# libsdl-org/libjxl

Hardware: AMD Instinct MI355X
Metric: megapixels/sec decode, 3840x2160 VarDCT d1.0 (higher is better)
Workload: dtype f32

## Files before the change

libjxl_amd/csrc/hip/jxl_hip_api.hip:

```cpp
#include <hip/hip_runtime.h>

#include <cmath>
#include <cstdio>
#include <cstdlib>
#include <cstring>
#include <algorithm>
#include <atomic>
#include <unistd.h>
#include <mutex>
#include <new>
#include <chrono>
#include <string>
#include <vector>

#include "../../../include/jxl_amd_hip.h"
#include "../host/jxh_enc_shared.h"
#include "jxl_hip_kernels.h"
#include "jxl_hip_entropy_lanes.h"
#include "jxl_hip_filter_fused.h"
#include "jxl_hip_modular.h"
#include "jxl_hip_enc.h"
#include "jxl_hip_canvas.h"
#include "jxl_hip_dc.h"

namespace {
#include "../host/afv_basis.inc"
#include "../host/dither.inc"

#define HIP_TRY(expr)                          \
  do {                                         \
    hipError_t e_ = (expr);                    \
    if (e_ != hipSuccess) return -int(e_);     \
  } while (0)

std::atomic<bool> g_yield_waits{false};
inline hipError_t WaitStream(hipStream_t st) {
  if (!g_yield_waits.load(std::memory_order_relaxed)) return hipStreamSynchronize(st);
  for (;;) {
    const hipError_t q = hipStreamQuery(st);
    if (q != hipErrorNotReady) return q;
    usleep(200);
  }
}
inline hipError_t WaitEvent(hipEvent_t ev) {
  if (!g_yield_waits.load(std::memory_order_relaxed)) return hipEventSynchronize(ev);
  for (;;) {
    const hipError_t q = hipEventQuery(ev);
    if (q != hipErrorNotReady) return q;
    usleep(100);
  }
}

constexpr size_t kGuardBytes = 4096;
inline bool GuardOn() {
  const char* e = getenv("JXLHIP_GUARD");
  return e && *e && atoi(e) != 0;
}
inline int GuardByte() {
  const char* e = getenv("JXLHIP_GUARD_BYTE");
  return e && *e ? (int(strtol(e, nullptr, 0)) & 0xFF) : 0xA5;
}

struct Buf {
  void* p = nullptr;
  size_t cap = 0;
  bool view = false;
  void* base = nullptr;
  int guard_byte = 0xA5;
  int Ensure(size_t n) {
    if (view) {
      p = nullptr;
      cap = 0;
      view = false;
    }
    if (n <= cap && p) return 0;
    if (p) {
      hipError_t e = hipFree(base ? base : p);
      p = base = nullptr;
      cap = 0;
      if (e != hipSuccess) return -int(e);
    }
    size_t want = n < 256 ? 256 : n;
    if (GuardOn()) {
      want = (want + 255) & ~size_t(255);
      hipError_t e = hipMalloc(&base, want + 2 * kGuardBytes);
      guard_byte = GuardByte();
      if (e == hipSuccess) e = hipMemset(base, guard_byte, want + 2 * kGuardBytes);
      if (e == hipSuccess) e = hipStreamSynchronize(nullptr);
      if (e != hipSuccess) {
        if (base) (void)hipFree(base);
        base = nullptr;
        return -int(e);
      }
      p = static_cast<uint8_t*>(base) + kGuardBytes;
      cap = want;
      return 0;
    }
    hipError_t e = hipMalloc(&p, want);
    if (e != hipSuccess) {
      p = nullptr;
      return -int(e);
    }
    cap = want;
    return 0;
  }
  void Free() {
    if (p && !view) (void)hipFree(base ? base : p);
    p = base = nullptr;
    cap = 0;
    view = false;
  }
  int GuardsTouched() const {
    if (!base || view) return 0;
    std::vector<uint8_t> h(2 * kGuardBytes);
    if (hipMemcpy(h.data(), base, kGuardBytes, hipMemcpyDeviceToHost) != hipSuccess) return 3;
    if (hipMemcpy(h.data() + kGuardBytes, static_cast<uint8_t*>(base) + kGuardBytes + cap, kGuardBytes, hipMemcpyDeviceToHost) != hipSuccess) return 3;
    int r = 0;
    for (size_t i = 0; i < kGuardBytes; i++) {
      if (h[i] != guard_byte) r |= 1;
      if (h[kGuardBytes + i] != guard_byte) r |= 2;
    }
    return r;
  }
  template <typename T>
  T* as() const { return static_cast<T*>(p); }
};

struct PassBufs {
  Buf ctx_map, alias, cfg, orders, ptable, poffset, alias_packed;
};

struct ModLaunch {
  uint32_t kind;
  size_t offset;
  uint32_t count, gx, gy;
};

struct Stage {
  uint8_t* p = nullptr;
  size_t cap = 0, used = 0;
  hipEvent_t done = nullptr;
  bool recorded = false;
};

constexpr int kEntropyWPG = 4;
constexpr int kLanesAdmitWaves = 4;
constexpr size_t kLdsBudget = 150 * 1024;

}

struct JxlHipContext {
  int device = 0;
  hipStream_t stream = nullptr;
  hipEvent_t ev[6] = {};
  bool ev_valid[3] = {false, false, false};
  Buf basis;
  Stage stage;
  Buf frame_blob;
  bool blob_mode = false;
  bool have_frame = false;
  uint32_t xs = 0, ys = 0, xb = 0, yb = 0, xg = 0, ng = 0, np = 0, xp = 0, yp = 0, coef_bits = 16;
  int gab = 0, epf_iters = 0;
  float epf_pass0 = 0.9f, epf_pass2 = 6.5f, epf_border = 2.0f / 3;
  Buf sections, sec_word, sec_size, blocks, gbb, bctx_lut, dequant, dc, inv_sigma, ytox, ytob, passes_dev, coeffs, errors;
  Buf dc_q, dc_ep;
  Buf dc_raw, sharp;
  Buf plane[3], rgb, tlist, scratch, sec_end, lz_window;
  bool generic_codec = false;
  bool lane_prefix = false;
  struct Modular {
    bool have = false;
    Buf pool, sections, blob, streams, rects, status, end_bits, scratch, windows, batch_streams;
    std::vector<size_t> buf_off;
    std::vector<uint32_t> buf_w, buf_h;
    std::vector<JxlHipModOp> ops;
    std::vector<jxlhip::ModStream> streams_host;
    std::vector<uint32_t> stream_samples;
    uint32_t out_buffer[4] = {0, 0, 0, 0};
    uint32_t num_color = 3, has_alpha = 0, bits = 8, alpha_bits = 8, xs = 0, ys = 0, nstreams = 0;
    bool xyb = false;
    float xyb_factor[3] = {0, 0, 0};
    jxlhip::FilterParams xyb_color;
    JxlHipColorTarget xyb_target;
    std::vector<const JxlHipContext*> batch_ctxs;
    std::vector<uint64_t> batch_gens;
    uint32_t batch_n = 0, batch_tree_cap = 0, batch_table_cap = 0;
    bool batch_wp = true, batch_refs = true;
    std::vector<uint32_t> code_table_words;
    Buf batch_ops;
    std::vector<ModLaunch> batch_launches;
  } mod;
  size_t plane_bytes = 0;
  Buf ep_dev;
  size_t batch_off_units = 0, batch_off_queue = 0, batch_off_wave_lanes = 0, batch_units = 0;
  Buf batch_params, batch_map, batch_lanes;
  uint32_t batch_wait_shift = 2;
  bool batch_galias = false;
  bool batch_a6 = false;
  bool batch_prefix = false;
  int batch_kernel = -1;
  std::vector<uint32_t> sec_size_host, sec_sel_host, pass_clusters, pass_log_alpha;
  std::vector<uint32_t> group_list;
  std::vector<uint32_t> absent_groups;
  std::vector<uint32_t> absent_blocks;
  std::vector<uint32_t> absent_sections;
  uint32_t band_y0 = 0, band_y1 = 0;
  uint32_t ext_y0 = 0, ext_y1 = 0;
  uint32_t ups = 1, oxs = 0, oys = 0;
  Buf ups_kernel;
  bool scan_order = false;
  bool lanes = false, lane_multi = false;
  uint32_t nblocks = 0;
  bool keep_filtered = false;
  bool keep_upsampled = false;
  bool ups_kept = false;
  bool transform_dense = false;
  bool band_halo = false;
  uint32_t out_type = 2, out_nc = 3, out_bits = 8, out_swap = 0;
  Buf enc_rgb, enc_planes[3], enc_act, enc_acs, enc_qf, enc_off, enc_dc, enc_coef, enc_lut, enc_dq, enc_ytox, enc_ytob;
  hipEvent_t enc_ev[6] = {nullptr, nullptr, nullptr, nullptr, nullptr, nullptr};
  bool enc_timed = false;
  jxlhip::EncTok enc_tok;
  bool enc_tok_ready = false;
  std::vector<uint32_t> enc_tok_totals;
  Buf enc_tok_orders, enc_tok_blk, enc_tok_info, enc_tok_off, enc_tok_nzmap, enc_tok_small, enc_tok_out, enc_tok_base;
  std::vector<uint32_t> ent_base, ent_count, ent_bits;
  bool ent_resident = false, ent_sized = false, ent_timed[3] = {false, false, false};
  jxlhip::EncAns ent;
  Buf ent_counts, ent_status, ent_grp, ent_tab, ent_rec, ent_fl, ent_small, ent_out, ent_obase;
  hipEvent_t ent_ev[6] = {nullptr, nullptr, nullptr, nullptr, nullptr, nullptr};
  jxlhip::EncFwd enc_last;
  jxlhip::EncAq enc_last_aq;
  Buf enc_aq_cells, enc_aq_map, enc_aq_mask, enc_aq_in;
  Buf enc_mask1x1;
  hipEvent_t mask_ev[2] = {nullptr, nullptr};
  bool mask_timed = false;
  bool enc_last_gaborish = false;
  uint32_t out_orient = 0;
  bool out_unpremul = false;
  Buf spl_seg, spl_row_start, spl_row_seg, spl_planes;
  uint32_t spl_segments = 0;
  Buf pat_rec, pat_row_start, pat_row_list;
  uint32_t pat_positions = 0;
  const float* pat_src[4] = {nullptr, nullptr, nullptr, nullptr};
  const float* pat_src_alpha[4] = {nullptr, nullptr, nullptr, nullptr};
  bool pat_uses_alpha = false, pat_premultiplied = false;
  Buf alpha_patched;
  bool alpha_patched_valid = false;
  uint32_t pat_src_w[4] = {0, 0, 0, 0}, pat_src_h[4] = {0, 0, 0, 0};
  bool keep_xyb = false;
  Buf noise;
  bool has_noise = false;
  float noise_lut[8] = {0, 0, 0, 0, 0, 0, 0, 0};
  uint32_t noise_seed[2] = {0, 0};
  float noise_ytox = 0.0f, noise_ytob = 1.0f;
  Buf alpha;
  bool have_alpha = false;
  bool color_out = false;
  bool gray8_fast = false;
  JxlHipColorTarget ct{};
  Buf kend, block_recs, dequant_scan;
  Buf trecs;
  Buf ec_stage;
  std::vector<JxlHipVarBlock> blocks_host;
  std::vector<uint32_t> gbb_host;
  std::vector<uint16_t> orders_host;
  uint32_t order_offset_host[39] = {};
  std::vector<const JxlHipContext*> batch_ctxs;
  std::vector<uint64_t> batch_gens;
  uint32_t batch_wgs = 0;
  size_t batch_lds = 0;
  hipEvent_t batch_done = nullptr;
  hipEvent_t pending_wait = nullptr;
  bool filter_async = false;
  bool entropy_gate = false;
  hipEvent_t halo_event = nullptr;
  Buf ups_planes;
  bool pooled_once = false;
  bool owns_stream = false;
  hipStream_t stream2 = nullptr;
  hipStream_t fstream = nullptr;
  hipEvent_t fork_event = nullptr, filter_done = nullptr, filter_wait = nullptr;
  hipEvent_t transform_done = nullptr;
  bool transform_done_valid = false;
  JxlHipContext* plane_lender = nullptr;
  hipEvent_t planes_event = nullptr;
  hipStream_t planes_stream = nullptr;
  struct FilterGroup {
    int key;
    uint32_t first, count, tiles_x, tiles_y;
    bool u8srgb;
  };
  Buf tb_params, tb_desc, fb_params;
  std::vector<const JxlHipContext*> db_ctxs;
  std::vector<uint64_t> db_gens;
  uint32_t desc_begin[27] = {}, desc_count[27] = {};
  uint32_t cs = 0;
  std::vector<FilterGroup> fgroups;
  hipEvent_t down_done = nullptr;
  uint64_t generation = 0;
  std::vector<PassBufs> pass_bufs;
  uint32_t list_begin[27] = {}, list_count[27] = {};
  jxlhip::EntropyParams ep;
  jxlhip::TransformParams tp;
  jxlhip::FilterParams fp;
  size_t lds_entropy = 0;
  bool alias_lds = false;
  int final_plane = 0;
};

static bool SectionEntropyForced() {
  static const bool v = [] {
    const char* e = getenv("JXLHIP_ENTROPY");
    return e && e[0] == '1';
  }();
  return v;
}
static JxlHipContext* PlaneHolder(JxlHipContext* c) { return c->plane_lender ? c->plane_lender : c; }
static const JxlHipContext* PlaneHolder(const JxlHipContext* c) { return c->plane_lender ? c->plane_lender : c; }

static size_t OutSampleBytes(const JxlHipContext* c) { return c->out_type == 2 ? 1 : (c->out_type == 0 ? 4 : 2); }
static size_t OutPixelBytes(const JxlHipContext* c) { return OutSampleBytes(c) * c->out_nc; }
static bool OutIsRgb8(const JxlHipContext* c) { return c->out_type == 2 && c->out_nc == 3 && c->out_bits == 8; }
static bool OutIsGray8(const JxlHipContext* c) { return c->out_type == 2 && c->out_nc == 1 && c->out_bits == 8; }
static bool OutIsRgbF32(const JxlHipContext* c) { return c->out_type == 0 && c->out_nc == 3 && !c->out_swap; }

static bool ValidPrefixTables(uint32_t offset_word, const uint32_t* table, size_t table_size) {
  const size_t first = offset_word & 0xFFFFFFu, root_bits = offset_word >> 24;
  if (root_bits > 15 || first + (size_t(1) << root_bits) > table_size) return false;
  for (size_t r = 0; r < (size_t(1) << root_bits); r++) {
    const uint32_t e = table[first + r];
    if (!(e & 0x80u)) {
      if ((e & 0xFFu) > 15) return false;
      continue;
    }
    const size_t sub_bits = e & 0x7Fu, sub = first + (e >> 8);
    if (sub_bits == 0 || root_bits + sub_bits > 15 || sub + (size_t(1) << sub_bits) > table_size) return false;
    for (size_t j = 0; j < (size_t(1) << sub_bits); j++)
      if ((table[sub + j] & 0x80u) || (table[sub + j] & 0xFFu) > 15) return false;
  }
  return true;
}

static int EnvInt(const char* name, int def) {
  const char* e = getenv(name);
  return e && *e ? atoi(e) : def;
}

extern "C" {

const char* jxlhip_version(void) { return "libjxl_amd 0.1 (gfx950)"; }

int jxlhip_device_count(void) {
  int n = 0;
  if (hipGetDeviceCount(&n) != hipSuccess) return 0;
  return n;
}

static hipStream_t PoolStream(int device) {
  static std::mutex mu;
  static std::vector<hipStream_t> pool[64];
  static size_t next[64] = {};
  std::lock_guard<std::mutex> lock(mu);
  if (device < 0 || device >= 64) return nullptr;
  if (pool[device].empty()) {
    int n = 4;
    if (const char* e = getenv("JXLHIP_STREAMS")) n = atoi(e);
    n = n < 1 ? 1 : (n > 16 ? 16 : n);
    for (int i = 0; i < n; i++) {
      hipStream_t st = nullptr;
      if (hipStreamCreateWithFlags(&st, hipStreamNonBlocking) != hipSuccess) break;
      pool[device].push_back(st);
    }
    if (pool[device].empty()) return nullptr;
  }
  return pool[device][next[device]++ % pool[device].size()];
}

static int EnsureOwnStream(JxlHipContext* c);

static std::mutex g_ctx_pool_mu;
static std::vector<JxlHipContext*> g_ctx_pool;
constexpr size_t kCtxPoolMax = 4, kCtxPoolBytes = size_t(1) << 30;
static std::vector<Buf*> AllBufs(JxlHipContext* c);
static JxlHipContext* RecycleContext(int device) {
  if (GuardOn() || !EnvInt("JXLHIP_CTX_POOL", 1)) return nullptr;
  JxlHipContext* o = nullptr;
  {
    std::lock_guard<std::mutex> lk(g_ctx_pool_mu);
    for (size_t i = 0; i < g_ctx_pool.size(); i++)
      if (g_ctx_pool[i]->device == device) {
        o = g_ctx_pool[i];
        g_ctx_pool.erase(g_ctx_pool.begin() + long(i));
        break;
      }
  }
  if (!o) return nullptr;
  JxlHipContext* c = new (std::nothrow) JxlHipContext;
  if (!c) {
    jxlhip_ctx_destroy(o);
    return nullptr;
  }
  c->device = device;
  c->stream = PoolStream(device);
  std::vector<Buf*> to = AllBufs(c), from = AllBufs(o);
  for (size_t i = 0; i < to.size(); i++) {
    *to[i] = *from[i];
    if (to[i]->view) *to[i] = Buf();
    *from[i] = Buf();
  }
  c->pass_bufs = std::move(o->pass_bufs);
  o->pass_bufs.clear();
  for (size_t i = 0; i < sizeof(c->ev) / sizeof(c->ev[0]); i++) std::swap(c->ev[i], o->ev[i]);
  for (size_t i = 0; i < sizeof(c->enc_ev) / sizeof(c->enc_ev[0]); i++) std::swap(c->enc_ev[i], o->enc_ev[i]);
  for (size_t i = 0; i < sizeof(c->ent_ev) / sizeof(c->ent_ev[0]); i++) std::swap(c->ent_ev[i], o->ent_ev[i]);
  for (size_t i = 0; i < sizeof(c->mask_ev) / sizeof(c->mask_ev[0]); i++) std::swap(c->mask_ev[i], o->mask_ev[i]);
  std::swap(c->stage, o->stage);
  jxlhip_ctx_destroy(o);
  return c;
}

int jxlhip_ctx_create(int device, JxlHipContext** out) {
  if (!out) return JXLHIP_ERR_INVALID_ARGUMENT;
  *out = nullptr;
  HIP_TRY(hipSetDevice(device));
  if (JxlHipContext* recycled = RecycleContext(device)) {
    *out = recycled;
    return 0;
  }
  JxlHipContext* c = new (std::nothrow) JxlHipContext;
  if (!c) return JXLHIP_ERR_INVALID_ARGUMENT;
  c->device = device;
  hipError_t e = hipSuccess;
  c->stream = PoolStream(device);
  if (!c->stream) {
    delete c;
    return JXLHIP_ERR_INVALID_ARGUMENT;
  }
  for (auto& ev : c->ev) {
    e = hipEventCreate(&ev);
    if (e != hipSuccess) {
      delete c;
      return -int(e);
    }
  }
  constexpr size_t kBasisFloats = 87381;
  std::vector<float> bt(2 * kBasisFloats + 4);
  for (int l = 0; l <= 8; l++) {
    const int N = 1 << l;
    float* dst = bt.data() + (size_t(N) * N - 1) / 3;
    float* dst_t = dst + kBasisFloats + 3;
    for (int k = 0; k < N; k++)
      for (int n = 0; n < N; n++) {
        const float v = float((k ? std::sqrt(2.0) : 1.0) * std::cos((n + 0.5) * k * M_PI / N));
        dst[size_t(k) * N + n] = v;
        dst_t[size_t(n) * N + k] = v;
      }
  }
  int r = c->basis.Ensure(bt.size() * sizeof(float));
  if (r) {
    jxlhip_ctx_destroy(c);
    return r;
  }
  float resample[63];
  for (int n = 1; n <= 32; n *= 2)
    for (int i = 0; i < n; i++) {
      const double N = 8.0 * n;
      resample[n - 1 + i] = float(1.0 / (std::cos(i / (2 * N) * M_PI) * std::cos(i / N * M_PI) * std::cos(i / (N / 2) * M_PI)));
    }
  e = hipMemcpy(c->basis.p, bt.data(), bt.size() * sizeof(float), hipMemcpyHostToDevice);
  if (e == hipSuccess) e = hipMemcpyToSymbol(HIP_SYMBOL(jxlhip::c_afv_basis), kAfvBasis, sizeof(kAfvBasis));
  if (e == hipSuccess) e = hipMemcpyToSymbol(HIP_SYMBOL(jxlhip::c_dither), kDither32, sizeof(kDither32));
  if (e == hipSuccess) e = hipMemcpyToSymbol(HIP_SYMBOL(jxlhip::c_resample), resample, sizeof(resample));
  if (e != hipSuccess) {
    jxlhip_ctx_destroy(c);
    return -int(e);
  }
  *out = c;
  return 0;
}

static std::vector<Buf*> AllBufs(JxlHipContext* c) {
  std::vector<Buf*> all = {&c->basis, &c->sections, &c->sec_word, &c->sec_size, &c->blocks, &c->gbb, &c->bctx_lut, &c->dequant, &c->dc, &c->dc_raw, &c->dc_q, &c->dc_ep, &c->sharp,
                &c->inv_sigma, &c->ytox, &c->ytob, &c->passes_dev, &c->coeffs, &c->errors, &c->plane[0], &c->plane[1],
                &c->plane[2], &c->rgb, &c->tlist, &c->scratch, &c->ep_dev, &c->batch_params, &c->batch_map, &c->batch_lanes, &c->ups_kernel, &c->kend, &c->block_recs, &c->dequant_scan, &c->ec_stage, &c->alpha_patched, &c->trecs, &c->enc_tok_orders, &c->enc_tok_blk, &c->enc_tok_info,
                &c->enc_tok_off, &c->enc_tok_nzmap, &c->enc_tok_small, &c->enc_tok_out, &c->enc_tok_base, &c->tb_params, &c->tb_desc, &c->fb_params, &c->alpha, &c->sec_end, &c->lz_window, &c->mod.pool, &c->mod.sections, &c->mod.blob, &c->mod.streams,
                &c->mod.rects, &c->mod.status, &c->mod.end_bits, &c->mod.scratch, &c->mod.windows, &c->mod.batch_streams, &c->mod.batch_ops, &c->frame_blob, &c->noise, &c->spl_seg, &c->spl_row_start, &c->spl_row_seg, &c->spl_planes, &c->pat_rec, &c->pat_row_start, &c->pat_row_list,
                &c->enc_rgb, &c->enc_planes[0], &c->enc_planes[1], &c->enc_planes[2], &c->enc_act, &c->enc_acs, &c->enc_qf, &c->enc_off, &c->enc_dc, &c->enc_coef, &c->enc_lut, &c->enc_dq, &c->enc_ytox, &c->enc_ytob, &c->ups_planes, &c->enc_aq_cells, &c->enc_aq_map, &c->enc_aq_mask, &c->enc_aq_in, &c->enc_mask1x1,
                &c->ent_counts, &c->ent_status, &c->ent_grp, &c->ent_tab, &c->ent_rec, &c->ent_fl, &c->ent_small, &c->ent_out, &c->ent_obase};
  for (auto& pb : c->pass_bufs)
    for (Buf* b : {&pb.ctx_map, &pb.alias, &pb.cfg, &pb.orders, &pb.ptable, &pb.poffset, &pb.alias_packed}) all.push_back(b);
  return all;
}

void jxlhip_ctx_destroy(JxlHipContext* c) {
  if (!c) return;
  (void)hipSetDevice(c->device);
  if (c->stream) (void)hipStreamSynchronize(c->stream);
  if (c->stream2) (void)hipStreamSynchronize(c->stream2);
  if (c->basis.p && !c->pooled_once && !GuardOn() && EnvInt("JXLHIP_CTX_POOL", 1)) {
    size_t bytes = 0;
    for (Buf* b : AllBufs(c))
      if (!b->view) bytes += b->cap;
    std::lock_guard<std::mutex> lk(g_ctx_pool_mu);
    if (bytes <= kCtxPoolBytes && g_ctx_pool.size() < kCtxPoolMax) {
      c->pooled_once = true;
      g_ctx_pool.push_back(c);
      return;
    }
  }
  std::vector<Buf*> all = AllBufs(c);
  for (Buf* b : all) b->Free();
  for (auto& ev : c->ev)
    if (ev) (void)hipEventDestroy(ev);
  for (auto& ev : c->enc_ev)
    if (ev) (void)hipEventDestroy(ev);
  for (auto& ev : c->ent_ev)
    if (ev) (void)hipEventDestroy(ev);
  for (auto& ev : c->mask_ev)
    if (ev) (void)hipEventDestroy(ev);
  if (c->stage.done) (void)hipEventDestroy(c->stage.done);
  if (c->stage.p) (void)hipHostFree(c->stage.p);
  if (c->batch_done) (void)hipEventDestroy(c->batch_done);
  if (c->down_done) (void)hipEventDestroy(c->down_done);
  if (c->fork_event) (void)hipEventDestroy(c->fork_event);
  if (c->transform_done) (void)hipEventDestroy(c->transform_done);
  if (c->filter_done) (void)hipEventDestroy(c->filter_done);
  if (c->halo_event) (void)hipEventDestroy(c->halo_event);
  if (c->stream2) (void)hipStreamDestroy(c->stream2);
  if (c->stream && c->owns_stream) (void)hipStreamDestroy(c->stream);
  delete c;
}

static int ApplyPendingWait(JxlHipContext* c) {
  if (c->pending_wait) {
    HIP_TRY(hipStreamWaitEvent(c->stream, c->pending_wait, 0));
    c->pending_wait = nullptr;
  }
  if (c->filter_wait) {
    HIP_TRY(hipStreamWaitEvent(c->stream, c->filter_wait, 0));
    c->filter_wait = nullptr;
  }
  return 0;
}

static hipStream_t CopyStream(int device) {
  static std::mutex mu;
  static hipStream_t streams[64] = {};
  std::lock_guard<std::mutex> lock(mu);
  if (device < 0 || device >= 64) return nullptr;
  if (!streams[device]) {
    int lo = 0, hi = 0;
    if (hipDeviceGetStreamPriorityRange(&lo, &hi) != hipSuccess) return nullptr;
    if (hipStreamCreateWithPriority(&streams[device], hipStreamNonBlocking, hi) != hipSuccess) streams[device] = nullptr;
  }
  return streams[device];
}

static int StageReset(JxlHipContext* c) {
  Stage& s = c->stage;
  if (!s.done) HIP_TRY(hipEventCreateWithFlags(&s.done, hipEventDisableTiming));
  if (s.recorded) HIP_TRY(hipEventSynchronize(s.done));
  else if (s.used) HIP_TRY(hipStreamSynchronize(c->stream));
  s.recorded = false;
  s.used = 0;
  return 0;
}
static int StageAlloc(JxlHipContext* c, size_t bytes, void** out) {
  Stage& s = c->stage;
  const size_t need = (bytes + 63) & ~size_t(63);
  if (s.used + need > s.cap) {
    if (c->blob_mode) return JXLHIP_ERR_INVALID_ARGUMENT;
    HIP_TRY(hipStreamSynchronize(c->stream));
    if (hipStream_t cs = CopyStream(c->device)) HIP_TRY(hipStreamSynchronize(cs));
    size_t want = s.cap * 2 > need ? s.cap * 2 : need;
    if (want < (size_t(1) << 22)) want = size_t(1) << 22;
    if (s.p) HIP_TRY(hipHostFree(s.p));
    s.p = nullptr;
    s.cap = 0;
    HIP_TRY(hipHostMalloc(reinterpret_cast<void**>(&s.p), want, hipHostMallocDefault));
    s.cap = want;
    s.used = 0;
  }
  *out = s.p + s.used;
  s.used += need;
  return 0;
}
static int UploadStaged(JxlHipContext* c, Buf& b, const void* staged, size_t bytes) {
  if (c->blob_mode) {
    const size_t at = size_t(static_cast<const uint8_t*>(staged) - c->stage.p);
    if (!staged || at + (bytes ? bytes : 16) > c->frame_blob.cap) return JXLHIP_ERR_INVALID_ARGUMENT;
    if (!b.view) b.Free();
    b.p = c->frame_blob.as<uint8_t>() + at;
    b.cap = bytes ? bytes : 16;
// ... 622 lines not shown
        rec |= (bctx & 15u) << (12 + 4 * ch);
        if (!carried) rec |= 1u << (24 + ch);
        rec |= hs << (27 + ch);
      }
      recs[i] = rec;
    }
    if ((r = Upload(c, c->block_recs, recs.data(), recs.size() * 4))) return r;
    ep.block_recs = c->block_recs.as<uint32_t>();
  }
  lap("records");
  c->absent_blocks.clear();
  for (uint32_t g : c->absent_groups) {
    c->absent_blocks.push_back(d->group_block_begin[g]);
    c->absent_blocks.push_back(d->group_block_begin[g + 1] - d->group_block_begin[g]);
  }
  if (c->scan_order) {
    c->blocks_host.assign(d->blocks, d->blocks + d->num_blocks);
    c->gbb_host.assign(d->group_block_begin, d->group_block_begin + d->num_groups + 1);
    c->orders_host.assign(d->passes[0].orders, d->passes[0].orders + d->passes[0].orders_size);
    memcpy(c->order_offset_host, d->passes[0].order_offset, sizeof(c->order_offset_host));
  }
  if ((r = Upload(c, c->ep_dev, &ep, sizeof(ep)))) return r;
  c->generation++;

  jxlhip::TransformParams& tp = c->tp;
  memset(&tp, 0, sizeof(tp));
  tp.coeffs = c->coeffs.p;
  tp.coef_bits = d->coef_bits;
  tp.blocks = c->blocks.as<JxlHipVarBlock>();
  tp.dequant = c->dequant.as<float>();
  memcpy(tp.dq_offset, d->dequant_offset, sizeof(tp.dq_offset));
  memcpy(tp.dq_size, d->dequant_size, sizeof(tp.dq_size));
  for (int s = 0; s < 27; s++) {
    if (c->list_count[s] == 0) continue;
    const uint32_t k = jxlhip::kStrategyQuantTable[s];
    if (d->dequant_size[k] != 64u * jxlhip::CoveredBlocks(s) || size_t(d->dequant_offset[k]) + 3 * size_t(d->dequant_size[k]) > d->dequant_floats)
      return JXLHIP_ERR_INVALID_ARGUMENT;
  }
  tp.dense = c->transform_dense ? 1 : 0;
  tp.cs = cs;
  tp.cs_out = c->plane[1].as<float>();
  tp.dc = c->dc.as<float>();
  tp.ytox = c->ytox.as<int8_t>();
  tp.ytob = c->ytob.as<int8_t>();
  tp.basis_t = c->basis.as<float>();
  tp.basis_n = c->basis.as<float>() + 87381 + 3;
  tp.inv_global_scale = d->inv_global_scale;
  tp.x_dm = d->x_dm;
  tp.b_dm = d->b_dm;
  tp.color_scale = d->color_scale;
  tp.base_x = d->base_corr_x;
  tp.base_b = d->base_corr_b;
  memcpy(tp.biases, d->quant_biases, sizeof(tp.biases));
  tp.xb = c->xb; tp.yb = c->yb; tp.xg = c->xg; tp.xp = c->xp; tp.yp = c->yp;
  tp.out = PlaneHolder(c)->plane[0].as<float>();
  tp.scratch = c->scratch.as<float>();
  tp.tlist = c->tlist.as<uint32_t>();
  tp.trecs = c->trecs.as<uint4>();
  memcpy(tp.list_begin, c->list_begin, sizeof(tp.list_begin));
  memcpy(tp.list_count, c->list_count, sizeof(tp.list_count));
  tp.scan_order = c->scan_order ? 1 : 0;
  tp.kend = c->kend.as<uint32_t>();
  tp.orders = c->pass_bufs[0].orders.as<uint16_t>();
  tp.dequant_scan = nullptr;
  if (c->scan_order) {
    std::vector<float> scan(d->dequant_floats, 0.0f);
    for (int st = 0; st < 27; st++) {
      if (!c->list_count[st]) continue;
      const uint32_t kind = jxlhip::kStrategyQuantTable[st], size = d->dequant_size[kind];
      for (int ch = 0; ch < 3; ch++) {
        const uint32_t oo = d->passes[0].order_offset[jxlhip::kStrategyOrder[st] * 3 + ch];
        if (size_t(oo) + size > d->passes[0].orders_size) return JXLHIP_ERR_INVALID_ARGUMENT;
        const uint16_t* order = d->passes[0].orders + oo;
        const float* m = d->dequant + d->dequant_offset[kind] + size_t(ch) * size;
        float* o = scan.data() + d->dequant_offset[kind] + size_t(ch) * size;
        for (uint32_t k = 0; k < size; k++) {
          if (order[k] >= size) return JXLHIP_ERR_INVALID_ARGUMENT;
          o[k] = m[order[k]];
        }
      }
    }
    if ((r = Upload(c, c->dequant_scan, scan.data(), scan.size() * 4))) return r;
    tp.dequant_scan = c->dequant_scan.as<float>();
  }
  memcpy(tp.order_offset, d->passes[0].order_offset, sizeof(tp.order_offset));

  jxlhip::FilterParams& fp = c->fp;
  memset(&fp, 0, sizeof(fp));
  fp.xs = c->xs; fp.ys = c->ys; fp.xp = c->xp; fp.yp = c->yp; fp.xb = c->xb;
  fp.y_begin = c->band_y0; fp.y_end = c->band_y1;
  fp.inv_sigma = c->inv_sigma.as<float>();
  for (int ch = 0; ch < 3; ch++) {
    const float w1 = d->gab_w[ch * 2], w2 = d->gab_w[ch * 2 + 1];
    const float mul = 1.0f / (1.0f + 4 * (w1 + w2));
    fp.gab_w[ch * 3] = mul;
    fp.gab_w[ch * 3 + 1] = w1 * mul;
    fp.gab_w[ch * 3 + 2] = w2 * mul;
    fp.ch_scale[ch] = d->epf_channel_scale[ch];
    fp.opsin_bias[ch] = d->opsin_bias[ch];
    fp.opsin_bias_cbrt[ch] = cbrtf(d->opsin_bias[ch]);
  }
  memcpy(fp.opsin_inv, d->opsin_inv, sizeof(fp.opsin_inv));
  fp.linear_output = d->linear_output;
  c->gray8_fast = OutIsGray8(c) && !c->color_out;
  fp.rgb = OutIsRgb8(c) || c->gray8_fast ? c->rgb.as<uint8_t>() : nullptr;
  fp.rgbf = !OutIsRgb8(c) && !c->gray8_fast && !c->color_out ? c->rgb.as<float>() : nullptr;
  c->epf_pass0 = d->epf_pass0_sigma_scale;
  c->epf_pass2 = d->epf_pass2_sigma_scale;
  c->epf_border = d->epf_border_sad_mul;
  c->ev_valid[0] = c->ev_valid[1] = c->ev_valid[2] = false;
  if ((r = BlobEnd(c, dev_smooth && !d->dc_device ? &smooth_p : nullptr, dev_sigma ? &sigma_p : nullptr, dev_dequant ? &dequant_p : nullptr))) return r;
  HIP_TRY(WaitEvent(c->stage.done));
  lap("rest");
  if (prof) fprintf(stderr, "[upload] %s\n", prof_line.c_str());
  c->have_frame = true;
  c->mod.have = false;
  return 0;
}

}

template <typename CoefT>
static int LaunchEntropy(JxlHipContext* c) {
  const dim3 grid(c->ng), block(64);
  if (c->generic_codec) {
    hipLaunchKernelGGL(jxlhip::k_entropy_generic<CoefT>, grid, block, 3072, c->stream, c->ep);
  } else if (c->alias_lds) {
    const size_t shared = size_t(c->ep.lds_ctx_bytes) + c->ep.lds_alias_bytes + 1024;
    jxlhip::EntropyBatch b{c->ep_dev.as<jxlhip::EntropyParams>(), nullptr};
    if (c->ep.num_hist == 1) {
      constexpr int WPG = kEntropyWPG;
      auto k = jxlhip::k_entropy_uni<CoefT, WPG>;
      const size_t lds = shared + WPG * 5120;
      if (lds > 48 * 1024)
        HIP_TRY(hipFuncSetAttribute(reinterpret_cast<const void*>(k), hipFuncAttributeMaxDynamicSharedMemorySize, int(lds)));
      hipLaunchKernelGGL(k, dim3((c->ng + WPG - 1) / WPG), dim3(64 * WPG), lds, c->stream, b);
    } else {
      auto k = jxlhip::k_entropy_uni<CoefT, 1>;
      const size_t lds = shared + 5120;
      if (lds > 48 * 1024)
        HIP_TRY(hipFuncSetAttribute(reinterpret_cast<const void*>(k), hipFuncAttributeMaxDynamicSharedMemorySize, int(lds)));
      hipLaunchKernelGGL(k, grid, block, lds, c->stream, b);
    }
  } else {
    hipLaunchKernelGGL(jxlhip::k_entropy_ans<CoefT>, grid, block, c->lds_entropy, c->stream, c->ep);
  }
  HIP_TRY(hipGetLastError());
  return 0;
}

static int RunEntropySingle(JxlHipContext* c) {
  if (!c) return JXLHIP_ERR_INVALID_ARGUMENT;
  if (!c->have_frame) return JXLHIP_ERR_NO_FRAME;
  HIP_TRY(hipSetDevice(c->device));
  {
    int pw = ApplyPendingWait(c);
    if (pw) return pw;
  }
  HIP_TRY(hipEventRecord(c->ev[0], c->stream));
  HIP_TRY(hipMemsetAsync(c->errors.p, 0, size_t(c->ng) * 4, c->stream));
  int r = c->coef_bits == 16 ? LaunchEntropy<int16_t>(c) : LaunchEntropy<int32_t>(c);
  if (r) return r;
  HIP_TRY(hipEventRecord(c->ev[1], c->stream));
  c->ev_valid[0] = true;
  return 0;
}

static uint32_t BlocksPerWG(int s) {
  const uint32_t cx = jxlhip::kCoveredX[s], cy = jxlhip::kCoveredY[s];
  if (s == 0 || (s >= 4 && s <= 11) || (s >= 18 && s <= 20))
    return jxlhip::IdctFastThreads(cx, cy) / ((cx > cy ? cx : cy) * 8);
  return 4;
}

template <typename CoefT, int CX, int CY, bool CS = false>
static int LaunchIdctFast(JxlHipContext* c0, int s) {
  constexpr int C = CX * 8, R = CY * 8, TB = R > C ? R : C, GROUPS = jxlhip::IdctFastThreads(CX, CY) / TB;
  constexpr size_t lds = size_t(GROUPS) * R * (C + 1) * sizeof(float);
  const int li = CS ? 21 : s;
  hipLaunchKernelGGL((jxlhip::k_idct_fast<CoefT, CX, CY, CS>), dim3(c0->desc_count[li]), dim3(jxlhip::IdctFastThreads(CX, CY)), lds, c0->stream,
                     c0->tb_params.as<jxlhip::TransformParams>(), c0->tb_desc.as<uint2>() + c0->desc_begin[li], uint32_t(s));
  return 0;
}

template <typename CoefT>
static int LaunchTransforms(JxlHipContext* c0) {
  for (int s = 0; s < 21; s++) {
    if (!c0->desc_count[s]) continue;
    int e = 0;
    switch (s) {
      case 0: e = LaunchIdctFast<CoefT, 1, 1>(c0, s); break;
      case 4: e = LaunchIdctFast<CoefT, 2, 2>(c0, s); break;
      case 5: e = LaunchIdctFast<CoefT, 4, 4>(c0, s); break;
      case 6: e = LaunchIdctFast<CoefT, 1, 2>(c0, s); break;
      case 7: e = LaunchIdctFast<CoefT, 2, 1>(c0, s); break;
      case 8: e = LaunchIdctFast<CoefT, 1, 4>(c0, s); break;
      case 9: e = LaunchIdctFast<CoefT, 4, 1>(c0, s); break;
      case 10: e = LaunchIdctFast<CoefT, 2, 4>(c0, s); break;
      case 11: e = LaunchIdctFast<CoefT, 4, 2>(c0, s); break;
      case 18: e = LaunchIdctFast<CoefT, 8, 8>(c0, s); break;
      case 19: e = LaunchIdctFast<CoefT, 4, 8>(c0, s); break;
      case 20: e = LaunchIdctFast<CoefT, 8, 4>(c0, s); break;
      default:
        hipLaunchKernelGGL((jxlhip::k_special<CoefT>), dim3(c0->desc_count[s]), dim3(256), 0, c0->stream,
                           c0->tb_params.as<jxlhip::TransformParams>(), c0->tb_desc.as<uint2>() + c0->desc_begin[s], uint32_t(s));
    }
    if (e) return e;
    HIP_TRY(hipGetLastError());
  }
  if (c0->desc_count[21]) {
    int e = LaunchIdctFast<CoefT, 1, 1, true>(c0, 0);
    if (e) return e;
    HIP_TRY(hipGetLastError());
  }
  for (const JxlHipContext* c : c0->db_ctxs) {
    if (!c->cs) continue;
    for (uint32_t ch = 0; ch < 3; ch++) {
      jxlhip::ChromaUpParams up;
      up.hs = (c->cs >> (2 * ch)) & 1u;
      up.vs = (c->cs >> (2 * ch + 1)) & 1u;
      if (!(up.hs | up.vs)) continue;
      const size_t plane = size_t(c->xp) * c->yp;
      up.src = c->plane[1].as<float>() + ch * plane;
      up.dst = PlaneHolder(c)->plane[0].as<float>() + ch * plane;
      up.xs = c->xs;
      up.ys = c->ys;
      up.xp = c->xp;
      up.y0 = c->ext_y0;
      up.y1 = c->ext_y1;
      if (up.y1 <= up.y0) continue;
      hipLaunchKernelGGL(jxlhip::k_chroma_upsample, dim3((up.xs + 63) / 64, (up.y1 - up.y0 + 3) / 4), dim3(256), 0, c0->stream, up);
    }
    HIP_TRY(hipGetLastError());
  }
  for (const JxlHipContext* c : c0->db_ctxs)
    for (int s = 21; s < 27; s++) {
      const uint32_t n = c->list_count[s];
      if (!n) continue;
      const uint32_t* list = c->tlist.as<uint32_t>() + c->list_begin[s];
      for (uint32_t i = 0; i < n; i += 32) {
        const uint32_t m = n - i < 32 ? n - i : 32;
        hipLaunchKernelGGL((jxlhip::k_dct_big<CoefT>), dim3(m * 3), dim3(256), 0, c0->stream, c->tp, list + i, m, uint32_t(s));
      }
      HIP_TRY(hipGetLastError());
    }
  return 0;
}

static void FillFusedParams(const JxlHipContext* c, jxlhip::FusedFilterParams* p) {
  p->debug = uint32_t(EnvInt("JXLHIP_FILTER_DEBUG", 0));
  p->f = c->fp;
  p->f.in = PlaneHolder(c)->plane[0].as<float>();
  p->f.out = nullptr;
  for (int stage = 0; stage < 3; stage++) {
    const float scale = stage == 0 ? c->epf_pass0 : stage == 2 ? c->epf_pass2 : 1.0f;
    p->sm[stage] = stage == 1 ? 1.65f : float(scale * 1.65);
    p->bsm[stage] = p->sm[stage] * c->epf_border;
  }
  p->filtered = (c->keep_filtered || c->ups != 1 || c->color_out) ? c->plane[1].as<float>() : nullptr;
  if (c->ups != 1 || c->color_out) {
    p->f.rgb = nullptr;
    p->f.rgbf = nullptr;
  }
}
static int FilterKey(const JxlHipContext* c) {
  const int epf = c->epf_iters < 0 ? 0 : (c->epf_iters > 3 ? 3 : c->epf_iters);
  return (c->gray8_fast ? 8 : 0) + (c->gab ? 4 : 0) + epf;
}
static int PrepareDownstream(JxlHipContext* c0, JxlHipContext* const* ctxs, size_t n) {
  bool same = c0->db_ctxs.size() == n;
  for (size_t i = 0; same && i < n; i++) same = c0->db_ctxs[i] == ctxs[i] && c0->db_gens[i] == ctxs[i]->generation;
  if (same) return 0;
  std::vector<jxlhip::TransformParams> tparams(n);
  for (size_t i = 0; i < n; i++) {
    tparams[i] = ctxs[i]->tp;
    const JxlHipContext* h = PlaneHolder(ctxs[i]);
    if (!h->plane[0].p || h->plane[0].cap < ctxs[i]->plane_bytes) return JXLHIP_ERR_INVALID_ARGUMENT;
    tparams[i].out = h->plane[0].as<float>();
    if (ctxs[i]->cs && (!ctxs[i]->plane[1].p || ctxs[i]->plane[1].cap < ctxs[i]->plane_bytes)) return JXLHIP_ERR_INVALID_ARGUMENT;
    tparams[i].cs_out = ctxs[i]->plane[1].as<float>();
  }
  std::vector<uint2> desc;
  for (int s = 0; s < 22; s++) {
    c0->desc_begin[s] = uint32_t(desc.size());
    const int st = s == 21 ? 0 : s;
    const uint32_t bpw = BlocksPerWG(st);
    for (size_t i = 0; i < n; i++) {
      if (st == 0 && (ctxs[i]->cs != 0) != (s == 21)) continue;
      for (uint32_t j = 0; j < ctxs[i]->list_count[st]; j += bpw) desc.push_back(make_uint2(uint32_t(i), j));
    }
    c0->desc_count[s] = uint32_t(desc.size()) - c0->desc_begin[s];
  }
  std::vector<size_t> order(n);
  for (size_t i = 0; i < n; i++) order[i] = i;
  std::stable_sort(order.begin(), order.end(), [&](size_t a, size_t b) { return FilterKey(ctxs[a]) < FilterKey(ctxs[b]); });
  std::vector<jxlhip::FusedFilterParams> fparams(n);
  c0->fgroups.clear();
  for (size_t j = 0; j < n; j++) {
    const JxlHipContext* c = ctxs[order[j]];
    FillFusedParams(c, &fparams[j]);
    const int key = FilterKey(c);
    const uint32_t tx = (c->xs + jxlhip::kFusedTW - 1) / jxlhip::kFusedTW;
    const uint32_t ty = (c->band_y1 - c->band_y0 + jxlhip::kFusedTH - 1) / jxlhip::kFusedTH;
    if (c0->fgroups.empty() || c0->fgroups.back().key != key) c0->fgroups.push_back({key, uint32_t(j), 0, 0, 0, true});
    JxlHipContext::FilterGroup& g = c0->fgroups.back();
    g.count++;
    g.u8srgb = g.u8srgb && fparams[j].f.rgb && !fparams[j].f.rgbf && !fparams[j].filtered && !fparams[j].f.linear_output;
    if (c->gray8_fast && !g.u8srgb) return JXLHIP_ERR_INVALID_ARGUMENT;
    g.tiles_x = tx > g.tiles_x ? tx : g.tiles_x;
    g.tiles_y = ty > g.tiles_y ? ty : g.tiles_y;
  }
  int r;
  if ((r = c0->tb_params.Ensure(n * sizeof(tparams[0])))) return r;
  if ((r = c0->tb_desc.Ensure((desc.size() + 1) * sizeof(uint2)))) return r;
  if ((r = c0->fb_params.Ensure(n * sizeof(fparams[0])))) return r;
  {
    ParamCopy pc;
    if ((r = pc.Begin(c0))) return r;
    if ((r = pc.Add(c0->tb_params.p, tparams.data(), n * sizeof(tparams[0])))) return r;
    if ((r = pc.Add(c0->tb_desc.p, desc.data(), desc.size() * sizeof(uint2)))) return r;
    if ((r = pc.Add(c0->fb_params.p, fparams.data(), n * sizeof(fparams[0])))) return r;
    if ((r = pc.End())) return r;
  }
  c0->db_ctxs.assign(ctxs, ctxs + n);
  c0->db_gens.resize(n);
  for (size_t i = 0; i < n; i++) c0->db_gens[i] = ctxs[i]->generation;
  return 0;
}

template <bool GAB, int EPF>
static int LaunchFused(JxlHipContext* c0, const JxlHipContext::FilterGroup& g) {
  auto k = jxlhip::k_filter_fused<GAB, EPF>;
  constexpr size_t lds = jxlhip::FusedLdsBytes(GAB, EPF);
  if (lds > 48 * 1024)
    HIP_TRY(hipFuncSetAttribute(reinterpret_cast<const void*>(k), hipFuncAttributeMaxDynamicSharedMemorySize, int(lds)));
  for (uint32_t z = 0; z < g.count; z += 65535) {
    const uint32_t zn = g.count - z < 65535 ? g.count - z : 65535;
    hipLaunchKernelGGL(k, dim3(g.tiles_x, g.tiles_y, zn), dim3(jxlhip::kFusedThreads), lds, c0->fstream,
                       c0->fb_params.as<jxlhip::FusedFilterParams>() + g.first + z);
  }
  HIP_TRY(hipGetLastError());
  return 0;
}

static int LaunchFilterRows(JxlHipContext* c0, const JxlHipContext::FilterGroup& g, int epf, bool gab, bool gray = false) {
  const uint32_t cols = g.tiles_x * jxlhip::kFusedTW, rows = g.tiles_y * jxlhip::kFusedTH;
  const uint32_t gx = ((cols + jxlhip::kRows2Cols - 1) / jxlhip::kRows2Cols + jxlhip::kRowsWaves - 1) / jxlhip::kRowsWaves;
  uint32_t strip = jxlhip::kRowsStrip;
  if (uint64_t(gx) * jxlhip::kRowsWaves * ((rows + 2 * strip - 1) / (2 * strip)) * g.count >= 6 * 1024) strip *= 2;
  const uint32_t gy = (rows + strip - 1) / strip;
  typedef void (*RowsKernel)(const jxlhip::FusedFilterParams*, int);
  const RowsKernel k1t = jxlhip::k_filter_rows2<true, 1>, k1f = jxlhip::k_filter_rows2<false, 1>;
  const RowsKernel k2t = jxlhip::k_filter_rows2<true, 2>, k2f = jxlhip::k_filter_rows2<false, 2>;
  const RowsKernel n1t = jxlhip::k_filter_rows2<true, 1, false>, n1f = jxlhip::k_filter_rows2<false, 1, false>;
  const RowsKernel n2t = jxlhip::k_filter_rows2<true, 2, false>, n2f = jxlhip::k_filter_rows2<false, 2, false>;
  const RowsKernel k1g = jxlhip::k_filter_rows2<true, 1, true, true>, k2g = jxlhip::k_filter_rows2<true, 2, true, true>;
  const RowsKernel n1g = jxlhip::k_filter_rows2<true, 1, false, true>, n2g = jxlhip::k_filter_rows2<true, 2, false, true>;
  if (gray && !g.u8srgb) return JXLHIP_ERR_INVALID_ARGUMENT;
  const RowsKernel k = gray ? (gab ? (epf == 2 ? k2g : k1g) : (epf == 2 ? n2g : n1g))
                       : gab ? (epf == 2 ? (g.u8srgb ? k2t : k2f) : (g.u8srgb ? k1t : k1f))
                             : (epf == 2 ? (g.u8srgb ? n2t : n2f) : (g.u8srgb ? n1t : n1f));
  for (uint32_t z = 0; z < g.count; z += 65535) {
    const uint32_t zn = g.count - z < 65535 ? g.count - z : 65535;
    const jxlhip::FusedFilterParams* fp = c0->fb_params.as<jxlhip::FusedFilterParams>() + g.first + z;
    hipLaunchKernelGGL(k, dim3(gx, gy, zn), dim3(64 * jxlhip::kRowsWaves), 0, c0->fstream, fp, int(strip));
  }
  HIP_TRY(hipGetLastError());
  return 0;
}

static int EnsureOwnStream(JxlHipContext* c) {
  if (c->owns_stream) return 0;
  HIP_TRY(hipSetDevice(c->device));
  HIP_TRY(hipStreamSynchronize(c->stream));
  hipStream_t st = nullptr;
  HIP_TRY(hipStreamCreateWithFlags(&st, hipStreamNonBlocking));
  c->stream = st;
  c->owns_stream = true;
  return 0;
}

struct EntropyGate {
  unsigned long long* counter = nullptr;
  unsigned long long total = 0;
  unsigned long long target = 0;
  unsigned cus = 256;
  size_t lds_per_cu = 160 * 1024;
  bool tried = false;
};
static std::mutex g_gate_mu;
static EntropyGate g_gate[16];
static bool RuntimeMaySerialise() {
  static const bool v = [] {
    auto on = [](const char* n) {
      const char* e = getenv(n);
      return e && *e && !(e[0] == '0' && !e[1]);
    };
    if (on("AMD_SERIALIZE_KERNEL") || on("AMD_SERIALIZE_COPY") || on("HIP_LAUNCH_BLOCKING") || on("ROCPROF_COUNTER_COLLECTION") ||
        on("HSA_ENABLE_DEBUG") || on("ROCM_DEBUG_AGENT") || on("HIP_ENABLE_DEFERRED_LOADING_DEBUG"))
      return true;
    if (const char* q = getenv("GPU_MAX_HW_QUEUES"))
      if (*q && atoi(q) < 2) return true;
    if (const char* t = getenv("HSA_TOOLS_LIB"))
      if (*t && (strstr(t, "debug") || strstr(t, "rocgdb"))) return true;
    return false;
  }();
  return v;
}
static unsigned long long* GateCounter(const JxlHipContext* c0) {
  const int device = c0->device;
  if (device < 0 || device >= 16 || !c0->entropy_gate || !EnvInt("JXLHIP_ENTROPY_GATE", 1) || RuntimeMaySerialise()) return nullptr;
  std::lock_guard<std::mutex> lk(g_gate_mu);
  EntropyGate& g = g_gate[device];
  if (!g.tried) {
    g.tried = true;
    int can = 0;
    if (hipDeviceGetAttribute(&can, hipDeviceAttributeCanUseStreamWaitValue, device) == hipSuccess && can) {
      void* p = nullptr;
      if (hipExtMallocWithFlags(&p, 8, hipMallocSignalMemory) == hipSuccess && hipMemset(p, 0, 8) == hipSuccess)
        g.counter = static_cast<unsigned long long*>(p);
    }
    (void)hipGetLastError();
    int cus = 0, lds = 0;
    if (hipDeviceGetAttribute(&cus, hipDeviceAttributeMultiprocessorCount, device) == hipSuccess && cus > 0) g.cus = unsigned(cus);
    if (hipDeviceGetAttribute(&lds, hipDeviceAttributeMaxSharedMemoryPerMultiprocessor, device) == hipSuccess && lds > 0) g.lds_per_cu = size_t(lds);
    (void)hipGetLastError();
  }
  return g.counter;
}
static void GateAdvance(int device, unsigned long long workgroups, unsigned long long resident_cap) {
  std::lock_guard<std::mutex> lk(g_gate_mu);
  EntropyGate& g = g_gate[device];
  g.target = g.total + (workgroups < resident_cap ? workgroups : resident_cap);
  g.total += workgroups;
}
static int GateWait(int device, hipStream_t stream) {
  if (device < 0 || device >= 16) return 0;
  unsigned long long* counter;
  unsigned long long target;
  {
    std::lock_guard<std::mutex> lk(g_gate_mu);
    counter = g_gate[device].counter;
    target = g_gate[device].target;
  }
  if (!counter || !target) return 0;
  HIP_TRY(hipStreamWaitValue64(stream, counter, target, hipStreamWaitValueGte, ~0ull));
  return 0;
}

static int BeginDownstreamBatch(JxlHipContext* const* ctxs, size_t n, bool filter_stage = false) {
  if (!ctxs || !n) return JXLHIP_ERR_INVALID_ARGUMENT;
  JxlHipContext* c0 = ctxs[0];
  for (size_t i = 0; i < n; i++) {
    if (!ctxs[i]) return JXLHIP_ERR_INVALID_ARGUMENT;
    if (!ctxs[i]->have_frame) return JXLHIP_ERR_NO_FRAME;
    if (ctxs[i]->device != c0->device || ctxs[i]->coef_bits != c0->coef_bits) return JXLHIP_ERR_INVALID_ARGUMENT;
  }
  HIP_TRY(hipSetDevice(c0->device));
  if (n > 1) {
    const int r = EnsureOwnStream(c0);
    if (r) return r;
  }
  hipStream_t ls = c0->stream;
  if (filter_stage && c0->filter_async) {
    if (!c0->stream2) {
      HIP_TRY(hipStreamCreateWithFlags(&c0->stream2, hipStreamNonBlocking));
      if (!c0->fork_event) HIP_TRY(hipEventCreateWithFlags(&c0->fork_event, hipEventDisableTiming));
      HIP_TRY(hipEventCreateWithFlags(&c0->filter_done, hipEventDisableTiming));
    }
    ls = c0->stream2;
    if (c0->transform_done_valid) {
      HIP_TRY(hipStreamWaitEvent(ls, c0->transform_done, 0));
    } else {
      HIP_TRY(hipEventRecord(c0->fork_event, c0->stream));
      HIP_TRY(hipStreamWaitEvent(ls, c0->fork_event, 0));
    }
  }
  c0->fstream = ls;
  if (n > 1 && c0->entropy_gate && !RuntimeMaySerialise()) {
    const int r = GateWait(c0->device, ls);
    if (r) return r;
  }
  hipEvent_t waited = nullptr;
  for (size_t i = 0; i < n; i++)
    if (ctxs[i]->pending_wait) {
      if (ctxs[i]->pending_wait != waited) HIP_TRY(hipStreamWaitEvent(ls, ctxs[i]->pending_wait, 0));
      waited = ctxs[i]->pending_wait;
      ctxs[i]->pending_wait = nullptr;
    }
  waited = nullptr;
  for (size_t i = 0; i < n; i++)
    if (ctxs[i]->filter_wait) {
      if (ctxs[i]->filter_wait != waited) HIP_TRY(hipStreamWaitEvent(ls, ctxs[i]->filter_wait, 0));
      waited = ctxs[i]->filter_wait;
      ctxs[i]->filter_wait = nullptr;
    }
  waited = nullptr;
  for (size_t i = 0; i < n; i++) {
    JxlHipContext* h = PlaneHolder(ctxs[i]);
    if (h->planes_event && h->planes_stream != ls && h->planes_event != waited) {
      HIP_TRY(hipStreamWaitEvent(ls, h->planes_event, 0));
      waited = h->planes_event;
    }
  }
  return PrepareDownstream(c0, ctxs, n);
}
static int EndDownstreamBatch(JxlHipContext* const* ctxs, size_t n, bool filter_stage = false) {
  JxlHipContext* c0 = ctxs[0];
  bool shared = false;
  for (size_t i = 0; i < n && !shared; i++) shared = ctxs[i]->plane_lender != nullptr || ctxs[i]->planes_event != nullptr;
  hipEvent_t done = nullptr;
  if (filter_stage && c0->fstream != c0->stream) {
    HIP_TRY(hipEventRecord(c0->filter_done, c0->fstream));
    done = c0->filter_done;
    for (size_t i = 0; i < n; i++) ctxs[i]->filter_wait = done;
  } else if (n > 1 || shared) {
    if (!c0->down_done) HIP_TRY(hipEventCreateWithFlags(&c0->down_done, hipEventDisableTiming));
    HIP_TRY(hipEventRecord(c0->down_done, c0->stream));
    done = c0->down_done;
    for (size_t i = 1; i < n; i++) ctxs[i]->pending_wait = done;
  }
  if (!filter_stage && c0->filter_async) {
    if (!c0->transform_done) HIP_TRY(hipEventCreateWithFlags(&c0->transform_done, hipEventDisableTiming));
    HIP_TRY(hipEventRecord(c0->transform_done, c0->stream));
    c0->transform_done_valid = true;
  }
  if (shared && filter_stage)
    for (size_t i = 0; i < n; i++) {
      JxlHipContext* h = PlaneHolder(ctxs[i]);
      h->planes_event = done;
      h->planes_stream = c0->fstream;
    }
  return 0;
}

template <typename CoefT, bool AIDS, bool GALIAS, bool PREFIX = false, bool A6 = false>
static int LaunchEntropyLanesW(JxlHipContext* c0) {
  auto k = jxlhip::k_entropy_lanes<CoefT, AIDS, GALIAS, PREFIX, A6>;
  if (c0->batch_lds > 48 * 1024)
    HIP_TRY(hipFuncSetAttribute(reinterpret_cast<const void*>(k), hipFuncAttributeMaxDynamicSharedMemorySize, int(c0->batch_lds)));
  jxlhip::EntropyLaneBatch b;
  b.params = c0->batch_params.as<jxlhip::EntropyParams>();
  uint8_t* blob = c0->batch_lanes.as<uint8_t>();
  b.wg_unit = c0->batch_map.as<uint32_t>();
  b.list = reinterpret_cast<const uint32_t*>(blob);
  b.units = reinterpret_cast<const uint4*>(blob + c0->batch_off_units);
  b.queue = reinterpret_cast<uint32_t*>(blob + c0->batch_off_queue);
  b.wave_lanes = blob + c0->batch_off_wave_lanes;
  HIP_TRY(hipMemsetAsync(b.queue, 0, c0->batch_units * 4, c0->stream));
  b.wait_shift = c0->batch_wait_shift;
  b.refill_mask = jxlhip::kLanesAsmTrip<CoefT, GALIAS, PREFIX> ? 0u : jxlhip::kLanesRefillEvery - 1;
  b.extra_pass_min = jxlhip::kLanesExtraPassMin;
  b.debug = uint32_t(EnvInt("JXLHIP_LANES_DEBUG", 0));
  b.prof = nullptr;
  b.started = c0->batch_ctxs.size() > 1 ? GateCounter(c0) : nullptr;
  const bool prof = EnvInt("JXLHIP_LANES_PROF", 0) != 0;
  const size_t nwaves = c0->batch_wgs;
  if (prof) {
    HIP_TRY(hipMalloc(reinterpret_cast<void**>(&b.prof), nwaves * 64));
    HIP_TRY(hipMemsetAsync(b.prof, 0, nwaves * 64, c0->stream));
  }
  hipLaunchKernelGGL(k, dim3(c0->batch_wgs), dim3(64), c0->batch_lds, c0->stream, b);
  HIP_TRY(hipGetLastError());
  if (b.started) {
    unsigned long long cus, lds_cu;
    {
      std::lock_guard<std::mutex> lk(g_gate_mu);
      cus = g_gate[c0->device].cus;
      lds_cu = g_gate[c0->device].lds_per_cu;
    }
    const unsigned long long per_cu = c0->batch_lds ? lds_cu / c0->batch_lds : 8, cap = cus * (per_cu ? per_cu : 1) * 3 / 4;
    GateAdvance(c0->device, c0->batch_wgs, cap);
  }
  if (prof) {
    std::vector<unsigned long long> h(nwaves * 8);
    HIP_TRY(hipStreamSynchronize(c0->stream));
    HIP_TRY(hipMemcpy(h.data(), b.prof, nwaves * 64, hipMemcpyDeviceToHost));
    (void)hipFree(b.prof);
    unsigned long long mx[8] = {0, 0, 0, 0, 0, 0, 0, 0};
    double sum[8] = {0, 0, 0, 0, 0, 0, 0, 0};
    size_t used = 0;
    for (size_t w = 0; w < nwaves; w++) {
      if (!h[w * 8 + 3] && !h[w * 8 + 2]) continue;
      used++;
      if (h[w * 8] > mx[0]) for (int j = 0; j < 8; j++) mx[j] = h[w * 8 + j];
      for (int j = 0; j < 8; j++) sum[j] += double(h[w * 8 + j]);
    }
    const char* names[8] = {"cycles", "refill_cycles", "passes", "trips", "lane_trips", "trip_cycles", "pass_lanes_served", "pass_cycles"};
    std::string line = "{\"waves\": " + std::to_string(used) + ", \"longest\": {";
    for (int j = 0; j < 8; j++) line += std::string(j ? ", " : "") + "\"" + names[j] + "\": " + std::to_string(mx[j]);
    line += "}, \"mean\": {";
    for (int j = 0; j < 8; j++) line += std::string(j ? ", " : "") + "\"" + names[j] + "\": " + std::to_string((unsigned long long)(sum[j] / (used ? used : 1)));
    line += "}}";
    fprintf(stderr, "[lanes prof] %s\n", line.c_str());
    if (b.debug & 16)
      for (size_t w = 0; w < nwaves && w < 64; w++) {
        const unsigned long long hw = h[w * 8 + 6];
        fprintf(stderr, "[lanes wave] %zu cycles %llu trips %llu trip_cycles %llu pass_cycles %llu passes %llu refill_cycles %llu simd %llu cu %llu sh %llu se %llu xcc %llu\n", w, h[w * 8], h[w * 8 + 3], h[w * 8 + 5], h[w * 8 + 7], h[w * 8 + 2], h[w * 8 + 1], (hw >> 4) & 3,
                (hw >> 8) & 15, (hw >> 12) & 1, (hw >> 13) & 7, (hw >> 32) & 15);
      }
  }
  return 0;
}

template <typename CoefT>
static int LaunchEntropyLanes(JxlHipContext* c0) {
  if (c0->batch_prefix) return LaunchEntropyLanesW<CoefT, false, true, true>(c0);
  if constexpr (sizeof(CoefT) == 2) {
    if (c0->batch_a6) return LaunchEntropyLanesW<CoefT, false, false, false, true>(c0);
  }
  if (EnvInt("JXLHIP_LANES_DEBUG", 0) || EnvInt("JXLHIP_LANES_PROF", 0))
    return c0->batch_galias ? LaunchEntropyLanesW<CoefT, true, true>(c0) : LaunchEntropyLanesW<CoefT, true, false>(c0);
  return c0->batch_galias ? LaunchEntropyLanesW<CoefT, false, true>(c0) : LaunchEntropyLanesW<CoefT, false, false>(c0);
}

template <typename CoefT>
static int LaunchEntropyUniBatch(JxlHipContext* c0) {
  auto k = jxlhip::k_entropy_uni<CoefT, kEntropyWPG>;
  if (c0->batch_lds > 48 * 1024)
    HIP_TRY(hipFuncSetAttribute(reinterpret_cast<const void*>(k), hipFuncAttributeMaxDynamicSharedMemorySize, int(c0->batch_lds)));
  jxlhip::EntropyBatch b{c0->batch_params.as<jxlhip::EntropyParams>(), c0->batch_map.as<uint32_t>()};
  hipLaunchKernelGGL(k, dim3(c0->batch_wgs), dim3(64 * kEntropyWPG), c0->batch_lds, c0->stream, b);
  HIP_TRY(hipGetLastError());
  return 0;
}

static int PrepareBatch(JxlHipContext* c0, JxlHipContext* const* ctxs, size_t n, int kernel) {
  bool same = c0->batch_ctxs.size() == n && c0->batch_kernel == kernel;
  for (size_t i = 0; same && i < n; i++) same = c0->batch_ctxs[i] == ctxs[i] && c0->batch_gens[i] == ctxs[i]->generation;
  if (same) return 0;
  std::vector<jxlhip::EntropyParams> params(n);
  std::vector<uint32_t> map, list, unit_desc;
  std::vector<uint8_t> wave_lanes;
  size_t lds = 0;
  for (size_t i = 0; i < n; i++) params[i] = ctxs[i]->ep;
  if (kernel == 2) {
    constexpr uint32_t kSectionBytes = 4000;
    constexpr size_t kTargetWaves = 1024;
    const int forced = EnvInt("JXLHIP_LANES", 0);
    c0->batch_wait_shift = uint32_t(EnvInt("JXLHIP_WAIT_SHIFT", 1));
    struct Unit {
      uint32_t frame, sel, pass, begin, count, min_lanes, lanes;
    };
    std::vector<Unit> units;
    std::vector<uint32_t> order;
    size_t min_total = 0, total_sections = 0;
    for (size_t i = 0; i < n; i++) {
      const JxlHipContext* c = ctxs[i];
      for (uint32_t pass = 0; pass < c->np; pass++)
      for (uint32_t sel = 0; sel < c->ep.num_hist; sel++) {
        const uint32_t* sz = c->sec_size_host.data() + size_t(pass) * c->ng;
        const uint32_t* ssel = c->sec_sel_host.data() + size_t(pass) * c->ng;
        order.clear();
        for (uint32_t g : c->group_list) {
          if (pass && sz[g] == 0 && !c->absent_sections.empty()) continue;
          if (ssel[g] == sel || (sel == 0 && ssel[g] >= c->ep.num_hist)) order.push_back(g);
        }
        if (order.empty()) continue;
        std::stable_sort(order.begin(), order.end(), [sz](uint32_t a, uint32_t b) { return sz[a] > sz[b]; });
        uint64_t total = 0;
        for (uint32_t g : order) total += uint64_t(sz[g]) + kSectionBytes;
        const uint64_t longest = uint64_t(sz[order[0]]) + kSectionBytes;
        Unit u;
        u.frame = uint32_t(i);
        u.sel = sel;
        u.pass = pass;
        u.begin = uint32_t(list.size());
        u.count = uint32_t(order.size());
        u.min_lanes = uint32_t((total + longest - 1) / longest);
        u.min_lanes = u.min_lanes > u.count ? u.count : (u.min_lanes ? u.min_lanes : 1);
        u.lanes = u.min_lanes;
        list.insert(list.end(), order.begin(), order.end());
        min_total += u.min_lanes;
        total_sections += u.count;
        units.push_back(u);
      }
    }
    uint32_t lanes_per_wave = 1;
    while (lanes_per_wave < 64 && (min_total + lanes_per_wave - 1) / lanes_per_wave > kTargetWaves) lanes_per_wave *= 2;
    if (forced >= 1 && forced <= 64 && (forced & (forced - 1)) == 0) lanes_per_wave = uint32_t(forced);
    if (lanes_per_wave >= 32) {
      lanes_per_wave = 64;
      for (Unit& u : units)
        if (u.lanes < 64) u.lanes = u.count < 64 ? u.count : 64;
    }
    if (lanes_per_wave == 1 && min_total < kTargetWaves) {
      const double grow = double(kTargetWaves) / double(min_total);
      for (Unit& u : units) {
        const uint32_t want = uint32_t(double(u.min_lanes) * grow);
        u.lanes = want > u.count ? u.count : (want < u.min_lanes ? u.min_lanes : want);
      }
    }
    for (const Unit& u : units) {
      const uint32_t waves = (u.lanes + lanes_per_wave - 1) / lanes_per_wave;
      const uint32_t unit_index = uint32_t(unit_desc.size() / 4);
      unit_desc.push_back(u.frame | u.sel << 16);
      unit_desc.push_back(u.begin);
      unit_desc.push_back(u.count);
      unit_desc.push_back(u.pass);
      for (uint32_t w = 0; w < waves; w++) {
        const uint32_t cnt = u.lanes / waves + (w < u.lanes % waves ? 1u : 0u);
        map.push_back(unit_index);
        wave_lanes.push_back(uint8_t(cnt));
      }
    }
    size_t lds_by_form[3] = {0, 0, 0};
    const size_t num_wgs = map.size();
    bool a6_ok = !c0->lane_prefix && c0->coef_bits == 16 && EnvInt("JXLHIP_A6", 1) != 0;
    for (int form = 0; form < 3; form++)
      for (size_t wg = 0; wg < num_wgs; wg++) {
        const JxlHipContext* c = ctxs[unit_desc[size_t(map[wg]) * 4] & 0xFFFF];
        const uint32_t up = unit_desc[size_t(map[wg]) * 4 + 3];
        if (c->pass_log_alpha[up] > 7 || c->pass_clusters[up] > jxlhip::kLanesA6Clusters ||
            (size_t(c->pass_clusters[up]) << c->pass_log_alpha[up]) > jxlhip::kLanesA6Slots)
          a6_ok = false;
        size_t l = jxlhip::LanesLdsLayout(1, c->ep.nctx, c->pass_clusters[up], c->pass_log_alpha[up], 0, 0, form == 0 && !c0->lane_prefix,
                                          c0->lane_prefix, form == 2).wave0;
        l += size_t(jxlhip::kLanesPerLaneBytes) * 64;
        lds_by_form[form] = l > lds_by_form[form] ? l : lds_by_form[form];
      }
    int dev_cus = 256;
    (void)hipDeviceGetAttribute(&dev_cus, hipDeviceAttributeMultiprocessorCount, c0->device);
    const size_t resident = lds_by_form[0] ? size_t(dev_cus) * ((160 * 1024) / lds_by_form[0]) : num_wgs;
    bool galias = lds_by_form[0] > kLdsBudget || resident < num_wgs;
    const int forced_form = EnvInt("JXLHIP_GALIAS", -1);
    if (forced_form == 0 && lds_by_form[0] <= kLdsBudget) galias = false;
    if (forced_form == 1) galias = true;
    if (c0->lane_prefix) galias = true;
    const size_t resident6 = lds_by_form[2] ? size_t(dev_cus) * ((160 * 1024) / lds_by_form[2]) : num_wgs;
    const bool a6 = a6_ok && lds_by_form[2] <= kLdsBudget &&
                    ((galias && forced_form != 1 && resident6 >= num_wgs) || EnvInt("JXLHIP_A6", 1) == 2);
    if (a6) galias = false;
    c0->batch_a6 = a6;
    c0->batch_galias = galias;
    c0->batch_prefix = c0->lane_prefix;
    lds = lds_by_form[a6 ? 2 : (galias ? 1 : 0)];
    if (EnvInt("JXLHIP_PACK_DEBUG", 0))
      fprintf(stderr, "[pack] units %zu sections %zu lanes(min) %zu lanes/wave %u waves/wg 1 workgroups %zu lds %zu tables %s\n", units.size(),
              total_sections, min_total, lanes_per_wave, map.size(), lds,
              c0->lane_prefix ? "prefix" : (a6 ? "lds6" : (galias ? "global" : "lds8")));
  } else {
    for (size_t i = 0; i < n; i++) {
      const uint32_t wgs = (ctxs[i]->ng + kEntropyWPG - 1) / kEntropyWPG;
      for (uint32_t j = 0; j < wgs; j++) map.push_back(uint32_t(i) << 16 | j);
      const size_t l = size_t(ctxs[i]->ep.lds_ctx_bytes) + ctxs[i]->ep.lds_alias_bytes + 1024 + kEntropyWPG * 5120;
      lds = l > lds ? l : lds;
    }
  }
  int r;
  if ((r = c0->batch_params.Ensure(params.size() * sizeof(params[0])))) return r;
  if ((r = c0->batch_map.Ensure(map.size() * 4))) return r;
  ParamCopy pc;
  if ((r = pc.Begin(c0))) return r;
  if ((r = pc.Add(c0->batch_params.p, params.data(), params.size() * sizeof(params[0])))) return r;
  if ((r = pc.Add(c0->batch_map.p, map.data(), map.size() * 4))) return r;
  if (!list.empty()) {
    const size_t o_units = (list.size() * 4 + 15) & ~size_t(15), o_queue = o_units + unit_desc.size() * 4;
    const size_t o_wl = o_queue + unit_desc.size(), total = o_wl + wave_lanes.size();
    std::vector<uint8_t> blob(total, 0);
    memcpy(blob.data(), list.data(), list.size() * 4);
    memcpy(blob.data() + o_units, unit_desc.data(), unit_desc.size() * 4);
    memcpy(blob.data() + o_wl, wave_lanes.data(), wave_lanes.size());
    if ((r = c0->batch_lanes.Ensure(total))) return r;
    if ((r = pc.Add(c0->batch_lanes.p, blob.data(), total))) return r;
    c0->batch_off_units = o_units;
    c0->batch_off_queue = o_queue;
    c0->batch_off_wave_lanes = o_wl;
    c0->batch_units = unit_desc.size() / 4;
  }
  if ((r = pc.End())) return r;
  c0->batch_ctxs.assign(ctxs, ctxs + n);
  c0->batch_gens.resize(n);
  for (size_t i = 0; i < n; i++) c0->batch_gens[i] = ctxs[i]->generation;
  c0->batch_wgs = uint32_t(map.size());
  c0->batch_lds = lds;
  c0->batch_kernel = kernel;
  return 0;
}

extern "C" int jxlhip_run_entropy_batch(JxlHipContext* const* ctxs, size_t n) {
  if (!ctxs || !n || n > 0xFFFF) return JXLHIP_ERR_INVALID_ARGUMENT;
  JxlHipContext* c0 = ctxs[0];
  bool all_scan = true, all_uni = true;
  for (size_t i = 0; i < n; i++) {
    const JxlHipContext* c = ctxs[i];
    if (!c) return JXLHIP_ERR_INVALID_ARGUMENT;
    if (!c->have_frame) return JXLHIP_ERR_NO_FRAME;
    if (c->device != c0->device) return JXLHIP_ERR_INVALID_ARGUMENT;
    if (n > 1 && !c->absent_groups.empty()) return JXLHIP_ERR_INVALID_ARGUMENT;
    if (!c->lanes || c->coef_bits != c0->coef_bits || c->lane_prefix != c0->lane_prefix) all_scan = false;
    if (c->lanes || c->generic_codec || !c->alias_lds || c->ep.num_hist != 1 || c->np != 1 || c->coef_bits != c0->coef_bits ||
        c->ng > 0xFFFF * kEntropyWPG)
      all_uni = false;
  }
  if (!all_scan && !all_uni) {
    for (size_t i = 0; i < n; i++) {
      int r = ctxs[i]->lanes ? jxlhip_run_entropy_batch(&ctxs[i], 1) : RunEntropySingle(ctxs[i]);
      if (r) return r;
    }
    return 0;
  }
  const int kernel = all_scan ? 2 : 1;
  HIP_TRY(hipSetDevice(c0->device));
  if (n > 1) {
    const int r = EnsureOwnStream(c0);
    if (r) return r;
  }
  const bool prof = EnvInt("JXLHIP_BATCH_PROF", 0) != 0;
  std::chrono::steady_clock::time_point tp0 = std::chrono::steady_clock::now();
  std::string prof_line;
  auto lap = [&](const char* what) {
    if (!prof) return;
    const auto now = std::chrono::steady_clock::now();
    prof_line += std::string(what) + " " + std::to_string(std::chrono::duration_cast<std::chrono::microseconds>(now - tp0).count()) + "  ";
    tp0 = now;
  };
  if (!c0->batch_done) HIP_TRY(hipEventCreateWithFlags(&c0->batch_done, hipEventDisableTiming));
  int r = PrepareBatch(c0, ctxs, n, kernel);
  if (r) return r;
  lap("prepare");
  for (size_t i = 1; i < n; i++) {
    if (ctxs[i]->ev_valid[2]) HIP_TRY(hipStreamWaitEvent(c0->stream, ctxs[i]->ev[5], 0));
  }
  hipEvent_t waited = nullptr;
  for (size_t i = 0; i < n; i++)
    if (ctxs[i]->pending_wait) {
      if (ctxs[i]->pending_wait != waited) HIP_TRY(hipStreamWaitEvent(c0->stream, ctxs[i]->pending_wait, 0));
      waited = ctxs[i]->pending_wait;
      ctxs[i]->pending_wait = nullptr;
    }
  lap("waits");
  HIP_TRY(hipEventRecord(c0->ev[0], c0->stream));
  for (size_t i = 0; i < n; i++)
    if (kernel != 2 || ctxs[i]->np > 1) HIP_TRY(hipMemsetAsync(ctxs[i]->errors.p, 0, size_t(ctxs[i]->ng) * 4, c0->stream));
  if (kernel == 2) r = c0->coef_bits == 16 ? LaunchEntropyLanes<int16_t>(c0) : LaunchEntropyLanes<int32_t>(c0);
  else r = c0->coef_bits == 16 ? LaunchEntropyUniBatch<int16_t>(c0) : LaunchEntropyUniBatch<int32_t>(c0);
  if (r) return r;
  if (kernel == 2)
    for (size_t i = 0; i < n; i++) {
      const JxlHipContext* c = ctxs[i];
      if (!c->lane_multi) continue;
      jxlhip::MergeParams m;
      m.coeffs = c->coeffs.p;
      m.blocks = c->blocks.as<JxlHipVarBlock>();
      m.passes = c->passes_dev.as<jxlhip::PassDev>();
      m.kend = c->kend.as<uint32_t>();
      m.pass_stride = c->ep.coef_pass_stride;
      m.num_blocks = c->nblocks;
      m.num_passes = c->np;
      m.xg = c->xg;
      m.kend_stride = c->ep.kend_pass_stride;
      if (!m.num_blocks) continue;
      if (c->coef_bits == 16) hipLaunchKernelGGL(jxlhip::k_merge_passes<int16_t>, dim3(m.num_blocks), dim3(64), 0, c0->stream, m);
      else hipLaunchKernelGGL(jxlhip::k_merge_passes<int32_t>, dim3(m.num_blocks), dim3(64), 0, c0->stream, m);
      HIP_TRY(hipGetLastError());
    }
  lap("launch");
  if (prof) fprintf(stderr, "[entropy batch] %s\n", prof_line.c_str());
  HIP_TRY(hipEventRecord(c0->ev[1], c0->stream));
  c0->ev_valid[0] = true;
  if (n > 1) {
    HIP_TRY(hipEventRecord(c0->batch_done, c0->stream));
    for (size_t i = 1; i < n; i++) {
      ctxs[i]->pending_wait = c0->batch_done;
      ctxs[i]->ev_valid[0] = false;
    }
  }
  return 0;
}

static int ZeroAbsentGroups(JxlHipContext* c) {
  if (c->absent_groups.empty() && c->absent_sections.empty()) return 0;
  HIP_TRY(hipSetDevice(c->device));
  const size_t coef_group_bytes = size_t(3) * 65536 * (c->coef_bits / 8);
  for (size_t i = 0; i < c->absent_groups.size(); i++) {
    const uint32_t g = c->absent_groups[i], b0 = c->absent_blocks[2 * i], nb = c->absent_blocks[2 * i + 1];
    HIP_TRY(hipMemsetAsync(c->coeffs.as<uint8_t>() + size_t(g) * coef_group_bytes, 0, coef_group_bytes, c->stream));
    for (uint32_t p = 0; p < c->np && nb && c->lanes; p++)
      HIP_TRY(hipMemsetAsync(c->kend.as<uint32_t>() + size_t(p) * c->ep.kend_pass_stride + size_t(b0) * 3, 0, size_t(nb) * 12, c->stream));
  }
  for (size_t i = 0; c->lanes && i + 2 < c->absent_sections.size(); i += 3) {
    const uint32_t p = c->absent_sections[i], b0 = c->absent_sections[i + 1], nb = c->absent_sections[i + 2];
    if (nb) HIP_TRY(hipMemsetAsync(c->kend.as<uint32_t>() + size_t(p) * c->ep.kend_pass_stride + size_t(b0) * 3, 0, size_t(nb) * 12, c->stream));
  }
  return 0;
}

extern "C" int jxlhip_run_entropy(JxlHipContext* c) {
  if (!c) return JXLHIP_ERR_INVALID_ARGUMENT;
  if (!c->have_frame) return JXLHIP_ERR_NO_FRAME;
  const int r = ZeroAbsentGroups(c);
  if (r) return r;
  if (c->group_list.empty()) {
    HIP_TRY(hipMemsetAsync(c->errors.p, 0, size_t(c->ng) * 4, c->stream));
    return 0;
  }
  return c->lanes ? jxlhip_run_entropy_batch(&c, 1) : RunEntropySingle(c);
}


static int UploadSplines(JxlHipContext* c, const JxlHipSplines& sp, uint32_t ysize) {
// ... 2137 lines not shown
```

libjxl_amd/csrc/hip/jxl_hip_entropy_lanes.h:

```cpp
#ifndef JXL_HIP_ENTROPY_LANES_H_
#define JXL_HIP_ENTROPY_LANES_H_

#include "jxl_hip_kernels.h"
#include "jxl_hip_lanes_trip.inc"

namespace jxlhip {

struct EntropyLaneBatch {
  const EntropyParams* params;
  const uint32_t* wg_unit;
  const uint4* units;
  const uint32_t* list;
  uint32_t* queue;
  const uint8_t* wave_lanes;
  uint32_t extra_pass_min;
  uint32_t wait_shift;
  uint32_t refill_mask;
  uint32_t debug;
  unsigned long long* started;
  unsigned long long* prof;
};

struct LanesLds {
  uint32_t f2, alias, ctx, ctx2, cfg, poff, wave0, per_wave, total;
};
constexpr uint32_t kLanesF2Bytes = 128;
constexpr uint32_t kLanesNzRows = 96;
constexpr uint32_t kLanesRingWords = 16;
constexpr uint32_t kLanesBlockRing = 8;
constexpr int kLanesTrips = 4;
constexpr uint32_t kLanesRefillEvery = 4;
constexpr uint32_t kLanesExtraPassMin = 8;
constexpr uint32_t kLanesPerLaneBytes = kLanesNzRows + (kLanesRingWords + 2) * 4 + kLanesBlockRing * 4;
constexpr uint32_t kLanesA6Clusters = 128, kLanesA6Slots = 8192, kLanesA6B = 128, kLanesA6A = kLanesA6B + kLanesA6Slots * 2,
                   kLanesA6Cfg = kLanesA6A + kLanesA6Slots * 4, kLanesA6End = kLanesA6Cfg + kLanesA6Clusters * 2;
static_assert(kLanesA6A == 16512 && kLanesA6Cfg == 49280, "jxl_hip_lanes_trip.inc LT_EREAD_6 has these as immediates");
__host__ __device__ inline LanesLds LanesLdsLayout(uint32_t num_hist, uint32_t nctx, uint32_t num_clusters, uint32_t log_alpha,
                                                   uint32_t waves, uint32_t lanes, bool alias_lds = true, bool prefix = false, bool a6 = false) {
  LanesLds l;
  l.f2 = 0;
  l.alias = kLanesF2Bytes;
  l.ctx = a6 ? kLanesA6End : l.alias + (alias_lds ? (num_clusters << log_alpha) * 8 : 0);
  l.ctx2 = l.ctx + ((num_hist * nctx + 16 + 15) & ~15u);
  l.cfg = l.ctx2 + 64 * 2;
  l.poff = l.cfg + (prefix ? 256 * 2 : 0);
  l.wave0 = l.poff + (prefix ? 256 * 4 : 0);
  l.per_wave = kLanesPerLaneBytes * lanes;
  l.total = l.wave0 + waves * l.per_wave;
  return l;
}

typedef uint8_t __attribute__((address_space(3))) LdsU8;
typedef uint16_t __attribute__((address_space(3))) LdsU16;
typedef uint32_t __attribute__((address_space(3))) LdsU32;
typedef uint32_t LanesU32x2 __attribute__((ext_vector_type(2)));
typedef LanesU32x2 __attribute__((address_space(3))) LdsU32x2;

__device__ __forceinline__ void LaneStore64(const void* base, uint32_t off, uint32_t lo, uint32_t hi) {
  const LanesU32x2 v = {lo, hi};
  asm volatile("global_store_dwordx2 %0, %1, %2" : : "v"(off), "v"(v), "s"(base));
}
__device__ __forceinline__ void LaneStore32(const void* base, uint32_t off, uint32_t v) {
  asm volatile("global_store_dword %0, %1, %2" : : "v"(off), "v"(v), "s"(base));
}
__device__ __forceinline__ void LaneStore16(const void* base, uint32_t off, uint32_t v) {
  asm volatile("global_store_short %0, %1, %2" : : "v"(off), "v"(v), "s"(base));
}
__device__ __forceinline__ void LaneDmaDword(uint32_t lds_row, const void* base, uint32_t off) {
  uint32_t keep;
  asm volatile(
      "s_mov_b32 %0, m0\n\ts_mov_b32 m0, %2\n\ts_nop 0\n\tglobal_load_lds_dword %1, %3\n\ts_mov_b32 m0, %0"
      : "=&s"(keep)
      : "v"(off), "s"(lds_row), "s"(base)
      : "memory");
}
__device__ __forceinline__ void LaneDmaWait() { asm volatile("s_waitcnt vmcnt(0)" : : : "memory"); }
typedef uint32_t LanesU32x4 __attribute__((ext_vector_type(4)));
__device__ __forceinline__ void LaneLoad128(LanesU32x4& d, unsigned long long mask, const void* base, uint32_t off) {
  asm volatile("s_mov_b64 s[96:97], exec\n\ts_and_b64 exec, exec, %3\n\tglobal_load_dwordx4 %0, %1, %2\n\ts_mov_b64 exec, s[96:97]"
               : "+v"(d)
               : "v"(off), "s"(base), "s"(mask)
               : "memory", "s96", "s97", "scc");
}
__device__ __forceinline__ void LaneLoadWait(LanesU32x4& a, LanesU32x4& b) {
  asm volatile("s_waitcnt vmcnt(0)" : "+v"(a), "+v"(b) : : "memory");
}

__device__ __forceinline__ uint32_t LaneHybrid(uint32_t tok, uint32_t cfg, uint32_t w0, uint32_t w1, uint32_t w2, uint32_t boff,
                                               uint32_t& nb) {
  const uint32_t se = cfg & 15, msb = (cfg >> 4) & 15, lsb = (cfg >> 8) & 15;
  nb = (se - (msb + lsb) + ((tok - (1u << se)) >> (msb + lsb))) & 31u;
  const uint32_t low = tok & ((1u << lsb) - 1), top = tok >> lsb;
  const bool up = boff >= 32;
  const uint32_t xb = __builtin_amdgcn_alignbit(up ? w2 : w1, up ? w1 : w0, boff & 31) & ((1u << nb) - 1);
  return (((((1u << msb) | (top & ((1u << msb) - 1))) << nb) | xb) << lsb) | low;
}

template <typename CoefT, bool GALIAS, bool PREFIX>
constexpr bool kLanesAsmTrip = sizeof(CoefT) == 2 && !GALIAS && !PREFIX;

template <typename CoefT, bool AIDS, bool GALIAS = false, bool PREFIX = false, bool A6 = false>
__global__ __launch_bounds__(64) void k_entropy_lanes(EntropyLaneBatch B_) {
  constexpr bool ASMT = kLanesAsmTrip<CoefT, GALIAS, PREFIX>;
  static_assert(!A6 || (!GALIAS && !PREFIX), "the six-byte form is an LDS form of the rANS tables");
  EntropyLaneBatch B = B_;
  if (!AIDS) {
    B.prof = nullptr;
    B.debug = 0;
  }
  extern __shared__ __align__(16) uint8_t lds_raw[];
  const uint32_t tid = threadIdx.x, lane = tid & 63;
  if (B_.started && tid == 0) __hip_atomic_fetch_add(B_.started, 1ull, __ATOMIC_RELAXED, __HIP_MEMORY_SCOPE_SYSTEM);
  typedef const uint32_t __attribute__((address_space(4)))* CU32;
  const uint32_t wid = blockIdx.x;
  const uint32_t unit = ((CU32)(uintptr_t)B.wg_unit)[wid];
  const CU32 ud = (CU32)(uintptr_t)(B.units + unit);
  const uint32_t wg_desc = ud[0], list_begin = ud[1], list_count = ud[2], pass = ud[3];
  const uint32_t wg_sel = wg_desc >> 16;
  EntropyParams P;
  LoadParams(P, B.params + (wg_desc & 0xFFFF));
  PassDev T;
  LoadParams(T, P.passes + pass);
  const uint32_t log_alpha = T.log_alpha, log_entry = 12 - log_alpha, nclusters = T.num_clusters;
  const uint32_t entry_mask = (1u << log_entry) - 1, cl_shift = (A6 ? 1 : 3) + log_alpha;
  const uint32_t num_bctx = P.num_bctx, nctx = P.nctx, num_hist = P.num_hist;
  const LanesLds L = LanesLdsLayout(1, nctx, nclusters, log_alpha, 0, 0, !GALIAS && !PREFIX, PREFIX, A6);
  const uint2* const galias = T.alias_packed;
  const uint32_t* const ptable = T.prefix_table;
  LdsU8* const lds = (LdsU8*)lds_raw;
  auto alias_entry = [&](uint32_t cluster, uint32_t slot) -> LanesU32x2 {
    if constexpr (A6) {
      const uint32_t i = ((cluster << log_alpha) + slot) & (kLanesA6Slots - 1);
      const uint32_t b = ((LdsU16*)(lds + kLanesA6B))[i], a = ((LdsU32*)(lds + kLanesA6A))[i];
      const uint32_t cfg = ((LdsU16*)(lds + kLanesA6Cfg))[cluster & (kLanesA6Clusters - 1)];
      const uint32_t cutoff = (b >> 12) << (8 - log_alpha) | a >> (24 + log_alpha);
      return LanesU32x2{(b & 0xFFFu) | cfg << 12 | cutoff << 24, a & ((1u << (24 + log_alpha)) - 1)};
    } else {
      return *(LdsU32x2*)((LdsU8*)lds + kLanesF2Bytes + (cluster << cl_shift) + slot * 8);
    }
  };
  LdsU8* const l_ctx = lds + L.ctx;
  LdsU16* const l_nnz2 = (LdsU16*)(lds + L.ctx2);
  LdsU16* const l_cfg = (LdsU16*)(lds + L.cfg);
  LdsU32* const l_poff = (LdsU32*)(lds + L.poff);
  const uint32_t wave_base = L.wave0;
  const uint32_t col = lane;
  LdsU8* const l_nz = lds + wave_base + col;
  const uint32_t ring_row0 = wave_base + kLanesNzRows * 64;
  const uint32_t bring_row0 = ring_row0 + (kLanesRingWords + 2) * 256;
  LdsU32* const ring = (LdsU32*)(lds + ring_row0) + col;
  LdsU32* const bring = (LdsU32*)(lds + bring_row0) + col;
  const uint32_t lds_abs = uint32_t(uintptr_t(lds));

  {
    const uint32_t n_ctx = nctx + 16;
    const uint8_t* ctx_slice = T.ctx_map + size_t(wg_sel) * nctx;
    for (uint32_t i = tid; i < n_ctx; i += 64) {
      const uint32_t cl = ctx_slice[i];
      l_ctx[i] = uint8_t(cl < nclusters ? cl : nclusters - 1);
    }
    if (PREFIX)
      for (uint32_t i = tid; i < nclusters; i += 64) {
        const uint32_t cfg = T.cfg[i];
        l_cfg[i] = uint16_t((cfg & 15) | (((cfg >> 8) & 15) << 4) | (((cfg >> 16) & 15) << 8));
      }
    if (PREFIX)
      for (uint32_t i = tid; i < nclusters; i += 64) l_poff[i] = T.prefix_offset[i];
    const uint32_t n_alias = (GALIAS || PREFIX) ? 0u : nclusters << log_alpha;
    if constexpr (A6) {
      LdsU16* const lb = (LdsU16*)(lds + kLanesA6B);
      LdsU32* const la = (LdsU32*)(lds + kLanesA6A);
      LdsU16* const lc = (LdsU16*)(lds + kLanesA6Cfg);
      for (uint32_t i = tid; i < n_alias; i += 64) {
        const uint2 e = galias[i];
        uint32_t cutoff = e.x >> 24, y = e.y & ((1u << (24 + log_alpha)) - 1);
        if (cutoff > entry_mask) {
          cutoff = entry_mask;
          y = (e.x & 0xFFFu) | (i & ((1u << log_alpha) - 1)) << 24;
        }
        const uint32_t lo_bits = 8 - log_alpha;
        lb[i] = uint16_t((e.x & 0xFFFu) | (cutoff >> lo_bits) << 12);
        la[i] = y | (cutoff & ((1u << lo_bits) - 1)) << (24 + log_alpha);
        if ((i & ((1u << log_alpha) - 1)) == 0) lc[i >> log_alpha] = uint16_t((e.x >> 12) & 0xFFFu);
      }
    } else {
      LdsU32x2* l_alias = (LdsU32x2*)(lds + L.alias);
      for (uint32_t i = tid; i < n_alias; i += 64) {
        const uint2 e = galias[i];
        l_alias[i] = LanesU32x2{e.x, e.y};
      }
    }
    if (tid < 64) l_nnz2[tid] = uint16_t(uint32_t(c_coeff_nnz_ctx[tid]) * 2);
    for (uint32_t b = tid; b < kLanesF2Bytes; b += 64)
      lds[L.f2 + b] = uint8_t(b < 64 ? uint32_t(c_coeff_freq_ctx[b]) * 2 : 2 * min(min(b - 1, 7 + (b >> 1)), 15 + (b >> 2)));
    LdsU32* z = (LdsU32*)(lds + wave_base);
    for (uint32_t i = lane; i < kLanesNzRows * 64 / 4; i += 64) z[i] = 0;
  }
  __syncthreads();

  enum : uint32_t { kWait = 0, kRun = 1, kFlush = 2, kDone = 3 };
  auto take_section = [&]() -> uint32_t {
    const uint32_t idx = atomicAdd(B.queue + unit, 1u);
    return idx < list_count ? B.list[list_begin + idx] : 0xFFFFFFFFu;
  };
  uint32_t g = lane < B.wave_lanes[wid] ? take_section() : 0xFFFFFFFFu;
  uint32_t mode = g == 0xFFFFFFFFu ? uint32_t(kDone) : uint32_t(kWait);
  uint32_t err = 0, ntok = 0;
  uint32_t b1 = 0, bi = 0, ci = 2;
  const uint32_t sec0 = pass * P.num_groups;
  const void* const kend_base = P.kend + size_t(pass) * P.kend_pass_stride;
  const void* const coef_base = static_cast<CoefT*>(P.coeffs) + P.coef_pass_base + size_t(pass) * P.coef_pass_stride;
  uint32_t sec_off = 0, nwords = 0, sec_size = 0, ring_end = 0, pend_s = 0, bring_end = 0, pend_b = 0, bitpos = 0, state = 0;
  LanesU32x4 stg = {0, 0, 0, 0}, btg = {0, 0, 0, 0};
  uint32_t stg_n = 0, btg_n = 0;
  bool started = false;
  uint32_t info = 0, lbx = 0, lby = 0, coef_offset = 0, next_offset = 0;
  auto open_section = [&]() {
    const uint32_t first = P.gbb[g];
    bi = first - 1;
    b1 = P.gbb[g + 1];
    bring_end = first;
    sec_off = P.sec_word[sec0 + g] * 4;
    sec_size = P.sec_size[sec0 + g];
    nwords = (sec_size + 3) / 4;
    bitpos = sec0 + g == 0 ? P.first_bit_offset : 0;
    ring_end = 0;
    pend_s = pend_b = 0;
    stg_n = btg_n = 0;
    next_offset = 0;
    ci = 2;
    err = 0;
    started = false;
  };
  if (mode == kWait) open_section();
  uint32_t nzeros = 0, k = 0, size = 0, log2c = 0, covm1 = 0, cbase = 0, addr_a = 0, nnz_b = 0, ctxe = 0, kidx = 0, covm2 = 0;
  const uint32_t ring_addr = uint32_t(uintptr_t(ring)), cl_mul = 1u << cl_shift, nnz2_addr = uint32_t(uintptr_t(l_nnz2));
  if (ASMT && uint32_t(uintptr_t(lds)) != 0) __builtin_trap();
  uint32_t acc_lo = 0, acc_hi = 0;
  uint32_t dst = 0;
  const uint32_t shift = T.shift;
  constexpr uint32_t kPerChunk = 8 / sizeof(CoefT);

  unsigned long long t_begin = 0, t_service = 0, n_service = 0, n_trips = 0, n_lane_trips = 0, t_wait = 0, t_dma = 0, t_trans = 0, n_calls = 0;
  if (B.prof) t_begin = __builtin_readcyclecounter();
  __builtin_amdgcn_s_waitcnt(0);
  auto dma_group4 = [&](bool in, uint32_t row_lds, const void* base, uint32_t off) {
    if (in) {
      uint32_t keep, tmp;
      asm volatile(
          "s_mov_b32 %0, m0\n\t"
          "s_mov_b32 m0, %3\n\ts_nop 0\n\tglobal_load_lds_dword %2, %4\n\t"
          "v_add_u32 %1, 4, %2\n\ts_add_u32 m0, m0, 0x100\n\ts_nop 0\n\tglobal_load_lds_dword %1, %4\n\t"
          "v_add_u32 %1, 8, %2\n\ts_add_u32 m0, m0, 0x100\n\ts_nop 0\n\tglobal_load_lds_dword %1, %4\n\t"
          "v_add_u32 %1, 12, %2\n\ts_add_u32 m0, m0, 0x100\n\ts_nop 0\n\tglobal_load_lds_dword %1, %4\n\t"
          "s_mov_b32 m0, %0"
          : "=&s"(keep), "=&v"(tmp)
          : "v"(off), "s"(row_lds), "s"(base)
          : "memory", "scc");
    }
  };
  uint32_t round = 0;
  for (;;) {
    {
      const bool low = (ring_end - (bitpos >> 5)) < 2 * kLanesTrips + 1;
      bool act = mode == kRun && !low;
      if constexpr (ASMT) {
        const unsigned long long actm = __ballot(act);
        if (actm) {
          unsigned long long th = 0;
          const uint32_t k_before = k;
          const uint32_t n_total = uint32_t(__popcll(actm)) + uint32_t(__popcll(__ballot(mode == kWait || mode == kFlush)));
          const uint32_t cont_min = __builtin_amdgcn_readfirstlane(((n_total << B.wait_shift) / (1u + (1u << B.wait_shift))) + 1u);
          uint32_t groups = 0;
          if (AIDS) {
            if (B.prof) th = __builtin_readcyclecounter();
            if constexpr (A6) {
              JXL_LANES_TRIP_LOOP6_COUNTED(groups, state, bitpos, k, nzeros, ctxe, addr_a, nnz_b, dst, acc_lo, acc_hi, log2c, cbase, covm2, ring_addr,
                                           ring_end, size, actm, cont_min, log_entry, entry_mask, cl_mul, nnz2_addr, shift, coef_base, log_alpha);
            } else {
              JXL_LANES_TRIP_LOOP_COUNTED(groups, state, bitpos, k, nzeros, ctxe, addr_a, nnz_b, dst, acc_lo, acc_hi, log2c, cbase, covm2, ring_addr,
                                          ring_end, size, actm, cont_min, log_entry, entry_mask, cl_mul, nnz2_addr, shift, coef_base, log_alpha);
            }
            if (B.prof) t_wait += __builtin_readcyclecounter() - th;
            n_trips += groups * kLanesTrips;
            n_calls++;
          } else {
            if constexpr (A6) {
              JXL_LANES_TRIP_LOOP6(groups, state, bitpos, k, nzeros, ctxe, addr_a, nnz_b, dst, acc_lo, acc_hi, log2c, cbase, covm2, ring_addr, ring_end,
                                   size, actm, cont_min, log_entry, entry_mask, cl_mul, nnz2_addr, shift, coef_base, log_alpha);
            } else {
              JXL_LANES_TRIP_LOOP(groups, state, bitpos, k, nzeros, ctxe, addr_a, nnz_b, dst, acc_lo, acc_hi, log2c, cbase, covm2, ring_addr, ring_end,
                                  size, actm, cont_min, log_entry, entry_mask, cl_mul, nnz2_addr, shift, coef_base, log_alpha);
            }
          }
          mode = (act && (nzeros == 0 || k >= size)) ? uint32_t(kFlush) : mode;
          if (AIDS && B.prof) n_lane_trips += act ? k - k_before : 0u;
          if (AIDS && (B.debug & 2)) ntok += act ? k - k_before : 0u;
        }
      } else
      if (__ballot(act)) {
        unsigned long long th = 0;
        if (B.prof) th = __builtin_readcyclecounter();
        if (AIDS) n_trips += kLanesTrips;
        uint32_t pw0 = 0, pw1 = 0, pw2 = 0, pe_zero = 0, pe_nonzero = 0, pnnz_c = 0;
        uint32_t ppo = 0, pcfg = 0, proot = 0;
        LanesU32x2 pe = {0, 0};
        auto request = [&]() {
          LdsU32* const rp = ring + ((bitpos >> 5) & (kLanesRingWords - 1)) * 64;
          if (PREFIX) {
            ppo = l_poff[ctxe & 255];
            pcfg = l_cfg[ctxe & 255];
          } else if (GALIAS) {
            if (act) {
              const uint2 ge = galias[(ctxe << log_alpha) + ((state & 0xFFFu) >> log_entry)];
              pe = LanesU32x2{ge.x, ge.y};
            }
          } else {
            pe = alias_entry(ctxe, (state & 0xFFFu) >> log_entry);
          }
          pw0 = rp[0];
          pw1 = rp[64];
          pw2 = rp[128];
          __builtin_amdgcn_sched_barrier(0);
          const uint32_t b = (k + 1) >> log2c;
          const uint32_t f2 = min(min(b - 1, 7 + (b >> 1)), 15 + (b >> 2)) << 1;
          pe_zero = l_ctx[(GALIAS || PREFIX) ? ((addr_a + f2) & 0x1FFF) : (addr_a + f2)];
          pe_nonzero = l_ctx[(GALIAS || PREFIX) ? ((cbase + 1 + nnz_b + f2) & 0x1FFF) : (cbase + 1 + nnz_b + f2)];
          pnnz_c = l_nnz2[((nzeros - 2 + covm1) >> log2c) & 63];
          if (PREFIX) {
            const uint32_t win = __builtin_amdgcn_alignbit(pw1, pw0, bitpos);
            proot = 0;
            if (act) proot = ptable[(ppo & 0xFFFFFFu) + (win & ((1u << (ppo >> 24)) - 1))];
          }
        };
        request();
#pragma unroll
        for (int rep = 0; rep < kLanesTrips; rep++) {
          if (AIDS && B.prof) n_lane_trips += act ? 1u : 0u;
          uint32_t w0, w1, w2, e_zero, e_nonzero, nnz_c;
          const uint32_t kn = k + 1;
          const uint32_t addr_b = cbase + 1 + nnz_b;
          uint32_t tok, cfg, adv, nstate = state;
          w0 = pw0, w1 = pw1, w2 = pw2, e_zero = pe_zero, e_nonzero = pe_nonzero, nnz_c = pnnz_c;
          if (PREFIX) {
            uint32_t e = proot;
            if (act && (e & 0x80u)) {
              const uint32_t win = __builtin_amdgcn_alignbit(w1, w0, bitpos);
              e = ptable[(ppo & 0xFFFFFFu) + (e >> 8) + ((win >> (ppo >> 24)) & ((1u << (e & 0x7Fu)) - 1))];
            }
            tok = e >> 8;
            adv = e & 0xFFu;
            cfg = pcfg;
          } else {
            const LanesU32x2 e = pe;
            const uint32_t res = state & 0xFFFu, slot = res >> log_entry, pos = res & entry_mask;
            const bool gt = pos >= (e.x >> 24);
            const uint32_t x = gt ? e.y : e.x;
            tok = gt ? (e.y >> 24) : slot;
            const uint32_t hi = state >> 12;
            nstate = (x & 0xFFFu) * hi + hi + (gt ? ((e.y >> 12) & 0xFFFu) : 0u) + pos;
            const bool need = nstate < (1u << 16);
            const uint32_t win = __builtin_amdgcn_alignbit(w1, w0, bitpos);
            nstate = need ? ((nstate << 16) | (win & 0xFFFFu)) : nstate;
            adv = need ? 16u : 0u;
            cfg = e.x >> 12;
          }
          const bool take = act && tok >= (1u << (cfg & 15));
          if (__ballot(take)) {
            uint32_t nbits;
            const uint32_t big = LaneHybrid(tok, cfg, w0, w1, w2, (bitpos & 31) + adv, nbits);
            tok = take ? big : tok;
            adv += take ? nbits : 0u;
          }
          const bool nz = tok != 0;
          const uint32_t n_nzeros = nzeros - (nz ? 1u : 0u);
          const bool done = n_nzeros == 0 || kn >= size;
          const bool full = act && (kn & (kPerChunk - 1)) == 0;
          const uint32_t acc_lo0 = acc_lo, acc_hi0 = acc_hi, dst0 = dst;
          state = act ? nstate : state;
          bitpos += act ? adv : 0u;
          k = act ? kn : k;
          nzeros = act ? n_nzeros : nzeros;
          ctxe = act ? (nz ? e_nonzero : e_zero) : ctxe;
          addr_a = (act && nz) ? addr_b - 1 : addr_a;
          nnz_b = (act && nz) ? nnz_c : nnz_b;
          if (rep + 1 < kLanesTrips) request();
          const uint32_t sgn = uint32_t(-int32_t(tok & 1));
          const int32_t coeff = int32_t(((tok >> 1) ^ sgn) << shift);
          uint32_t n_lo, n_hi;
          if (sizeof(CoefT) == 2) {
            n_lo = __builtin_amdgcn_alignbit(acc_hi0, acc_lo0, 16);
            n_hi = (acc_hi0 >> 16) | (uint32_t(coeff) << 16);
          } else {
            n_lo = acc_hi0;
            n_hi = uint32_t(coeff);
          }
          if ((B.debug & 1) == 0 && full) LaneStore64(coef_base, dst0, n_lo, n_hi);
          if (AIDS && (B.debug & 2)) ntok += act ? 1u : 0u;
          acc_lo = act ? n_lo : acc_lo0;
          acc_hi = act ? n_hi : acc_hi0;
          dst = dst0 + (full ? 8u : 0u);
          mode = (act && done) ? uint32_t(kFlush) : mode;
          act = act && !done;
        }
        if (B.prof) t_wait += __builtin_readcyclecounter() - th;
      }
    }
    {
      unsigned long long t2 = 0;
      if (B.prof) t2 = __builtin_readcyclecounter();
      const bool fl = mode == kFlush;
      const bool next_block = ci == 2 && started;
      const bool ran_out = fl && nzeros != 0;
      const bool rare = !started || (next_block && bi + 1 >= b1) || ran_out;
      const bool go = (mode == kWait || fl) && !rare && (ring_end - (bitpos >> 5)) >= 3 && (!next_block || bi + 1 < bring_end);
      const uint32_t n_go = uint32_t(__popcll(__ballot(fl || go))), n_run = uint32_t(__popcll(__ballot(mode == kRun)));
      if (n_go && (n_go << B.wait_shift) >= n_run) {
        if (ASMT) {
          if (fl) {
            const uint32_t part = (k - covm1 - 1) & 3;
            if (!(B.debug & 1)) {
              if (part >= 2) LaneStore32(coef_base, dst, acc_lo);
              if (part & 1) LaneStore16(coef_base, dst + (part & 2) * 2, part == 3 ? acc_hi : acc_lo);
            }
            if (!(B.debug & 4)) LaneStore32(kend_base, kidx * 4, k);
          }
        } else
        if (fl) {
          const uint32_t part = k & (kPerChunk - 1);
          const uint64_t v = ((uint64_t(acc_hi) << 32) | acc_lo) >> (((kPerChunk - part) & (kPerChunk - 1)) * (64 / kPerChunk));
          if (!(B.debug & 1) && part) LaneStore64(coef_base, dst, uint32_t(v), uint32_t(v >> 32));
          if (!(B.debug & 4)) LaneStore32(kend_base, kidx * 4, k);
        }
        err |= ran_out ? kErrNzeros : 0u;
        bi = ran_out ? b1 : bi;
        ci = ran_out ? 2u : ci;
        mode = fl ? uint32_t(kWait) : mode;
        if constexpr (ASMT) {
          if (go) {
            const bool nb = ci == 2;
            const uint32_t n_ci = nb ? 0u : ci + 1, n_bi = bi + (nb ? 1u : 0u);
            if (nb) {
              info = bring[(n_bi & (kLanesBlockRing - 1)) * 64];
              coef_offset = next_offset;
            }
            const uint32_t n_log2c = ((info >> 6) & 7) + ((info >> 9) & 7);
            if (nb) next_offset += 64u << n_log2c;
            const uint32_t c = n_ci == 0 ? 1u : (n_ci == 1 ? 0u : 2u);
            if ((info >> (24 + c)) & 1u) {
              if (!(B.debug & 4)) LaneStore32(kend_base, (n_bi * 3 + c) * 4, 0);
              bi = n_bi;
              ci = n_ci;
            } else {
            const uint32_t n_lbx = (info & 31) >> ((info >> (27 + c)) & 1u), n_lby = (info >> 5) & 1;
            const uint32_t log2cx = (info >> 6) & 7;
            const uint32_t bctx = (info >> (12 + 4 * c)) & 15;
            LdsU8* line = l_nz + (c * 32) * 64;
            const uint32_t top = line[n_lbx * 64], left = line[(n_lbx ? n_lbx - 1 : 0) * 64];
            const uint32_t l0 = n_lbx ? left : 32u, tt = n_lby ? top : l0, ll = n_lbx ? left : tt;
            const uint32_t pred = (tt + ll + 1) >> 1;
            uint32_t nzb = pred >= 64 ? 64 : pred;
            nzb = nzb < 8 ? nzb : 4 + nzb / 2;
            const uint32_t cluster = l_ctx[(nzb * num_bctx + bctx) & 0x1FFF];
            const uint32_t slotw = (bitpos >> 5) & (kLanesRingWords - 1);
            const uint32_t w0 = ring[slotw * 64], w1 = ring[slotw * 64 + 64], w2 = ring[slotw * 64 + 128];
            const uint32_t res = state & 0xFFFu, slot = res >> log_entry, pos = res & entry_mask;
            const LanesU32x2 e = alias_entry(cluster, slot);
            const bool gt = pos >= (e.x >> 24);
            const uint32_t x = gt ? e.y : e.x;
            uint32_t tok = gt ? (e.y >> 24) : slot;
            const uint32_t hi = state >> 12;
            uint32_t nstate = (x & 0xFFFu) * hi + hi + (gt ? ((e.y >> 12) & 0xFFFu) : 0u) + pos;
            const bool need = nstate < (1u << 16);
            const uint32_t win = __builtin_amdgcn_alignbit(w1, w0, bitpos);
            state = need ? ((nstate << 16) | (win & 0xFFFFu)) : nstate;
            uint32_t adv = need ? 16u : 0u;
            const uint32_t cfg = e.x >> 12;
            const bool take = tok >= (1u << (cfg & 15));
            if (__ballot(take)) {
              uint32_t nbits;
              const uint32_t big = LaneHybrid(tok, cfg, w0, w1, w2, (bitpos & 31) + adv, nbits);
              tok = take ? big : tok;
              adv += take ? nbits : 0u;
            }
            bitpos += adv;
            const uint32_t covered = 1u << n_log2c;
            log2c = n_log2c;
            size = covered * 64;
            kidx = n_bi * 3 + c;
            const bool bad = tok > size - covered;
            const uint8_t nzv = uint8_t((tok + covered - 1) >> n_log2c);
            if (!bad) {
              line[n_lbx * 64] = nzv;
              if (__ballot(log2cx != 0)) {
                const uint32_t cx = 1u << log2cx;
                for (uint32_t i = 1; i < cx; i++) line[(n_lbx + i) * 64] = nzv;
              }
            }
            if (tok == 0 && !(B.debug & 4)) LaneStore32(kend_base, kidx * 4, 0);
            covm1 = covered - 1;
            covm2 = covered - 3;
            const uint32_t n_cbase = num_bctx * 37 + 458 * bctx;
            const uint32_t prev = tok > size / 16 ? 0 : 1;
            const uint32_t n_addr_a = n_cbase + l_nnz2[((tok + covm1) >> n_log2c) & 63];
            nnz_b = l_nnz2[((tok - 1 + covm1) >> n_log2c) & 63];
            ctxe = l_ctx[(n_addr_a + prev) & 0x1FFF];
            cbase = n_cbase + L.ctx;
            addr_a = n_addr_a + L.ctx;
            dst = uint32_t(((g * 3 + c) * 65536 + coef_offset + covered) * sizeof(CoefT));
            nzeros = tok;
            k = covered;
            mode = (tok != 0 && !bad) ? uint32_t(kRun) : mode;
            err |= bad ? kErrNzeros : 0u;
            bi = bad ? b1 : n_bi;
            ci = bad ? 2u : n_ci;
            }
          }
        } else {
        const bool nb = ci == 2;
        const uint32_t n_ci = nb ? 0u : ci + 1, n_bi = bi + (nb ? 1u : 0u);
        const uint32_t rec = bring[(n_bi & (kLanesBlockRing - 1)) * 64];
        const uint32_t n_info = nb ? rec : info;
        const uint32_t n_log2c = ((n_info >> 6) & 7) + ((n_info >> 9) & 7);
        const uint32_t n_coef_offset = nb ? next_offset : coef_offset;
        const uint32_t c = n_ci == 0 ? 1u : (n_ci == 1 ? 0u : 2u);
        const bool absent = ((n_info >> (24 + c)) & 1u) != 0;
        const bool go_all = go;
        const bool go = go_all && !absent;
        const uint32_t n_lbx = (n_info & 31) >> ((n_info >> (27 + c)) & 1u), n_lby = (n_info >> 5) & 1;
        const uint32_t log2cx = (n_info >> 6) & 7;
        const uint32_t bctx = (n_info >> (12 + 4 * c)) & 15;
        LdsU8* line = l_nz + (c * 32) * 64;
        const uint32_t top = line[n_lbx * 64], left = line[(n_lbx ? n_lbx - 1 : 0) * 64];
        const uint32_t l0 = n_lbx ? left : 32u, tt = n_lby ? top : l0, ll = n_lbx ? left : tt;
        const uint32_t pred = (tt + ll + 1) >> 1;
        uint32_t nzb = pred >= 64 ? 64 : pred;
        nzb = nzb < 8 ? nzb : 4 + nzb / 2;
        const uint32_t cluster = l_ctx[(nzb * num_bctx + bctx) & 0x1FFF];
        const uint32_t slotw = (bitpos >> 5) & (kLanesRingWords - 1);
        const uint32_t w0 = ring[slotw * 64], w1 = ring[slotw * 64 + 64], w2 = ring[slotw * 64 + 128];
        uint32_t tok, cfg, adv, nstate = state;
        if (PREFIX) {
          const uint32_t po = l_poff[cluster];
          const uint32_t win = __builtin_amdgcn_alignbit(w1, w0, bitpos);
          uint32_t e = 0;
          if (go) e = PrefixLookup(ptable + (po & 0xFFFFFFu), po >> 24, win);
          tok = e >> 8;
          adv = e & 0xFFu;
          cfg = l_cfg[cluster];
        } else {
          const uint32_t res = state & 0xFFFu, slot = res >> log_entry, pos = res & entry_mask;
          LanesU32x2 e = {0, 0};
          if (GALIAS) {
            if (go) {
              const uint2 ge = galias[(cluster << log_alpha) + slot];
              e = LanesU32x2{ge.x, ge.y};
            }
          } else {
            e = alias_entry(cluster, slot);
          }
          const bool gt = pos >= (e.x >> 24);
          const uint32_t x = gt ? e.y : e.x;
          tok = gt ? (e.y >> 24) : slot;
          const uint32_t hi = state >> 12;
          nstate = (x & 0xFFFu) * hi + hi + (gt ? ((e.y >> 12) & 0xFFFu) : 0u) + pos;
          const bool need = nstate < (1u << 16);
          const uint32_t win = __builtin_amdgcn_alignbit(w1, w0, bitpos);
          nstate = need ? ((nstate << 16) | (win & 0xFFFFu)) : nstate;
          adv = need ? 16u : 0u;
          cfg = e.x >> 12;
        }
        const bool take = go && tok >= (1u << (cfg & 15));
        if (__ballot(take)) {
          uint32_t nbits;
          const uint32_t big = LaneHybrid(tok, cfg, w0, w1, w2, (bitpos & 31) + adv, nbits);
          tok = take ? big : tok;
          adv += take ? nbits : 0u;
        }
        const uint32_t covered = 1u << n_log2c, n_size = covered * 64;
        const uint32_t n_kidx = n_bi * 3 + c;
        const bool bad = tok > n_size - covered;
        const uint8_t nzv = uint8_t((tok + covered - 1) >> n_log2c);
        if (go && !bad) {
          line[n_lbx * 64] = nzv;
          if (__ballot(log2cx != 0)) {
            const uint32_t cx = 1u << log2cx;
            for (uint32_t i = 1; i < cx; i++) line[(n_lbx + i) * 64] = nzv;
          }
        }
        if (((go && tok == 0) || (go_all && absent)) && !(B.debug & 4)) LaneStore32(kend_base, n_kidx * 4, 0);
        const uint32_t n_covm1 = covered - 1;
        const uint32_t n_cbase = num_bctx * 37 + 458 * bctx;
        const uint32_t prev = tok > n_size / 16 ? 0 : 1;
        const uint32_t n_addr_a = n_cbase + l_nnz2[((tok + n_covm1) >> n_log2c) & 63];
        const uint32_t n_nnz_b = l_nnz2[((tok - 1 + n_covm1) >> n_log2c) & 63];
        const uint32_t n_ctxe = l_ctx[(n_addr_a + prev) & 0x1FFF];
        state = go ? nstate : state;
        bitpos += go ? adv : 0u;
        info = go_all ? n_info : info;
        coef_offset = go_all ? n_coef_offset : coef_offset;
        next_offset += (go_all && nb) ? (64u << n_log2c) : 0u;
        log2c = go ? n_log2c : log2c;
        size = go ? n_size : size;
        kidx = go ? n_kidx : kidx;
        nzeros = go ? tok : nzeros;
        k = go ? covered : k;
        covm1 = go ? n_covm1 : covm1;
        if (ASMT) {
          covm2 = go ? n_covm1 - 2 : covm2;
          cbase = go ? n_cbase + L.ctx : cbase;
          dst = go ? uint32_t(((g * 3 + c) * 65536 + n_coef_offset + covered) * sizeof(CoefT)) : dst;
          addr_a = go ? n_addr_a + L.ctx : addr_a;
        } else {
        cbase = go ? n_cbase : cbase;
        dst = go ? uint32_t(((g * 3 + c) * 65536 + n_coef_offset + (covered & ~(kPerChunk - 1))) * sizeof(CoefT)) : dst;
        acc_lo = go ? 0u : acc_lo;
        acc_hi = go ? 0u : acc_hi;
        addr_a = go ? n_addr_a : addr_a;
        }
        nnz_b = go ? n_nnz_b : nnz_b;
        ctxe = go ? n_ctxe : ctxe;
        mode = (go && tok != 0 && !bad) ? uint32_t(kRun) : mode;
        err |= (go && bad) ? kErrNzeros : 0u;
        bi = go_all ? ((go && bad) ? b1 : n_bi) : bi;
        ci = go_all ? ((go && bad) ? 2u : n_ci) : ci;
        }
        if (B.prof) {
          t_trans += __builtin_readcyclecounter() - t2;
          n_service++;
          t_dma += n_go;
        }
      }
    }
    if ((++round & B.refill_mask) != 0) continue;
    {
      unsigned long long t0 = 0;
      if (B.prof) t0 = __builtin_readcyclecounter();
      if (!__ballot(mode != kDone)) break;
      if constexpr (ASMT) {
        if (__ballot(stg_n | btg_n)) LaneLoadWait(stg, btg);
        if (__ballot(stg_n != 0)) {
          if (stg_n) {
            const bool zeros = stg_n == 8;
            const uint32_t s0 = zeros ? 0u : stg.x, s1 = zeros ? 0u : stg.y, s2 = zeros ? 0u : stg.z, s3 = zeros ? 0u : stg.w;
            LdsU32* const r4 = ring + (ring_end & (kLanesRingWords - 1)) * 64;
            r4[0] = s0;
            r4[64] = s1;
            r4[128] = s2;
            r4[192] = s3;
            if ((ring_end & (kLanesRingWords - 1)) == 0) {
              ring[16 * 64] = s0;
              ring[17 * 64] = s1;
            }
            ring_end += 4;
            stg_n = 0;
          }
        }
        if (__ballot(btg_n != 0)) {
          if (btg_n) {
            LdsU32* const r4 = bring + (bring_end & (kLanesBlockRing - 1) & ~3u) * 64;
            r4[0] = btg.x;
            r4[64] = btg.y;
            r4[128] = btg.z;
            r4[192] = btg.w;
            bring_end = (bring_end & ~3u) + 4;
            btg_n = 0;
          }
        }
      } else {
      LaneDmaWait();
      ring_end += pend_s;
      bring_end += pend_b;
      pend_s = pend_b = 0;
      }
      {
        const bool next_block = ci == 2 && started;
        const bool rare = mode == kWait && (ring_end - (bitpos >> 5)) >= 3 && (!started || (next_block && bi + 1 >= b1));
        if (__ballot(rare)) {
          if (rare) {
            if (!started) {
              started = true;
              uint32_t hb = 0;
              while ((1u << hb) < num_hist) hb++;
              const uint32_t w0 = ring[0], w1 = ring[64];
              const uint64_t win = ((uint64_t(w1) << 32) | w0) >> bitpos;
              const uint32_t sel = hb ? uint32_t(win) & ((1u << hb) - 1) : 0;
              if (sel != wg_sel) err = kErrSelector;
              state = PREFIX ? 0x13u << 16 : uint32_t(win >> hb);
              bitpos += hb + (PREFIX ? 0 : 32);
            } else {
              if (state != (0x13u << 16)) err |= kErrFinalState;
              if (bitpos > sec_size * 8) err |= kErrOverread;
              P.sec_end_bits[sec0 + g] = bitpos;
              if (P.num_passes > 1) atomicOr(P.errors + g, err);
              else P.errors[g] = (B.debug & 2) ? ntok : err;
              ntok = 0;
              g = take_section();
              if (g == 0xFFFFFFFFu) mode = kDone;
              else open_section();
            }
          }
          __builtin_amdgcn_s_waitcnt(0);
        }
      }
      if constexpr (ASMT) {
        const uint32_t used = ring_end - (bitpos >> 5);
        const bool want_s = mode != kDone && kLanesRingWords - used >= 4;
        const bool want_b = mode != kDone && bring_end < b1 && (bi + 1 + kLanesBlockRing - bring_end) >= 4;
        const unsigned long long ms = __ballot(want_s && ring_end < nwords), mb = __ballot(want_b);
        if (ms) LaneLoad128(stg, ms, P.sections, sec_off + ring_end * 4);
        if (mb) LaneLoad128(btg, mb, P.block_recs, (bring_end & ~3u) * 4);
        stg_n = want_s ? (ring_end < nwords ? 4u : 8u) : 0u;
        btg_n = want_b ? 4u : 0u;
      } else {
        const uint32_t used = ring_end - (bitpos >> 5);
        const uint32_t groups_s = mode == kDone ? 0u : (kLanesRingWords - used) >> 2;
        const uint32_t first_g = (ring_end >> 2) & 3;
        const uint32_t next_b = bi + 1;
        const uint32_t bfirst = (bring_end >> 2) & 1;
        uint32_t groups_b = 0;
        if (mode != kDone && bring_end < b1) groups_b = (next_b + kLanesBlockRing - bring_end) >> 2;
        if (__ballot(groups_s != 0)) {
#pragma unroll
          for (uint32_t gi = 0; gi < 4; gi++) {
            const uint32_t d = (gi - first_g) & 3;
            const bool in = d < groups_s;
            const uint32_t w = ring_end + d * 4;
            const bool beyond = w >= nwords;
            dma_group4(in && !beyond, lds_abs + ring_row0 + gi * 1024, P.sections, sec_off + w * 4);
            if (gi == 0) {
              if (in && !beyond) {
                LaneDmaDword(lds_abs + ring_row0 + 16 * 256, P.sections, sec_off + w * 4);
                LaneDmaDword(lds_abs + ring_row0 + 17 * 256, P.sections, sec_off + w * 4 + 4);
              }
            }
            if (__ballot(in && beyond)) {
              if (in && beyond) {
                for (uint32_t j = 0; j < 4; j++) ring[(gi * 4 + j) * 64] = 0;
                if (gi == 0) ring[16 * 64] = ring[17 * 64] = 0;
              }
            }
          }
          pend_s = groups_s * 4;
        }
        if (__ballot(groups_b != 0)) {
#pragma unroll
          for (uint32_t gi = 0; gi < 2; gi++) {
            const uint32_t d = (gi - bfirst) & 1;
            const bool in = d < groups_b;
            dma_group4(in, lds_abs + bring_row0 + gi * 1024, P.block_recs, ((bring_end & ~3u) + d * 4) * 4);
          }
          pend_b = groups_b * 4 - (groups_b ? (bring_end & 3) : 0);
        }
      }
      if (B.prof) t_service += __builtin_readcyclecounter() - t0;
    }
  }
  if (B.prof && lane == 0) {
    unsigned long long* o = B.prof + size_t(blockIdx.x) * 8;
    o[0] = __builtin_readcyclecounter() - t_begin;
    o[1] = t_service;
    o[2] = n_service;
    o[3] = n_trips;
    o[5] = t_wait;
    o[6] = t_dma;
    o[7] = t_trans;
    if (B.debug & 32) o[6] = n_calls;
    if (B.debug & 16) {
      uint32_t hw, xcc;
      asm volatile("s_getreg_b32 %0, hwreg(HW_REG_HW_ID)" : "=s"(hw));
      asm volatile("s_getreg_b32 %0, hwreg(HW_REG_XCC_ID)" : "=s"(xcc));
      o[6] = (unsigned long long)hw | ((unsigned long long)xcc << 32);
    }
  }
  if (B.prof) {
    unsigned long long total = n_lane_trips;
    for (int off = 32; off; off >>= 1) total += __shfl_down(total, off);
    if (lane == 0) B.prof[size_t(blockIdx.x) * 8 + 4] = total;
  }
}

}
#endif
```

libjxl_amd/csrc/hip/jxl_hip_filter_fused.h:

```cpp
#ifndef JXL_HIP_FILTER_FUSED_H_
#define JXL_HIP_FILTER_FUSED_H_

#include <type_traits>

#include "jxl_hip_color.h"
#include "jxl_hip_kernels.h"

namespace jxlhip {

struct FusedFilterParams {
  FilterParams f;
  float sm[3], bsm[3];
  float* filtered;
  uint32_t debug;
};

constexpr int kFusedTW = 64, kFusedTH = 16;
constexpr int kFusedThreads = 512;
constexpr int kFusedSigW = kFusedTW / 8 + 3, kFusedSigH = kFusedTH / 8 + 3;
__host__ __device__ constexpr int FusedHalo(bool gab, int epf) {
  return (gab ? 1 : 0) + (epf >= 3 ? 3 : 0) + (epf >= 1 ? 2 : 0) + (epf >= 2 ? 1 : 0);
}
__host__ __device__ constexpr size_t FusedLdsBytes(bool gab, int epf) {
  return (size_t(2) * 3 * (kFusedTW + 2 * FusedHalo(gab, epf)) * (kFusedTH + 2 * FusedHalo(gab, epf)) + kFusedSigW * kFusedSigH) *
// ... 35 lines not shown
          const int d = plus[k][0] * S + plus[k][1];
          s += fabsf(p[o + d] - p[n + d]);
        }
        sad = s * P.f.ch_scale[c] + sad;
      }
    }
    float weight = sad * inv_sig + 1.0f;
    weight = weight < 0.0f ? 0.0f : weight;
    w += weight;
    a0 = weight * src[n] + a0;
    a1 = weight * src[PL + n] + a1;
    a2 = weight * src[2 * PL + n] + a2;
  }
  const float inv_w = 1.0f / w;
  *out0 = a0 * inv_w;
  *out1 = a1 * inv_w;
  *out2 = a2 * inv_w;
}

template <int S, int PL, int HO, int H>
__device__ __forceinline__ void Epf1Stage(const FusedFilterParams& P, const float* src, float* dst, const float* l_sig, int x0,
                                          int y0, int xs, int ys, int tid) {
  const int sbx = (x0 >> 3) - 1, sby = (y0 >> 3) - 1;
  constexpr int TW = kFusedTW, TH = kFusedTH;
  {
    constexpr int w = TW + 2 * HO + 3, n = w * (TH + 2 * HO + 3), NITD = (n + kFusedThreads - 1) / kFusedThreads;
#pragma unroll 4
    for (int it = 0; it < NITD; it++) {
      const int i = tid + it * kFusedThreads;
      if (i >= n) break;
      const int ry = i / w, rx = i - ry * w;
      const int q = (ry + H - HO - 2) * S + rx + H - HO - 2;
      float dh = 0.0f, dv = 0.0f;
#pragma unroll
      for (int c = 0; c < 3; c++) {
        const float v = src[c * PL + q];
        dh = fabsf(v - src[c * PL + q + 1]) * P.f.ch_scale[c] + dh;
        dv = fabsf(v - src[c * PL + q + S]) * P.f.ch_scale[c] + dv;
      }
      dst[q] = dh;
      dst[PL + q] = dv;
    }
  }
  __syncthreads();
  constexpr int w = TW + 2 * HO, n = w * (TH + 2 * HO), NIT = (n + kFusedThreads - 1) / kFusedThreads;
  float out[NIT][3];
#pragma unroll
  for (int it = 0; it < NIT; it++) {
    const int i = tid + it * kFusedThreads;
    if (i < n) {
      const int ry = i / w, rx = i - ry * w;
      const int o = (ry + H - HO) * S + rx + H - HO;
      const int mx = MirrorI(x0 + rx - HO, xs), my = MirrorI(y0 + ry - HO, ys);
      const float is = l_sig[((my >> 3) - sby) * kFusedSigW + (mx >> 3) - sbx];
      const float c0 = src[o], c1 = src[PL + o], c2 = src[2 * PL + o];
      if (is < -3.90524291751269967465540850526868f) {
        out[it][0] = c0;
        out[it][1] = c1;
        out[it][2] = c2;
      } else {
        const bool border = ((mx & 7) == 0) || ((mx & 7) == 7) || ((my & 7) == 0) || ((my & 7) == 7);
        const float inv_sig = is * (border ? P.bsm[1] : P.sm[1]);
        const float* dh = dst;
        const float* dv = dst + PL;
        const int nb[4] = {o - S, o - 1, o + 1, o + S};
        const float sad[4] = {
            (dv[o - S] + dv[o - 2 * S]) + (dv[o - S - 1] + dv[o]) + dv[o - S + 1],
            (dh[o - 1] + dh[o - S - 1]) + (dh[o - 2] + dh[o + S - 1]) + dh[o],
            (dh[o] + dh[o - S]) + (dh[o - 1] + dh[o + S]) + dh[o + 1],
            (dv[o] + dv[o - S]) + (dv[o - 1] + dv[o + S]) + dv[o + 1]};
        float wsum = 1.0f, a0 = c0, a1 = c1, a2 = c2;
#pragma unroll
        for (int j = 0; j < 4; j++) {
          float weight = sad[j] * inv_sig + 1.0f;
          weight = weight < 0.0f ? 0.0f : weight;
          wsum += weight;
          a0 = weight * src[nb[j]] + a0;
          a1 = weight * src[PL + nb[j]] + a1;
          a2 = weight * src[2 * PL + nb[j]] + a2;
        }
        const float inv_w = __builtin_amdgcn_rcpf(wsum);
        out[it][0] = a0 * inv_w;
        out[it][1] = a1 * inv_w;
        out[it][2] = a2 * inv_w;
      }
    }
  }
  __syncthreads();
#pragma unroll
  for (int it = 0; it < NIT; it++) {
    const int i = tid + it * kFusedThreads;
    if (i < n) {
      const int ry = i / w, rx = i - ry * w;
      const int o = (ry + H - HO) * S + rx + H - HO;
      dst[o] = out[it][0];
      dst[PL + o] = out[it][1];
      dst[2 * PL + o] = out[it][2];
    }
  }
  __syncthreads();
}

struct UpsampleParams {
  FilterParams f;
  const float* kernel;
  uint32_t n, oxs, oys;
  PixelOut po;
  float* xyb_out;
  uint32_t oxp;
  JxlHipColorTarget t;
};

__device__ __forceinline__ void XybToRgb(const FilterParams& f, float X, float Y, float Bc, float* r, float* g, float* b) {
  if (f.linear_output >= 2) {
    if (f.linear_output == 2) {
      const float y = Y + 128.0f / 255;
      *r = fmaf(1.402f, Bc, y);
      *g = fmaf(-0.299f * 1.402f / 0.587f, Bc, fmaf(-0.114f * 1.772f / 0.587f, X, y));
      *b = fmaf(1.772f, X, y);
    } else {
      *r = X;
      *g = Y;
      *b = Bc;
    }
    return;
  }
  const float gr = (Y + X) - f.opsin_bias_cbrt[0], gg = (Y - X) - f.opsin_bias_cbrt[1], gb = Bc - f.opsin_bias_cbrt[2];
  const float mr = (gr * gr) * gr + f.opsin_bias[0], mg = (gg * gg) * gg + f.opsin_bias[1], mb = (gb * gb) * gb + f.opsin_bias[2];
  *r = f.opsin_inv[2] * mb + (f.opsin_inv[1] * mg + f.opsin_inv[0] * mr);
  *g = f.opsin_inv[5] * mb + (f.opsin_inv[4] * mg + f.opsin_inv[3] * mr);
  *b = f.opsin_inv[8] * mb + (f.opsin_inv[7] * mg + f.opsin_inv[6] * mr);
  if (!f.linear_output) {
    *r = LinearToSrgb(*r);
    *g = LinearToSrgb(*g);
    *b = LinearToSrgb(*b);
  }
}

struct ColorOutParams {
  FilterParams f;
  PixelOut po;
  JxlHipColorTarget t;
};
__global__ __launch_bounds__(256) void k_color_out(ColorOutParams P) {
  const int x = blockIdx.x * 64 + (threadIdx.x & 63), y = int(P.f.y_begin) + blockIdx.y * 4 + (threadIdx.x >> 6);
  if (x >= int(P.f.xs) || y >= int(P.f.y_end)) return;
  const size_t plane = size_t(P.f.xp) * P.f.yp, gi = size_t(y) * P.f.xp + x;
  float r, g, b;
  XybToRgb(P.f, P.f.in[gi], P.f.in[plane + gi], P.f.in[2 * plane + gi], &r, &g, &b);
  if (P.t.tf) ApplyColorTarget(P.t, &r, &g, &b);
  StorePixel(P.po, x, y, r, g, b);
}

__global__ __launch_bounds__(256) void k_upsample_color(UpsampleParams P) {
  const int x = blockIdx.x * 64 + (threadIdx.x & 63), y = blockIdx.y * 4 + (threadIdx.x >> 6);
  const int xs = int(P.f.xs), ys = int(P.f.ys);
  if (x >= xs || y >= ys) return;
  const size_t plane = size_t(P.f.xp) * P.f.yp;
  float v[3][25], mn[3], mx[3];
#pragma unroll
  for (int iy = 0; iy < 5; iy++) {
    const size_t row = size_t(MirrorI(y + iy - 2, ys)) * P.f.xp;
#pragma unroll
    for (int ix = 0; ix < 5; ix++) {
      const size_t g = row + MirrorI(x + ix - 2, xs);
#pragma unroll
      for (int c = 0; c < 3; c++) {
        const float t = P.f.in[c * plane + g];
        v[c][iy * 5 + ix] = t;
        mn[c] = (iy | ix) == 0 ? t : fminf(mn[c], t);
        mx[c] = (iy | ix) == 0 ? t : fmaxf(mx[c], t);
      }
    }
  }
  const int N = int(P.n);
  for (int oy = 0; oy < N; oy++) {
    const int Y = y * N + oy;
    if (Y >= int(P.oys)) break;
    for (int ox = 0; ox < N; ox++) {
      const int X = x * N + ox;
      if (X >= int(P.oxs)) break;
      const float* k = P.kernel + (N * oy + ox) * 25;
      float ch[3];
#pragma unroll
      for (int c = 0; c < 3; c++) {
        float a0 = v[c][0] * k[0], a1 = v[c][1] * k[1], a2 = v[c][2] * k[2];
#pragma unroll
        for (int i = 3; i < 24; i += 3) {
          a0 = fmaf(v[c][i], k[i], a0);
          a1 = fmaf(v[c][i + 1], k[i + 1], a1);
          a2 = fmaf(v[c][i + 2], k[i + 2], a2);
        }
        a0 = fmaf(v[c][24], k[24], a0);
        const float r = (a1 + a2) + a0;
        ch[c] = r < mn[c] ? mn[c] : (r > mx[c] ? mx[c] : r);
      }
      const float Xc = ch[0], Yc = ch[1], Bc = ch[2];
      if (P.xyb_out) {
        const size_t oplane = size_t(P.oxp) * P.oys, gi = size_t(Y) * P.oxp + X;
        P.xyb_out[gi] = Xc;
        P.xyb_out[oplane + gi] = Yc;
        P.xyb_out[2 * oplane + gi] = Bc;
        continue;
      }
      float r, g, b;
      XybToRgb(P.f, Xc, Yc, Bc, &r, &g, &b);
      if (P.t.tf) ApplyColorTarget(P.t, &r, &g, &b);
      if (P.po.dst) {
        StorePixel(P.po, X, Y, r, g, b);
        continue;
      }
      uint8_t* dst = P.f.rgb + (size_t(Y) * P.oxs + X) * 3;
      dst[0] = ToU8(r, X, Y, 0);
      dst[1] = ToU8(g, X, Y, 1);
      dst[2] = ToU8(b, X, Y, 2);
    }
  }
}

struct UpsamplePlaneParams {
  const float* in;
  float* out;
  const float* kernel;
  uint32_t xs, ys, n, oxs, oys;
};
__global__ __launch_bounds__(256) void k_upsample_plane(UpsamplePlaneParams P) {
  const int x = blockIdx.x * 64 + (threadIdx.x & 63), y = blockIdx.y * 4 + (threadIdx.x >> 6);
  const int xs = int(P.xs), ys = int(P.ys);
  if (x >= xs || y >= ys) return;
  float v[25], mn = 0.0f, mx = 0.0f;
#pragma unroll
  for (int iy = 0; iy < 5; iy++) {
    const size_t row = size_t(MirrorI(y + iy - 2, ys)) * P.xs;
#pragma unroll
    for (int ix = 0; ix < 5; ix++) {
      const float t = P.in[row + MirrorI(x + ix - 2, xs)];
      v[iy * 5 + ix] = t;
      mn = (iy | ix) == 0 ? t : fminf(mn, t);
      mx = (iy | ix) == 0 ? t : fmaxf(mx, t);
    }
  }
  const int N = int(P.n);
  for (int oy = 0; oy < N; oy++) {
    const int Y = y * N + oy;
    if (Y >= int(P.oys)) break;
    for (int ox = 0; ox < N; ox++) {
      const int X = x * N + ox;
      if (X >= int(P.oxs)) break;
      const float* k = P.kernel + (N * oy + ox) * 25;
      float a0 = v[0] * k[0], a1 = v[1] * k[1], a2 = v[2] * k[2];
#pragma unroll
      for (int i = 3; i < 24; i += 3) {
        a0 = fmaf(v[i], k[i], a0);
        a1 = fmaf(v[i + 1], k[i + 1], a1);
        a2 = fmaf(v[i + 2], k[i + 2], a2);
      }
      a0 = fmaf(v[24], k[24], a0);
      const float r = (a1 + a2) + a0;
      P.out[size_t(Y) * P.oxs + X] = r < mn ? mn : (r > mx ? mx : r);
    }
  }
}

constexpr int kRowsHalo = 3;
constexpr int kRowsStrip = 64;
constexpr int kRowsWaves = 4;

__device__ __forceinline__ float FromLeft(float v) {
  return __builtin_bit_cast(float, __builtin_amdgcn_update_dpp(0, __builtin_bit_cast(int, v), 0x138, 0xF, 0xF, true));
}
__device__ __forceinline__ float FromRight(float v) {
  return __builtin_bit_cast(float, __builtin_amdgcn_update_dpp(0, __builtin_bit_cast(int, v), 0x130, 0xF, 0xF, true));
}
__device__ __forceinline__ float FmacFromLeft(float acc, float v, float w) {
  asm("v_fmac_f32_dpp %0, %1, %2 wave_shr:1 row_mask:0xf bank_mask:0xf bound_ctrl:1" : "+v"(acc) : "v"(v), "v"(w));
  return acc;
}
__device__ __forceinline__ float FmacFromRight(float acc, float v, float w) {
  asm("v_fmac_f32_dpp %0, %1, %2 wave_shl:1 row_mask:0xf bank_mask:0xf bound_ctrl:1" : "+v"(acc) : "v"(v), "v"(w));
  return acc;
}

typedef float f2 __attribute__((ext_vector_type(2)));
constexpr int kRows2Cols = 120;
__device__ __forceinline__ f2 LeftOf(f2 v) { return f2{FromLeft(v.y), v.x}; }
__device__ __forceinline__ f2 RightOf(f2 v) { return f2{v.y, FromRight(v.x)}; }
__device__ __forceinline__ f2 Abs2(f2 v) { return __builtin_elementwise_abs(v); }
__device__ __forceinline__ f2 LinearToSrgb2(f2 v) {
  const f2 a = Abs2(v);
  const f2 s = f2{__builtin_amdgcn_sqrtf(a.x), __builtin_amdgcn_sqrtf(a.y)};
  f2 yp = 7.352629620e-01f * s + 1.474205315e+00f;
  yp = yp * s + 3.903842876e-01f;
  yp = yp * s + 5.287254571e-03f;
  yp = yp * s + -5.135152395e-04f;
  f2 yq = 2.424867759e-02f * s + 9.258482155e-01f;
  yq = yq * s + 1.340816930e+00f;
  yq = yq * s + 3.036675394e-01f;
  yq = yq * s + 1.004519624e-02f;
  const f2 hi = yp * f2{__builtin_amdgcn_rcpf(yq.x), __builtin_amdgcn_rcpf(yq.y)};
  const f2 lo = a * 12.92f;
  return f2{copysignf(a.x > 0.0031308f ? hi.x : lo.x, v.x), copysignf(a.y > 0.0031308f ? hi.y : lo.y, v.y)};
}

__device__ __forceinline__ f2 LinearToSrgb2ForU8(f2 v) {
  const f2 p = f2{__builtin_amdgcn_exp2f(__builtin_amdgcn_logf(v.x) * (1.0f / 2.4f)), __builtin_amdgcn_exp2f(__builtin_amdgcn_logf(v.y) * (1.0f / 2.4f))};
  const f2 hi = p * 1.055f - 0.055f;
  const f2 lo = v * 12.92f;
  return f2{v.x > 0.0031308f ? hi.x : lo.x, v.y > 0.0031308f ? hi.y : lo.y};
}

struct P2 {
  float x, y;
};
__device__ __forceinline__ P2 operator+(P2 a, P2 b) { return P2{a.x + b.x, a.y + b.y}; }
__device__ __forceinline__ P2 operator-(P2 a, P2 b) { return P2{a.x - b.x, a.y - b.y}; }
__device__ __forceinline__ P2 operator*(P2 a, P2 b) { return P2{a.x * b.x, a.y * b.y}; }
__device__ __forceinline__ P2 operator+(P2 a, float b) { return P2{a.x + b, a.y + b}; }
__device__ __forceinline__ P2 operator-(P2 a, float b) { return P2{a.x - b, a.y - b}; }
__device__ __forceinline__ P2 operator*(P2 a, float b) { return P2{a.x * b, a.y * b}; }
__device__ __forceinline__ P2 operator*(float b, P2 a) { return P2{b * a.x, b * a.y}; }
__device__ __forceinline__ P2 Max0(P2 a) { return P2{__builtin_fmaxf(a.x, 0.0f), __builtin_fmaxf(a.y, 0.0f)}; }
__device__ __forceinline__ P2 Srgb2(P2 v) {
  const f2 r = LinearToSrgb2(f2{v.x, v.y});
  return P2{r.x, r.y};
}
__device__ __forceinline__ P2 Srgb2ForU8(P2 v) {
  const f2 r = LinearToSrgb2ForU8(f2{v.x, v.y});
  return P2{r.x, r.y};
}
__device__ __forceinline__ __amdgpu_buffer_rsrc_t RawBuffer(const void* p) {
  return __builtin_amdgcn_make_buffer_rsrc(const_cast<void*>(p), 0, 0xFFFFFFFFu, 0x00020000);
}
template <int AUX = 0>
__device__ __forceinline__ float BufF32(__amdgpu_buffer_rsrc_t r, uint32_t voff, uint32_t soff) {
  return __builtin_bit_cast(float, __builtin_amdgcn_raw_buffer_load_b32(r, voff, soff, AUX));
}
template <int AUX = 0>
__device__ __forceinline__ P2 BufP2(__amdgpu_buffer_rsrc_t r, uint32_t voff, uint32_t soff) {
  typedef unsigned int u2 __attribute__((ext_vector_type(2)));
  const u2 v = __builtin_amdgcn_raw_buffer_load_b64(r, voff, soff, AUX);
  const f2 f = __builtin_bit_cast(f2, v);
  return P2{f.x, f.y};
}

template <bool U8SRGB, int EPF = 1, bool GAB = true, bool GREY = false>
__global__ __launch_bounds__(64 * kRowsWaves) void k_filter_rows2(const FusedFilterParams* params, int strip_rows) {
  static_assert(EPF == 1 || EPF == 2, "(Gaborish +) one or two EPF iterations");
  static_assert(U8SRGB || !GREY, "the one-channel writer exists for 8-bit sRGB only");
  constexpr int HALO = kRowsHalo + (EPF == 2 ? 1 : 0);
  FusedFilterParams P;
  LoadParams(P, params + blockIdx.z);
  const int lane = threadIdx.x & 63, wave = threadIdx.x >> 6;
  const int xs = int(P.f.xs), ys = int(P.f.ys);
  const int xw0 = (int(blockIdx.x) * kRowsWaves + wave) * kRows2Cols;
  const int y0 = int(P.f.y_begin) + int(blockIdx.y) * strip_rows;
  const int y1 = y0 + strip_rows < int(P.f.y_end) ? y0 + strip_rows : int(P.f.y_end);
  if (xw0 >= xs || y0 >= y1) return;
  const int x = xw0 - 4 + 2 * lane;
  const int mx0 = MirrorI(x, xs), mx1 = MirrorI(x + 1, xs);
  const bool emit_lane = lane >= 2 && lane < 62;
  const bool emit0 = emit_lane && x < xs, emit1 = emit_lane && x + 1 < xs;
  const bool xb0 = ((mx0 & 7) == 0) || ((mx0 & 7) == 7), xb1 = ((mx1 & 7) == 0) || ((mx1 & 7) == 7);
  const size_t gplane = size_t(P.f.xp) * P.f.yp;
  typedef float __attribute__((address_space(1)))* GF32W;
  typedef f2 __attribute__((address_space(1)))* GF32x2W;
  const bool paired = __all(x >= 0 && x + 1 < xs) && (P.f.xp & 1) == 0;
  const uint32_t vo0 = uint32_t(mx0) * 4u, vo1 = uint32_t(mx1) * 4u;
  const uint32_t vsig = uint32_t(mx0 >> 3) * 4u;
  const uint32_t vout = uint32_t(x) * (GREY ? 1u : 3u);
  const uint32_t vd0 = uint32_t(x & 31) * 4u;
  const uint32_t vd1a = uint32_t((x + 23) & 31) * 4u, vd1b = uint32_t((x + 24) & 31) * 4u;
  const uint32_t vd2 = uint32_t((x + 46) & 31) * 4u;
  const __amdgpu_buffer_rsrc_t in_buf = RawBuffer(P.f.in), sig_buf = RawBuffer(P.f.inv_sigma);
  const __amdgpu_buffer_rsrc_t dither_buf = RawBuffer(c_dither), rgb_buf = RawBuffer(P.f.rgb);
  const uint32_t plane_bytes = uint32_t(gplane * 4);
  const GF32W filtered = U8SRGB ? nullptr : (GF32W)(uintptr_t)P.filtered;
  const bool has_rgb = U8SRGB || P.f.rgb != nullptr;
  const GF32W rgbf = U8SRGB ? nullptr : (GF32W)(uintptr_t)P.f.rgbf;
  const bool linear_output = U8SRGB ? false : P.f.linear_output != 0;
  const P2 zero2 = P2{0.0f, 0.0f};
  P2 p[3][4], h1[3][4], g[3][4], dh[4], dv[4];
  P2 e[3][4];
  float is_prev = 0.0f;
  P2 pv_prev = zero2, dh_new = zero2;
#pragma unroll
  for (int c = 0; c < 3; c++) {
#pragma unroll
    for (int k = 0; k < 4; k++) p[c][k] = h1[c][k] = g[c][k] = e[c][k] = zero2;
  }
#pragma unroll
  for (int k = 0; k < 4; k++) dh[k] = dv[k] = zero2;
  const int steps = (y1 - y0 + 2 * HALO + 3) / 4 * 4;
  int ym = MirrorI(y0 - HALO, ys), ydir;
  {
    const int ym_next = MirrorI(y0 - HALO + 1, ys);
    ydir = ym_next > ym ? 1 : (ym_next < ym ? -1 : (ym == 0 ? -1 : 1));
  }
  constexpr int kPlaneAux = 0;
  auto load_row = [&](P2 (&dst)[3]) {
    const uint32_t row = uint32_t(ym) * uint32_t(P.f.xp) * 4u;
    if (paired) {
#pragma unroll
      for (int c = 0; c < 3; c++) dst[c] = BufP2<kPlaneAux>(in_buf, vo0, row + c * plane_bytes);
    } else {
#pragma unroll
      for (int c = 0; c < 3; c++) dst[c] = P2{BufF32<kPlaneAux>(in_buf, vo0, row + c * plane_bytes), BufF32<kPlaneAux>(in_buf, vo1, row + c * plane_bytes)};
    }
    int nxt = ym + ydir;
    if (nxt < 0) {
      nxt = 0;
      ydir = 1;
    } else if (nxt >= ys) {
      nxt = ys - 1;
      ydir = -1;
    }
    ym = nxt;
  };
  auto load_aux = [&](int rs, int r, float& is, P2 (&di)[3]) {
    const int rc = rs < 0 ? 0 : (rs >= ys ? ys - 1 : rs);
    is = BufF32(sig_buf, vsig, uint32_t(rc >> 3) * uint32_t(P.f.xb) * 4u);
    if (!has_rgb) return;
    di[0] = BufP2(dither_buf, vd0, uint32_t(r & 31) * 128u);
    if constexpr (GREY) return;
    di[1] = P2{BufF32(dither_buf, vd1a, uint32_t((r + 13) & 31) * 128u), BufF32(dither_buf, vd1b, uint32_t((r + 13) & 31) * 128u)};
    di[2] = BufP2(dither_buf, vd2, uint32_t((r + 26) & 31) * 128u);
  };
  P2 nx[3], ndi[3] = {zero2, zero2, zero2};
  float nis = 0.0f;
  load_row(nx);
  load_aux(y0 - 2 * HALO + (EPF == 2 ? 1 : 0), y0 - 2 * HALO, nis, ndi);
  auto step = [&](auto phase, int j) {
    constexpr int PH = decltype(phase)::value;
    constexpr int N = PH % 4, M1 = (PH + 3) % 4, M2 = (PH + 2) % 4, M3 = (PH + 1) % 4;
    const P2 cur[3] = {nx[0], nx[1], nx[2]};
    const float is = nis;
    const P2 di[3] = {ndi[0], ndi[1], ndi[2]};
    const int r = y0 - 2 * HALO + j;
    const int r1 = EPF == 2 ? r + 1 : r;
    load_row(nx);
    load_aux(r1 + 1, r + 1, nis, ndi);
#pragma unroll
    for (int c = 0; c < 3; c++) {
      p[c][N] = cur[c];
      if constexpr (GAB) h1[c][N] = P2{FromLeft(cur[c].y) + cur[c].y, cur[c].x + FromRight(cur[c].x)};
    }
#pragma unroll
    for (int c = 0; c < 3; c++) {
      const P2 m = p[c][M1];
      if constexpr (GAB) {
        const P2 s1 = h1[c][M1] + (p[c][M2] + p[c][N]);
        const P2 s2 = h1[c][M2] + h1[c][N];
        g[c][N] = s2 * P.f.gab_w[c * 3 + 2] + (s1 * P.f.gab_w[c * 3 + 1] + m * P.f.gab_w[c * 3]);
      } else {
        g[c][N] = m;
      }
    }
    dh[N] = dh_new;
    {
      P2 a = zero2, b = zero2;
#pragma unroll
      for (int c = 0; c < 3; c++) {
        const P2 gn = g[c][N], gm = g[c][M1];
        a.x = __builtin_fabsf(gn.x - gn.y) * P.f.ch_scale[c] + a.x;
        a.y = __builtin_fabsf(FromRight(gn.x) - gn.y) * P.f.ch_scale[c] + a.y;
        b.x = __builtin_fabsf(gm.x - gn.x) * P.f.ch_scale[c] + b.x;
        b.y = __builtin_fabsf(gm.y - gn.y) * P.f.ch_scale[c] + b.y;
      }
      dh_new = a;
      dv[N] = b;
    }
    auto plus_sum = [&](const P2 (&d)[4]) {
      const P2 t = d[M1] + d[M2];
      const P2 u = P2{FromLeft(d[M1].y) + d[N].x, d[M1].x + d[N].y};
      const P2 w = t + u;
      return P2{w.x + d[M1].y, w.y + FromRight(d[M1].x)};
    };
    const P2 pv = plus_sum(dv);
    const P2 ph = plus_sum(dh);
    if (EPF == 2 ? (j >= 2 * HALO - 2 && r1 <= y1) : (j >= 2 * HALO && r < y1)) {
      P2 o[3] = {g[0][M2], g[1][M2], g[2][M2]};
      {
        const float is_k = is < -3.90524291751269967465540850526868f ? -__builtin_inff() : is;
        const int rm1 = EPF == 2 ? (r1 < 0 ? -1 - r1 : (r1 >= ys ? 2 * ys - 1 - r1 : r1)) : r;
        const bool yb = ((rm1 & 7) == 0) || ((rm1 & 7) == 7);
        const P2 inv_sig = P2{is_k * ((xb0 || yb) ? P.bsm[1] : P.sm[1]), is_k * ((xb1 || yb) ? P.bsm[1] : P.sm[1])};
        P2 wk[4];
        wk[0] = pv_prev * inv_sig + 1.0f;
        wk[1] = P2{FromLeft(ph.y) * inv_sig.x + 1.0f, ph.x * inv_sig.y + 1.0f};
        wk[2] = ph * inv_sig + 1.0f;
        wk[3] = pv * inv_sig + 1.0f;
        P2 wsum = P2{1.0f, 1.0f};
#pragma unroll
        for (int k = 0; k < 4; k++) {
          wk[k] = Max0(wk[k]);
          wsum = wsum + wk[k];
        }
        const P2 inv_w = P2{__builtin_amdgcn_rcpf(wsum.x), __builtin_amdgcn_rcpf(wsum.y)};
#pragma unroll
        for (int c = 0; c < 3; c++) {
          const P2 oc = o[c];
          P2 a = wk[0] * g[c][M3] + oc;
          a.x = FmacFromLeft(a.x, oc.y, wk[1].x);
          a.y = wk[1].y * oc.x + a.y;
          a.x = wk[2].x * oc.y + a.x;
          a.y = FmacFromRight(a.y, oc.x, wk[2].y);
          a = wk[3] * g[c][M1] + a;
          o[c] = a * inv_w;
        }
      }
      if constexpr (EPF == 2) {
#pragma unroll
        for (int c = 0; c < 3; c++) e[c][N] = o[c];
      }
     if (EPF == 1 || (j >= 2 * HALO && r < y1)) {
      if constexpr (EPF == 2) {
        const float is2 = is_prev;
        const bool keep2 = is2 < -3.90524291751269967465540850526868f;
        const bool yb2 = ((r & 7) == 0) || ((r & 7) == 7);
        const P2 inv_sig2 = P2{is2 * ((xb0 || yb2) ? P.bsm[2] : P.sm[2]), is2 * ((xb1 || yb2) ? P.bsm[2] : P.sm[2])};
        P2 nb[4][3];
#pragma unroll
        for (int c = 0; c < 3; c++) {
          const P2 cc = e[c][M1];
          nb[0][c] = e[c][M2];
          nb[1][c] = P2{FromLeft(cc.y), cc.x};
          nb[2][c] = P2{cc.y, FromRight(cc.x)};
          nb[3][c] = e[c][N];
        }
        P2 wsum = P2{1.0f, 1.0f};
        P2 acc[3] = {e[0][M1], e[1][M1], e[2][M1]};
#pragma unroll
        for (int k = 0; k < 4; k++) {
          P2 sad = zero2;
#pragma unroll
          for (int c = 0; c < 3; c++) {
            sad.x = __builtin_fabsf(nb[k][c].x - e[c][M1].x) * P.f.ch_scale[c] + sad.x;
            sad.y = __builtin_fabsf(nb[k][c].y - e[c][M1].y) * P.f.ch_scale[c] + sad.y;
          }
          const P2 wk2 = Max0(sad * inv_sig2 + 1.0f);
          wsum = wsum + wk2;
#pragma unroll
          for (int c = 0; c < 3; c++) acc[c] = wk2 * nb[k][c] + acc[c];
        }
        const P2 inv_w2 = P2{__builtin_amdgcn_rcpf(wsum.x), __builtin_amdgcn_rcpf(wsum.y)};
#pragma unroll
        for (int c = 0; c < 3; c++) o[c] = P2{keep2 ? e[c][M1].x : acc[c].x * inv_w2.x, keep2 ? e[c][M1].y : acc[c].y * inv_w2.y};
      }
      if (U8SRGB || emit0) {
        if (!U8SRGB && filtered) {
          const size_t gi = size_t(r) * P.f.xp + x;
#pragma unroll
          for (int c = 0; c < 3; c++) {
            filtered[c * gplane + gi] = o[c].x;
            if (emit1) filtered[c * gplane + gi + 1] = o[c].y;
          }
        }
        if (has_rgb || rgbf) {
          const P2 X = o[0], Y = o[1], Bc = o[2];
          const P2 gr = (Y + X) - P.f.opsin_bias_cbrt[0], gg = (Y - X) - P.f.opsin_bias_cbrt[1], gb = Bc - P.f.opsin_bias_cbrt[2];
          const P2 mr = (gr * gr) * gr + P.f.opsin_bias[0], mg = (gg * gg) * gg + P.f.opsin_bias[1], mb = (gb * gb) * gb + P.f.opsin_bias[2];
          P2 cr = P.f.opsin_inv[2] * mb + (P.f.opsin_inv[1] * mg + P.f.opsin_inv[0] * mr);
          if constexpr (GREY) {
            cr = Srgb2ForU8(cr);
            const bool even = ((r & xs) & 1) == 0;
            uint32_t w = __builtin_amdgcn_cvt_pk_u8_f32(cr.x * 255.0f + di[0].x, 0, 0u);
            w = __builtin_amdgcn_cvt_pk_u8_f32(cr.y * 255.0f + di[0].y, 1, w);
            const uint32_t orow = uint32_t(r) * uint32_t(xs);
            asm volatile("" : "+v"(w));
            if (!emit0) {
            } else if (even && emit1) {
              __builtin_amdgcn_raw_buffer_store_b16(uint16_t(w), rgb_buf, vout, orow, 0);
            } else {
              __builtin_amdgcn_raw_buffer_store_b8(uint8_t(w), rgb_buf, vout, orow, 0);
              if (emit1) __builtin_amdgcn_raw_buffer_store_b8(uint8_t(w >> 8), rgb_buf, vout + 1, orow, 0);
            }
          } else {
          P2 cg = P.f.opsin_inv[5] * mb + (P.f.opsin_inv[4] * mg + P.f.opsin_inv[3] * mr);
          P2 cb = P.f.opsin_inv[8] * mb + (P.f.opsin_inv[7] * mg + P.f.opsin_inv[6] * mr);
          const bool even = ((r & xs) & 1) == 0;
          if (!U8SRGB && rgbf) {
            if (!linear_output) {
              cr = Srgb2(cr);
              cg = Srgb2(cg);
              cb = Srgb2(cb);
            }
            const GF32W d = rgbf + (size_t(r) * xs + x) * 3;
            if (emit1 && even) {
              *(GF32x2W)(d) = f2{cr.x, cg.x};
              *(GF32x2W)(d + 2) = f2{cb.x, cr.y};
              *(GF32x2W)(d + 4) = f2{cg.y, cb.y};
            } else {
              d[0] = cr.x;
              d[1] = cg.x;
              d[2] = cb.x;
              if (emit1) {
                d[3] = cr.y;
                d[4] = cg.y;
                d[5] = cb.y;
              }
            }
          } else {
            if (!linear_output) {
              cr = Srgb2ForU8(cr);
              cg = Srgb2ForU8(cg);
              cb = Srgb2ForU8(cb);
            }
            uint32_t w01 = __builtin_amdgcn_cvt_pk_u8_f32(cr.x * 255.0f + di[0].x, 0, 0u);
            w01 = __builtin_amdgcn_cvt_pk_u8_f32(cg.x * 255.0f + di[1].x, 1, w01);
            w01 = __builtin_amdgcn_cvt_pk_u8_f32(cb.x * 255.0f + di[2].x, 2, w01);
            w01 = __builtin_amdgcn_cvt_pk_u8_f32(cr.y * 255.0f + di[0].y, 3, w01);
            uint32_t w2 = __builtin_amdgcn_cvt_pk_u8_f32(cg.y * 255.0f + di[1].y, 0, 0u);
            w2 = __builtin_amdgcn_cvt_pk_u8_f32(cb.y * 255.0f + di[2].y, 1, w2);
            const uint32_t orow = uint32_t(r) * uint32_t(xs) * 3u;
            constexpr int kRgbAux = 0;
            if constexpr (U8SRGB) asm volatile("" : "+v"(w01), "+v"(w2));
            if (U8SRGB && !emit0) {
            } else if (even) {
              __builtin_amdgcn_raw_buffer_store_b16(uint16_t(w01), rgb_buf, vout, orow, kRgbAux);
              if (emit1) {
                __builtin_amdgcn_raw_buffer_store_b16(uint16_t(w01 >> 16), rgb_buf, vout + 2, orow, kRgbAux);
                __builtin_amdgcn_raw_buffer_store_b16(uint16_t(w2), rgb_buf, vout + 4, orow, kRgbAux);
              } else {
                __builtin_amdgcn_raw_buffer_store_b8(uint8_t(w01 >> 16), rgb_buf, vout + 2, orow, 0);
              }
            } else {
              __builtin_amdgcn_raw_buffer_store_b8(uint8_t(w01), rgb_buf, vout, orow, 0);
              __builtin_amdgcn_raw_buffer_store_b8(uint8_t(w01 >> 8), rgb_buf, vout + 1, orow, 0);
              __builtin_amdgcn_raw_buffer_store_b8(uint8_t(w01 >> 16), rgb_buf, vout + 2, orow, 0);
              if (emit1) {
                __builtin_amdgcn_raw_buffer_store_b8(uint8_t(w01 >> 24), rgb_buf, vout + 3, orow, 0);
                __builtin_amdgcn_raw_buffer_store_b8(uint8_t(w2), rgb_buf, vout + 4, orow, 0);
                __builtin_amdgcn_raw_buffer_store_b8(uint8_t(w2 >> 8), rgb_buf, vout + 5, orow, 0);
              }
            }
          }
          }
        }
      }
     }
    }
    if constexpr (EPF == 2) is_prev = is;
    pv_prev = pv;
  };
  for (int j = 0; j < steps; j += 4) {
    step(std::integral_constant<int, 0>{}, j);
    step(std::integral_constant<int, 1>{}, j + 1);
    step(std::integral_constant<int, 2>{}, j + 2);
    step(std::integral_constant<int, 3>{}, j + 3);
  }
}

template <bool GAB, int EPF>
__global__ __launch_bounds__(kFusedThreads) void k_filter_fused(const FusedFilterParams* params) {
  static_assert(EPF == 0 || EPF == 3, "1 or 2 EPF iterations: k_filter_rows2");
  FusedFilterParams P;
  LoadParams(P, params + blockIdx.z);
  constexpr int H = FusedHalo(GAB, EPF);
  constexpr int TW = kFusedTW, TH = kFusedTH, S = TW + 2 * H, SH = TH + 2 * H, PL = S * SH;
  extern __shared__ __align__(16) float lds_ff[];
  float* src = lds_ff;
  float* dst = lds_ff + 3 * PL;
  float* l_sig = lds_ff + 6 * PL;
  const int tid = threadIdx.x;
  const int x0 = blockIdx.x * TW, y0 = int(P.f.y_begin) + blockIdx.y * TH;
  const int xs = int(P.f.xs), ys = int(P.f.ys);
  if (x0 >= xs || y0 >= int(P.f.y_end)) return;
  const size_t gplane = size_t(P.f.xp) * P.f.yp;
  const int sbx = (x0 >> 3) - 1, sby = (y0 >> 3) - 1;
  if (EPF > 0 && tid < kFusedSigW * kFusedSigH) {
    int bx = sbx + tid % kFusedSigW, by = sby + tid / kFusedSigW;
    bx = bx < 0 ? 0 : (bx >= int(P.f.xb) ? int(P.f.xb) - 1 : bx);
    by = by < 0 ? 0 : (by >= int((P.f.ys + 7) / 8) ? int((P.f.ys + 7) / 8) - 1 : by);
    l_sig[tid] = P.f.inv_sigma[size_t(by) * P.f.xb + bx];
  }
  {
    constexpr int NLD = (PL + kFusedThreads - 1) / kFusedThreads;
    float v[NLD][3];
    const bool interior = x0 >= H && y0 >= H && x0 + TW + H <= xs && y0 + TH + H <= ys;
#pragma unroll
    for (int it = 0; it < NLD; it++) {
      const int i = tid + it * kFusedThreads;
      if (i < PL) {
        const int ly = i / S, lx = i - ly * S;
        const size_t g = interior ? size_t(y0 + ly - H) * P.f.xp + (x0 + lx - H)
                                  : size_t(MirrorI(y0 + ly - H, ys)) * P.f.xp + MirrorI(x0 + lx - H, xs);
        v[it][0] = P.f.in[g];
        v[it][1] = P.f.in[gplane + g];
        v[it][2] = P.f.in[2 * gplane + g];
      }
    }
#pragma unroll
    for (int it = 0; it < NLD; it++) {
      const int i = tid + it * kFusedThreads;
      if (i < PL) {
        src[i] = v[it][0];
        src[PL + i] = v[it][1];
        src[2 * PL + i] = v[it][2];
      }
    }
  }
  __syncthreads();
  int h = H;
  if (GAB && !(P.debug & 1)) {
    h -= 1;
    constexpr int HG = H - 1, w = TW + 2 * HG, n = w * (TH + 2 * HG), NIT = (n + kFusedThreads - 1) / kFusedThreads;
#pragma unroll 4
    for (int it = 0; it < NIT; it++) {
      const int i = tid + it * kFusedThreads;
      if (i >= n) break;
      const int ry = i / w, rx = i - ry * w;
      const int o = (ry + H - HG) * S + rx + H - HG;
#pragma unroll
      for (int c = 0; c < 3; c++) {
        const float* p = src + c * PL;
        const float m = p[o];
        const float s1 = (p[o - 1] + p[o + 1]) + (p[o - S] + p[o + S]);
        const float s2 = (p[o - S - 1] + p[o - S + 1]) + (p[o + S - 1] + p[o + S + 1]);
        dst[c * PL + o] = s2 * P.f.gab_w[c * 3 + 2] + (s1 * P.f.gab_w[c * 3 + 1] + m * P.f.gab_w[c * 3]);
      }
    }
    __syncthreads();
    float* t = src;
    src = dst;
    dst = t;
  }
#define JXL_EPF_STAGE(STAGE_, RADIUS_)                                                                       \
  {                                                                                                          \
    h -= RADIUS_;                                                                                            \
    const int w = TW + 2 * h, n = w * (TH + 2 * h);                                                          \
    for (int i = tid; i < n; i += kFusedThreads) {                                                                     \
      const int ry = i / w, rx = i - ry * w;                                                                 \
      const int o = (ry + H - h) * S + rx + H - h;                                                           \
      const int mx = MirrorI(x0 + rx - h, xs), my = MirrorI(y0 + ry - h, ys);                                \
      const float is = l_sig[((my >> 3) - sby) * kFusedSigW + (mx >> 3) - sbx];                              \
      const bool border = ((mx & 7) == 0) || ((mx & 7) == 7) || ((my & 7) == 0) || ((my & 7) == 7);          \
      EpfPixel<STAGE_, S, PL>(P, src, o, is, border, &dst[o], &dst[PL + o], &dst[2 * PL + o]);               \
    }                                                                                                        \
    __syncthreads();                                                                                         \
    float* t = src;                                                                                          \
    src = dst;                                                                                               \
    dst = t;                                                                                                 \
  }
  if (EPF >= 3) JXL_EPF_STAGE(0, 3)
  if (EPF >= 1 && !(P.debug & 2)) {
    constexpr int HO = H - (GAB ? 1 : 0) - (EPF >= 3 ? 3 : 0) - 2;
    Epf1Stage<S, PL, HO, H>(P, src, dst, l_sig, x0, y0, xs, ys, tid);
    h = HO;
    float* t = src;
    src = dst;
    dst = t;
  }
  if (EPF >= 2) JXL_EPF_STAGE(2, 1)
#undef JXL_EPF_STAGE
  uint8_t* bytes = reinterpret_cast<uint8_t*>(dst);
#pragma unroll 2
  for (int i = tid; i < TW * TH; i += kFusedThreads) {
    const int ry = i / TW, rx = i - ry * TW;
    const int o = (ry + H) * S + rx + H;
    const int x = x0 + rx, y = y0 + ry;
    const float X = src[o], Y = src[PL + o], Bc = src[2 * PL + o];
    if (P.filtered && x < xs && y < ys) {
      const size_t g = size_t(y) * P.f.xp + x;
      P.filtered[g] = X;
      P.filtered[gplane + g] = Y;
      P.filtered[2 * gplane + g] = Bc;
    }
    const float gr = (Y + X) - P.f.opsin_bias_cbrt[0], gg = (Y - X) - P.f.opsin_bias_cbrt[1], gb = Bc - P.f.opsin_bias_cbrt[2];
    const float mr = (gr * gr) * gr + P.f.opsin_bias[0], mg = (gg * gg) * gg + P.f.opsin_bias[1], mb = (gb * gb) * gb + P.f.opsin_bias[2];
    float r = P.f.opsin_inv[2] * mb + (P.f.opsin_inv[1] * mg + P.f.opsin_inv[0] * mr);
    float g = P.f.opsin_inv[5] * mb + (P.f.opsin_inv[4] * mg + P.f.opsin_inv[3] * mr);
    float b = P.f.opsin_inv[8] * mb + (P.f.opsin_inv[7] * mg + P.f.opsin_inv[6] * mr);
    if (!P.f.linear_output && !(P.debug & 4)) {
      r = LinearToSrgb(r);
      g = LinearToSrgb(g);
      b = LinearToSrgb(b);
    }
    bytes[i * 3] = ToU8(r, x, y, 0);
    bytes[i * 3 + 1] = ToU8(g, x, y, 1);
    bytes[i * 3 + 2] = ToU8(b, x, y, 2);
  }
  __syncthreads();
  if (!P.f.rgb) return;
  const int cols = xs - x0 < TW ? xs - x0 : TW;
  const int rows = int(P.f.y_end) - y0 < TH ? int(P.f.y_end) - y0 : TH;
  const int row_bytes = cols * 3;
  if (((size_t(xs) * 3) & 3) == 0) {
    const int dw = row_bytes >> 2;
    const uint32_t* b32 = reinterpret_cast<const uint32_t*>(bytes);
    for (int i = tid; i < rows * (TW * 3 / 4); i += kFusedThreads) {
      const int ry = i / (TW * 3 / 4), j = i - ry * (TW * 3 / 4);
      if (j < dw) reinterpret_cast<uint32_t*>(P.f.rgb + (size_t(y0 + ry) * xs + x0) * 3)[j] = b32[i];
    }
    for (int i = tid; i < rows * 4; i += kFusedThreads) {
      const int ry = i >> 2, j = (dw << 2) + (i & 3);
      if (j < row_bytes) P.f.rgb[(size_t(y0 + ry) * xs + x0) * 3 + j] = bytes[ry * TW * 3 + j];
    }
  } else {
    for (int i = tid; i < rows * TW * 3; i += kFusedThreads) {
      const int ry = i / (TW * 3), j = i - ry * (TW * 3);
      if (j < row_bytes) P.f.rgb[(size_t(y0 + ry) * xs + x0) * 3 + j] = bytes[i];
    }
  }
}

struct NoiseParams {
  float* raw;
  float* planes;
  uint32_t xsize, ysize, xp, yp, xgroups, ngroups;
  uint32_t seed[2];
  float lut[8];
  float ytox, ytob;
  uint32_t y_begin, y_end;
};
__device__ __forceinline__ uint64_t NoiseSplitMix64(uint64_t z) {
  z = (z ^ (z >> 30)) * 0xBF58476D1CE4E5B9ull;
  z = (z ^ (z >> 27)) * 0x94D049BB133111EBull;
  return z ^ (z >> 31);
}
__global__ __launch_bounds__(64) void k_noise_random(NoiseParams P) {
  const uint32_t t = blockIdx.x * 64 + threadIdx.x;
  const uint32_t g = t >> 3, lane = t & 7;
  if (g >= P.ngroups) return;
  const uint32_t x0 = (g % P.xgroups) * 256, y0 = (g / P.xgroups) * 256;
  uint64_t s0 = NoiseSplitMix64(((uint64_t(P.seed[0]) << 32) + P.seed[1]) + 0x9E3779B97F4A7C15ull);
  uint64_t s1 = NoiseSplitMix64(((uint64_t(x0) << 32) + y0) + 0x9E3779B97F4A7C15ull);
  for (uint32_t i = 0; i < lane; i++) {
    s0 = NoiseSplitMix64(s0);
    s1 = NoiseSplitMix64(s1);
  }
  const uint32_t w = min(256u, P.xsize - x0), h = min(256u, P.ysize - y0);
  const uint32_t steps = (w > 16 ? (w - 16 + 15) / 16 : 0) + 1;
  for (uint32_t c = 0; c < 3; c++)
    for (uint32_t y = 0; y < h; y++) {
      float* row = P.raw + (size_t(c) * P.ysize + y0 + y) * P.xsize + x0;
      for (uint32_t b = 0; b < steps; b++) {
        uint64_t a = s0;
        const uint64_t bb = s1;
        const uint64_t bits = a + bb;
        s0 = bb;
        a ^= a << 23;
        a ^= bb ^ (a >> 18) ^ (bb >> 5);
        s1 = a;
// ... 185 lines not shown
```

libjxl_amd/csrc/hip/jxl_hip_lanes_trip.inc:

```
#ifndef JXL_HIP_LANES_TRIP_INC_
#define JXL_HIP_LANES_TRIP_INC_

#ifndef LT_WAITCNT
#define LT_WAITCNT(N) "s_waitcnt lgkmcnt(" N ")\n\t"
#endif
#ifndef LT_STORE
#define LT_STORE "global_store_dwordx2 %[dst], " LT_A ", %[coef]\n\t"
#endif
#define LT_E0 "v100"
#define LT_E1 "v101"
#define LT_E "v[100:101]"
#define LT_W0 "v102"
#define LT_W1 "v103"
#define LT_W "v[102:103]"
#define LT_EZ "v104"
#define LT_ENZ "v105"
#define LT_NC "v106"
#define LT_RA "v107"
#define LT_F0 "v108"
#define LT_F1 "v109"
#define LT_F2 "v110"
#define LT_F3 "v111"
#define LT_RS "v112"
#define LT_SL "v113"
#define LT_T0 "v114"
#define LT_T1 "v115"
#define LT_T2 "v116"
#define LT_T3 "v117"
#define LT_T4 "v118"
#define LT_T5 "v119"
#define LT_T6 "v120"
#define LT_T7 "v121"
#define LT_T8 "v122"
#define LT_T9 "v123"
#define LT_TA "v124"
#define LT_TB "v125"
#define LT_TC "v126"
#define LT_TD "v127"
#define LT_TCD "v[126:127]"
#define LT_W2 "v128"
#define LT_CF "v129"
#define LT_A0 "v130"
#define LT_A1 "v131"
#define LT_A "v[130:131]"

#define LT_HEAD_8                                                                                                    \
  "v_lshrrev_b32 " LT_T0 ", 24, " LT_E0 "\n\t"                                                           \
  "v_lshrrev_b32 " LT_T2 ", 24, " LT_E1 "\n\t"
#define LT_HEAD_6                                                                                                    \
  "v_lshrrev_b32 " LT_T0 ", 12, " LT_E0 "\n\t"                                                                       \
  "v_lshrrev_b32 " LT_T9 ", %[a6s2], " LT_E1 "\n\t"                                                                  \
  "v_bfe_u32 " LT_T2 ", " LT_E1 ", 24, %[a6la]\n\t"                                            \
  "v_lshl_or_b32 " LT_T0 ", " LT_T0 ", %[a6s1], " LT_T9 "\n\t"
#define LT_SPLIT_8 "v_bfe_u32 " LT_T7 ", " LT_E0 ", 12, 4\n\t"
#define LT_SPLIT_6 "v_and_b32 " LT_T7 ", 15, " LT_CF "\n\t"
#define LT_MSB_8 "v_bfe_u32 " LT_T8 ", " LT_E0 ", 16, 4\n\t"
#define LT_MSB_6 "v_bfe_u32 " LT_T8 ", " LT_CF ", 4, 4\n\t"
#define LT_LSB_8 "v_bfe_u32 " LT_T9 ", " LT_E0 ", 20, 4\n\t"
#define LT_LSB_6 "v_bfe_u32 " LT_T9 ", " LT_CF ", 8, 4\n\t"
#define LT_SLOTSH_8 "3"
#define LT_SLOTSH_6 "1"
#define LT_EREAD_8 "ds_read_b64 " LT_E ", " LT_T4 " offset:128\n\t"
#define LT_EREAD_6                                                                                                   \
  "v_lshlrev_b32 " LT_TA ", 1, " LT_T4 "\n\t"                                                                        \
  "ds_read_u16 " LT_E0 ", " LT_T4 " offset:128\n\t"                                                                  \
  "v_lshlrev_b32 " LT_TB ", 1, %[ctxe]\n\t"                                                                          \
  "ds_read_b32 " LT_E1 ", " LT_TA " offset:16512\n\t"                                                                \
  "ds_read_u16 " LT_CF ", " LT_TB " offset:49280\n\t"
#define LT_PENDING_8 "3"
#define LT_PENDING_6 "5"

#define LT_TRIP(V, J, FPRE, WAIT, MID, WF, F, PACK, TAIL)                                                                  \
  "v_and_b32 " LT_T1 ", %[em], " LT_RS "\n\t"                                                               \
  "v_lshrrev_b32 " LT_T3 ", 12, %[st]\n\t"                                                          \
  FPRE                                                                                                               \
  WAIT                                                                                                               \
  LT_HEAD_##V                                                                                                        \
  "v_bfe_u32 " LT_T5 ", " LT_E1 ", 12, 12\n\t"                                                         \
  "v_cmp_lt_u32 vcc, " LT_T1 ", " LT_T0 "\n\t"                               \
  LT_SPLIT_##V                                                                    \
  "v_cndmask_b32 " LT_T4 ", " LT_E1 ", " LT_E0 ", vcc\n\t"                                                           \
  "v_cndmask_b32 " LT_T2 ", " LT_T2 ", " LT_SL ", vcc\n\t"                                            \
  "v_cndmask_b32_e64 " LT_T5 ", " LT_T5 ", 0, vcc\n\t"                                                               \
  "v_and_b32 " LT_T4 ", 0xfff, " LT_T4 "\n\t"                                                          \
  "v_lshrrev_b32 " LT_T8 ", " LT_T7 ", " LT_T2 "\n\t"                                   \
  "v_mad_u32_u24 " LT_T4 ", " LT_T4 ", " LT_T3 ", " LT_T3 "\n\t"                                                     \
  "v_cmp_ne_u32_e64 s[98:99], 0, " LT_T8 "\n\t"                                          \
  "v_add3_u32 " LT_T4 ", " LT_T4 ", " LT_T5 ", " LT_T1 "\n\t"                  \
  "v_alignbit_b32 " LT_T5 ", " LT_W1 ", " LT_W0 ", %[bp]\n\t"                                                        \
  "v_cmp_gt_u32 vcc, %[c64k], " LT_T4 "\n\t"                                          \
  "v_perm_b32 " LT_T5 ", " LT_T4 ", " LT_T5 ", %[perm]\n\t"                                                          \
  "v_cndmask_b32 %[st], " LT_T4 ", " LT_T5 ", vcc\n\t"                                            \
  "v_cndmask_b32_e64 " LT_T6 ", 0, 16, vcc\n\t"                                                                      \
  "v_cmp_ne_u32 vcc, 0, " LT_T2 "\n\t"                                             \
  "v_and_b32 " LT_RS ", 0xfff, %[st]\n\t"                                                                            \
  "v_cndmask_b32 %[ctxe], " LT_EZ ", " LT_ENZ ", vcc\n\t"                              \
  "v_lshrrev_b32 " LT_SL ", %[le], " LT_RS "\n\t"                                                                    \
  "v_add_u32 " LT_T9 ", %[cb], %[nb]\n\t"                                                                            \
  "v_lshlrev_b32 " LT_T4 ", " LT_SLOTSH_##V ", " LT_SL "\n\t"                                                        \
  "v_cndmask_b32 %[aa], %[aa], " LT_T9 ", vcc\n\t"                                                                   \
  "v_mad_u32_u24 " LT_T4 ", %[ctxe], %[clm], " LT_T4 "\n\t"                                                          \
  "v_cndmask_b32 %[nb], %[nb], " LT_NC ", vcc\n\t"                                                                   \
  "v_subbrev_co_u32 %[nzl], vcc, 0, %[nzl], vcc\n\t"                                                                 \
  "s_cmp_lg_u64 s[98:99], 0\n\t"                                                                                     \
  "s_cbranch_scc0 .Llt_skip" J "_%=\n\t"                                                                             \
                                       \
  "s_and_saveexec_b64 s[100:101], s[98:99]\n\t"                                                                      \
  LT_MSB_##V                                                                                       \
  LT_LSB_##V                                                                                       \
  "v_alignbit_b32 " LT_TC ", " LT_W1 ", " LT_W0 ", %[bp]\n\t"                \
  "v_alignbit_b32 " LT_TD ", " LT_W2 ", " LT_W1 ", %[bp]\n\t"                                                        \
  "v_lshl_add_u32 " LT_TB ", -1, " LT_T7 ", " LT_T2 "\n\t"                                 \
  "v_add_u32 " LT_TA ", " LT_T8 ", " LT_T9 "\n\t"                                                                    \
  "v_lshrrev_b64 " LT_TCD ", " LT_T6 ", " LT_TCD "\n\t"                      \
  "v_lshrrev_b32 " LT_TB ", " LT_TA ", " LT_TB "\n\t"                                                                \
  "v_sub_u32 " LT_TA ", " LT_T7 ", " LT_TA "\n\t"                                                                    \
  "v_add_u32 " LT_TB ", " LT_TA ", " LT_TB "\n\t"                             \
  "v_bfe_u32 " LT_TA ", " LT_T2 ", " LT_T9 ", " LT_T8 "\n\t"                  \
  "v_bfe_u32 " LT_TC ", " LT_TC ", 0, " LT_TB "\n\t"                                             \
  "v_and_b32 " LT_TD ", 31, " LT_TB "\n\t"                                                                           \
  "v_lshl_or_b32 " LT_TA ", 1, " LT_T8 ", " LT_TA "\n\t"                                       \
  "v_add_u32 " LT_T6 ", " LT_T6 ", " LT_TD "\n\t"                                                 \
  "v_lshl_or_b32 " LT_TA ", " LT_TA ", " LT_TB ", " LT_TC "\n\t"                      \
  "v_bfe_u32 " LT_TC ", " LT_T2 ", 0, " LT_T9 "\n\t"                                   \
  "v_lshl_or_b32 " LT_T2 ", " LT_TA ", " LT_T9 ", " LT_TC "\n\t"                                      \
  "s_mov_b64 exec, s[100:101]\n"                                                                                     \
  ".Llt_skip" J "_%=:\n\t"                                                                                           \
   \
                                                      \
  LT_EREAD_##V                                                                                                       \
  "v_add_u32 %[bp], %[bp], " LT_T6 "\n\t"                                                                            \
  "v_cmp_ne_u32 vcc, 0, %[nzl]\n\t"                                                                                  \
  "v_bfe_u32 " LT_RA ", %[bp], 5, 4\n\t"                                                                             \
  "v_add_u32 %[k], 1, %[k]\n\t"                                                                                      \
  "v_lshl_add_u32 " LT_RA ", " LT_RA ", 8, %[ring]\n\t"                                                              \
  MID                                                                                                                \
  "ds_read2_b32 " LT_W ", " LT_RA " offset1:64\n\t"                                                                  \
  "ds_read_b32 " LT_W2 ", " LT_RA " offset:512\n\t"                                                                  \
                                                        \
  WF                                                                                                                 \
  "v_add_u32 " LT_T5 ", %[aa], " F "\n\t"                                                                            \
  "v_add3_u32 " LT_T7 ", %[cb], %[nb], " F "\n\t"                                                                    \
  "v_add_u32 " LT_T8 ", %[nzl], %[covm2]\n\t"                                                                        \
  "ds_read_u8 " LT_EZ ", " LT_T5 "\n\t"                                                                              \
  "v_bfe_u32 " LT_T8 ", " LT_T8 ", %[log2c], 6\n\t"                                                                  \
  "ds_read_u8 " LT_ENZ ", " LT_T7 " offset:1\n\t"                                                                    \
  "v_lshl_add_u32 " LT_T8 ", " LT_T8 ", 1, %[nnz2]\n\t"                                                              \
  "ds_read_u16 " LT_NC ", " LT_T8 "\n\t"                                                                             \
                                                                                           \
  "v_bfe_i32 " LT_T8 ", " LT_T2 ", 0, 1\n\t"                                                \
  "v_lshrrev_b32 " LT_T9 ", 1, " LT_T2 "\n\t"                                                                        \
  "v_xor_b32 " LT_T8 ", " LT_T9 ", " LT_T8 "\n\t"                                                                    \
  PACK                                                                                                               \
  TAIL

#define LT_GROUP_MASKS                                            \
  "v_lshrrev_b32 " LT_T0 ", 5, %[bp]\n\t"                         \
  "v_cmp_lt_u32_e64 s[98:99], %[k], %[size]\n\t"                  \
  "v_sub_u32 " LT_T0 ", %[rend], " LT_T0 "\n\t"                   \
  "v_cmp_lt_u32_e64 s[100:101], 8, " LT_T0 "\n\t"

#define LT_LIVE                                     \
  "s_and_b64 exec, exec, vcc\n\t"                   \
  "s_cbranch_execz .Llt_end_%=\n\t"

#define LT_FREAD(D0, D1, D2, D3)                                 \
  "v_add_u32 " LT_T0 ", " D0 ", %[k]\n\t"                        \
  "v_add_u32 " LT_TA ", " D1 ", %[k]\n\t"                        \
  "v_add_u32 " LT_TB ", " D2 ", %[k]\n\t"                        \
  "v_add_u32 " LT_TC ", " D3 ", %[k]\n\t"                        \
  "v_lshrrev_b32 " LT_T0 ", %[log2c], " LT_T0 "\n\t"             \
  "v_lshrrev_b32 " LT_TA ", %[log2c], " LT_TA "\n\t"             \
  "v_lshrrev_b32 " LT_TB ", %[log2c], " LT_TB "\n\t"             \
  "v_lshrrev_b32 " LT_TC ", %[log2c], " LT_TC "\n\t"             \
  "ds_read_u8 " LT_F0 ", " LT_T0 "\n\t"                          \
  "ds_read_u8 " LT_F1 ", " LT_TA "\n\t"                          \
  "ds_read_u8 " LT_F2 ", " LT_TB "\n\t"                          \
  "ds_read_u8 " LT_F3 ", " LT_TC "\n\t"

#define JXL_LANES_TRIP_LOOP_(V, LT_COUNT, p_grp, p_st, p_bp, p_k, p_nzl, p_ctxe, p_aa, p_nb, p_dst, p_alo, p_ahi, p_log2c, p_cb, p_covm2, p_ring, p_rend, p_size, p_act,     \
                            p_cont, p_le, p_em, p_clm, p_nnz2, p_shift, p_coef, p_la)                                                                        \
  asm volatile(                                                                                                                                          \
      "s_mov_b64 s[96:97], exec\n\t"                                                                                                                     \
      "s_mov_b64 exec, %[act]\n\t"                                                                                                                       \
      LT_FREAD("1", "2", "3", "4")                                                                                                                       \
      "v_and_b32 " LT_RS ", 0xfff, %[st]\n\t"                                                                                                            \
      "v_bfe_u32 " LT_RA ", %[bp], 5, 4\n\t"                                                                                                             \
      "v_lshrrev_b32 " LT_SL ", %[le], " LT_RS "\n\t"                                                                                                    \
      "v_lshl_add_u32 " LT_RA ", " LT_RA ", 8, %[ring]\n\t"                                                                                              \
      "v_lshlrev_b32 " LT_T4 ", " LT_SLOTSH_##V ", " LT_SL "\n\t"                                                                                        \
      "v_mad_u32_u24 " LT_T4 ", %[ctxe], %[clm], " LT_T4 "\n\t"                                                                                          \
      LT_EREAD_##V                                                                                                                                       \
      "ds_read2_b32 " LT_W ", " LT_RA " offset1:64\n\t"                                                                                                  \
      "ds_read_b32 " LT_W2 ", " LT_RA " offset:512\n\t"                                                                                                  \
      LT_WAITCNT(LT_PENDING_##V)                                                                                                                         \
      "v_add_u32 " LT_T5 ", %[aa], " LT_F0 "\n\t"                                                                                                        \
      "v_add3_u32 " LT_T7 ", %[cb], %[nb], " LT_F0 "\n\t"                                                                                                \
      "v_add_u32 " LT_T8 ", %[nzl], %[covm2]\n\t"                                                                                                        \
      "ds_read_u8 " LT_EZ ", " LT_T5 "\n\t"                                                                                                              \
      "v_bfe_u32 " LT_T8 ", " LT_T8 ", %[log2c], 6\n\t"                                                                                                  \
      "ds_read_u8 " LT_ENZ ", " LT_T7 " offset:1\n\t"                                                                                                    \
      "v_lshl_add_u32 " LT_T8 ", " LT_T8 ", 1, %[nnz2]\n\t"                                                                                              \
      "ds_read_u16 " LT_NC ", " LT_T8 "\n"                                                                                                               \
      ".Llt_loop_%=:\n\t"                                                                                                                                \
      LT_TRIP(V, "0", "", LT_WAITCNT("0"), "", "", LT_F1, "v_lshlrev_b32 " LT_A0 ", %[shift], " LT_T8 "\n\t", LT_LIVE)                                            \
      LT_TRIP(V, "1", "", LT_WAITCNT("0"), "", "", LT_F2, "v_lshlrev_b32 " LT_T8 ", %[shift], " LT_T8 "\n\tv_perm_b32 " LT_A0 ", " LT_T8 ", " LT_A0 ", %[perm]\n\t",  \
              LT_LIVE)                                                                                                                                   \
      LT_TRIP(V, "2", "", LT_WAITCNT("0"), "", "", LT_F3, "v_lshlrev_b32 " LT_A1 ", %[shift], " LT_T8 "\n\t", LT_LIVE)                                            \
                     \
                        \
      LT_TRIP(V, "3", LT_FREAD("2", "3", "4", "5"), LT_WAITCNT("4"), LT_GROUP_MASKS, LT_WAITCNT(LT_PENDING_##V), LT_F0,                                                              \
              "v_lshlrev_b32 " LT_T8 ", %[shift], " LT_T8 "\n\tv_perm_b32 " LT_A1 ", " LT_T8 ", " LT_A1 ", %[perm]\n\t",                                 \
              LT_STORE LT_COUNT "v_add_u32 %[dst], 8, %[dst]\n\t")                                                                                              \
                                                             \
      "s_and_b64 vcc, vcc, s[98:99]\n\t"                                                                                                                 \
      "s_and_b64 vcc, vcc, s[100:101]\n\t"                                                                                                               \
      "s_and_b64 exec, exec, vcc\n\t"                                                                                                                    \
      "s_cbranch_execz .Llt_end_%=\n\t"                                                                                                                  \
      "s_bcnt1_i32_b64 s98, exec\n\t"                                                                                                                    \
      "s_cmp_ge_u32 s98, %[cont]\n\t"                                                                                                                    \
      "s_cbranch_scc1 .Llt_loop_%=\n"                                                                                                                    \
      ".Llt_end_%=:\n\t"                                                                                                                                 \
      "s_waitcnt lgkmcnt(0)\n\t"                                                                                                                         \
      "s_mov_b64 exec, %[act]\n\t"                                                                                                                       \
      "v_mov_b32 %[alo], " LT_A0 "\n\t"                                                                                                                  \
      "v_mov_b32 %[ahi], " LT_A1 "\n\t"                                                                                                                  \
      "s_mov_b64 exec, s[96:97]"                                                                                                                         \
      : [st] "+v"(p_st), [bp] "+v"(p_bp), [k] "+v"(p_k), [nzl] "+v"(p_nzl), [ctxe] "+v"(p_ctxe), [aa] "+v"(p_aa), [nb] "+v"(p_nb), [dst] "+v"(p_dst),    \
        [alo] "+v"(p_alo), [ahi] "+v"(p_ahi), [grp] "+s"(p_grp)                                                                                          \
      : [log2c] "v"(p_log2c), [cb] "v"(p_cb), [covm2] "v"(p_covm2), [ring] "v"(p_ring), [rend] "v"(p_rend), [size] "v"(p_size), [act] "s"(p_act),        \
        [cont] "s"(p_cont), [le] "s"(p_le), [em] "s"(p_em), [clm] "s"(p_clm), [nnz2] "s"(p_nnz2), [shift] "s"(p_shift), [coef] "s"(p_coef),              \
        [perm] "s"(0x05040100u), [c64k] "s"(0x10000u), [a6la] "s"(p_la), [a6s1] "s"(8u - (p_la)), [a6s2] "s"(24u + (p_la))                                                                                                  \
      : "memory", "vcc", "scc", "s96", "s97", "s98", "s99", "s100", "s101", "v100", "v101", "v102", "v103", "v104", "v105", "v106", "v107", "v108",       \
        "v109", "v110", "v111", "v112", "v113", "v114", "v115", "v116", "v117", "v118", "v119", "v120", "v121", "v122", "v123", "v124", "v125", "v126",  \
        "v127", "v128", "v129", "v130", "v131")

#define JXL_LANES_TRIP_LOOP(...) JXL_LANES_TRIP_LOOP_(8, "", __VA_ARGS__)
#define JXL_LANES_TRIP_LOOP_COUNTED(...) JXL_LANES_TRIP_LOOP_(8, "s_add_u32 %[grp], %[grp], 1\n\t", __VA_ARGS__)
#define JXL_LANES_TRIP_LOOP6(...) JXL_LANES_TRIP_LOOP_(6, "", __VA_ARGS__)
#define JXL_LANES_TRIP_LOOP6_COUNTED(...) JXL_LANES_TRIP_LOOP_(6, "s_add_u32 %[grp], %[grp], 1\n\t", __VA_ARGS__)

#endif
```

Before: 92360.

## Specialize EPF weight clamp and hoist sigma selection in row filter

Adds an LE1 template path that clamps EPF weights with a single fmed3 into [0,1] when all sigma multipliers are non-negative, and falls back to max(0) variants otherwise. For single-EPF iterations it precomputes the per-column sigma choice outside the row loop, moves the horizontal plus-sum inside the output-row branch, and pins some values with empty asm to steer register allocation. It also scalarizes the sRGB-for-u8 helper and extends the entropy lanes profiler with an extra-bits trip counter. The filter changes are meant to trim ALU work per pixel, at the cost of doubling the number of row-kernel instantiations.

```diff
diff --git a/libjxl_amd/csrc/hip/jxl_hip_api.hip b/libjxl_amd/csrc/hip/jxl_hip_api.hip
--- a/libjxl_amd/csrc/hip/jxl_hip_api.hip
+++ b/libjxl_amd/csrc/hip/jxl_hip_api.hip
@@ -290,6 +290,7 @@
     int key;
     uint32_t first, count, tiles_x, tiles_y;
     bool u8srgb;
+    bool le1;
   };
   Buf tb_params, tb_desc, fb_params;
   std::vector<const JxlHipContext*> db_ctxs;
@@ -1518,10 +1519,11 @@
     const int key = FilterKey(c);
     const uint32_t tx = (c->xs + jxlhip::kFusedTW - 1) / jxlhip::kFusedTW;
     const uint32_t ty = (c->band_y1 - c->band_y0 + jxlhip::kFusedTH - 1) / jxlhip::kFusedTH;
-    if (c0->fgroups.empty() || c0->fgroups.back().key != key) c0->fgroups.push_back({key, uint32_t(j), 0, 0, 0, true});
+    if (c0->fgroups.empty() || c0->fgroups.back().key != key) c0->fgroups.push_back({key, uint32_t(j), 0, 0, 0, true, true});
     JxlHipContext::FilterGroup& g = c0->fgroups.back();
     g.count++;
     g.u8srgb = g.u8srgb && fparams[j].f.rgb && !fparams[j].f.rgbf && !fparams[j].filtered && !fparams[j].f.linear_output;
+    for (int stage = 1; stage < 3; stage++) g.le1 = g.le1 && fparams[j].sm[stage] >= 0.0f && fparams[j].bsm[stage] >= 0.0f;
     if (c->gray8_fast && !g.u8srgb) return JXLHIP_ERR_INVALID_ARGUMENT;
     g.tiles_x = tx > g.tiles_x ? tx : g.tiles_x;
     g.tiles_y = ty > g.tiles_y ? ty : g.tiles_y;
@@ -1572,8 +1574,13 @@
   const RowsKernel n2t = jxlhip::k_filter_rows2<true, 2, false>, n2f = jxlhip::k_filter_rows2<false, 2, false>;
   const RowsKernel k1g = jxlhip::k_filter_rows2<true, 1, true, true>, k2g = jxlhip::k_filter_rows2<true, 2, true, true>;
   const RowsKernel n1g = jxlhip::k_filter_rows2<true, 1, false, true>, n2g = jxlhip::k_filter_rows2<true, 2, false, true>;
+  const RowsKernel w1f = jxlhip::k_filter_rows2<false, 1, true, false, false>, w2f = jxlhip::k_filter_rows2<false, 2, true, false, false>;
+  const RowsKernel v1f = jxlhip::k_filter_rows2<false, 1, false, false, false>, v2f = jxlhip::k_filter_rows2<false, 2, false, false, false>;
+  const RowsKernel w1g = jxlhip::k_filter_rows2<true, 1, true, true, false>, w2g = jxlhip::k_filter_rows2<true, 2, true, true, false>;
+  const RowsKernel v1g = jxlhip::k_filter_rows2<true, 1, false, true, false>, v2g = jxlhip::k_filter_rows2<true, 2, false, true, false>;
   if (gray && !g.u8srgb) return JXLHIP_ERR_INVALID_ARGUMENT;
-  const RowsKernel k = gray ? (gab ? (epf == 2 ? k2g : k1g) : (epf == 2 ? n2g : n1g))
+  const RowsKernel k = !g.le1 ? (gray ? (gab ? (epf == 2 ? w2g : w1g) : (epf == 2 ? v2g : v1g)) : (gab ? (epf == 2 ? w2f : w1f) : (epf == 2 ? v2f : v1f)))
+                       : gray ? (gab ? (epf == 2 ? k2g : k1g) : (epf == 2 ? n2g : n1g))
                        : gab ? (epf == 2 ? (g.u8srgb ? k2t : k2f) : (g.u8srgb ? k1t : k1f))
                              : (epf == 2 ? (g.u8srgb ? n2t : n2f) : (g.u8srgb ? n1t : n1f));
   for (uint32_t z = 0; z < g.count; z += 65535) {
@@ -1772,9 +1779,10 @@
   b.started = c0->batch_ctxs.size() > 1 ? GateCounter(c0) : nullptr;
   const bool prof = EnvInt("JXLHIP_LANES_PROF", 0) != 0;
   const size_t nwaves = c0->batch_wgs;
+  constexpr int W = jxlhip::kLanesProfWords;
   if (prof) {
-    HIP_TRY(hipMalloc(reinterpret_cast<void**>(&b.prof), nwaves * 64));
-    HIP_TRY(hipMemsetAsync(b.prof, 0, nwaves * 64, c0->stream));
+    HIP_TRY(hipMalloc(reinterpret_cast<void**>(&b.prof), nwaves * W * 8));
+    HIP_TRY(hipMemsetAsync(b.prof, 0, nwaves * W * 8, c0->stream));
   }
   hipLaunchKernelGGL(k, dim3(c0->batch_wgs), dim3(64), c0->batch_lds, c0->stream, b);
   HIP_TRY(hipGetLastError());
@@ -1789,30 +1797,30 @@
     GateAdvance(c0->device, c0->batch_wgs, cap);
   }
   if (prof) {
-    std::vector<unsigned long long> h(nwaves * 8);
+    std::vector<unsigned long long> h(nwaves * W);
     HIP_TRY(hipStreamSynchronize(c0->stream));
-    HIP_TRY(hipMemcpy(h.data(), b.prof, nwaves * 64, hipMemcpyDeviceToHost));
+    HIP_TRY(hipMemcpy(h.data(), b.prof, nwaves * W * 8, hipMemcpyDeviceToHost));
     (void)hipFree(b.prof);
-    unsigned long long mx[8] = {0, 0, 0, 0, 0, 0, 0, 0};
-    double sum[8] = {0, 0, 0, 0, 0, 0, 0, 0};
+    unsigned long long mx[W] = {};
+    double sum[W] = {};
     size_t used = 0;
     for (size_t w = 0; w < nwaves; w++) {
-      if (!h[w * 8 + 3] && !h[w * 8 + 2]) continue;
+      if (!h[w * W + 3] && !h[w * W + 2]) continue;
       used++;
-      if (h[w * 8] > mx[0]) for (int j = 0; j < 8; j++) mx[j] = h[w * 8 + j];
-      for (int j = 0; j < 8; j++) sum[j] += double(h[w * 8 + j]);
-    }
-    const char* names[8] = {"cycles", "refill_cycles", "passes", "trips", "lane_trips", "trip_cycles", "pass_lanes_served", "pass_cycles"};
+      if (h[w * W] > mx[0]) for (int j = 0; j < W; j++) mx[j] = h[w * W + j];
+      for (int j = 0; j < W; j++) sum[j] += double(h[w * W + j]);
+    }
+    const char* names[W] = {"cycles", "refill_cycles", "passes", "trips", "lane_trips", "trip_cycles", "pass_lanes_served", "pass_cycles", "extra_bits_trips"};
     std::string line = "{\"waves\": " + std::to_string(used) + ", \"longest\": {";
-    for (int j = 0; j < 8; j++) line += std::string(j ? ", " : "") + "\"" + names[j] + "\": " + std::to_string(mx[j]);
+    for (int j = 0; j < W; j++) line += std::string(j ? ", " : "") + "\"" + names[j] + "\": " + std::to_string(mx[j]);
     line += "}, \"mean\": {";
-    for (int j = 0; j < 8; j++) line += std::string(j ? ", " : "") + "\"" + names[j] + "\": " + std::to_string((unsigned long long)(sum[j] / (used ? used : 1)));
+    for (int j = 0; j < W; j++) line += std::string(j ? ", " : "") + "\"" + names[j] + "\": " + std::to_string((unsigned long long)(sum[j] / (used ? used : 1)));
     line += "}}";
     fprintf(stderr, "[lanes prof] %s\n", line.c_str());
     if (b.debug & 16)
       for (size_t w = 0; w < nwaves && w < 64; w++) {
-        const unsigned long long hw = h[w * 8 + 6];
-        fprintf(stderr, "[lanes wave] %zu cycles %llu trips %llu trip_cycles %llu pass_cycles %llu passes %llu refill_cycles %llu simd %llu cu %llu sh %llu se %llu xcc %llu\n", w, h[w * 8], h[w * 8 + 3], h[w * 8 + 5], h[w * 8 + 7], h[w * 8 + 2], h[w * 8 + 1], (hw >> 4) & 3,
+        const unsigned long long hw = h[w * W + 6];
+        fprintf(stderr, "[lanes wave] %zu cycles %llu trips %llu trip_cycles %llu pass_cycles %llu passes %llu refill_cycles %llu simd %llu cu %llu sh %llu se %llu xcc %llu\n", w, h[w * W], h[w * W + 3], h[w * W + 5], h[w * W + 7], h[w * W + 2], h[w * W + 1], (hw >> 4) & 3,
                 (hw >> 8) & 15, (hw >> 12) & 1, (hw >> 13) & 7, (hw >> 32) & 15);
       }
   }
diff --git a/libjxl_amd/csrc/hip/jxl_hip_entropy_lanes.h b/libjxl_amd/csrc/hip/jxl_hip_entropy_lanes.h
--- a/libjxl_amd/csrc/hip/jxl_hip_entropy_lanes.h
+++ b/libjxl_amd/csrc/hip/jxl_hip_entropy_lanes.h
@@ -28,6 +28,7 @@
 constexpr uint32_t kLanesNzRows = 96;
 constexpr uint32_t kLanesRingWords = 16;
 constexpr uint32_t kLanesBlockRing = 8;
+constexpr int kLanesProfWords = 9;
 constexpr int kLanesTrips = 4;
 constexpr uint32_t kLanesRefillEvery = 4;
 constexpr uint32_t kLanesExtraPassMin = 8;
@@ -241,7 +242,7 @@
   const uint32_t shift = T.shift;
   constexpr uint32_t kPerChunk = 8 / sizeof(CoefT);
 
-  unsigned long long t_begin = 0, t_service = 0, n_service = 0, n_trips = 0, n_lane_trips = 0, t_wait = 0, t_dma = 0, t_trans = 0, n_calls = 0;
+  unsigned long long t_begin = 0, t_service = 0, n_service = 0, n_trips = 0, n_lane_trips = 0, t_wait = 0, t_dma = 0, t_trans = 0, n_calls = 0, n_extra_trips = 0;
   if (B.prof) t_begin = __builtin_readcyclecounter();
   __builtin_amdgcn_s_waitcnt(0);
   auto dma_group4 = [&](bool in, uint32_t row_lds, const void* base, uint32_t off) {
@@ -282,7 +283,8 @@
                                           ring_end, size, actm, cont_min, log_entry, entry_mask, cl_mul, nnz2_addr, shift, coef_base, log_alpha);
             }
             if (B.prof) t_wait += __builtin_readcyclecounter() - th;
-            n_trips += groups * kLanesTrips;
+            n_trips += (groups & 0x7FFFu) * kLanesTrips;
+            n_extra_trips += groups >> 15;
             n_calls++;
           } else {
             if constexpr (A6) {
@@ -757,7 +759,7 @@
     }
   }
   if (B.prof && lane == 0) {
-    unsigned long long* o = B.prof + size_t(blockIdx.x) * 8;
+    unsigned long long* o = B.prof + size_t(blockIdx.x) * kLanesProfWords;
     o[0] = __builtin_readcyclecounter() - t_begin;
     o[1] = t_service;
     o[2] = n_service;
@@ -765,6 +767,7 @@
     o[5] = t_wait;
     o[6] = t_dma;
     o[7] = t_trans;
+    o[8] = n_extra_trips;
     if (B.debug & 32) o[6] = n_calls;
     if (B.debug & 16) {
       uint32_t hw, xcc;
@@ -776,7 +779,7 @@
   if (B.prof) {
     unsigned long long total = n_lane_trips;
     for (int off = 32; off; off >>= 1) total += __shfl_down(total, off);
-    if (lane == 0) B.prof[size_t(blockIdx.x) * 8 + 4] = total;
+    if (lane == 0) B.prof[size_t(blockIdx.x) * kLanesProfWords + 4] = total;
   }
 }
 
diff --git a/libjxl_amd/csrc/hip/jxl_hip_filter_fused.h b/libjxl_amd/csrc/hip/jxl_hip_filter_fused.h
--- a/libjxl_amd/csrc/hip/jxl_hip_filter_fused.h
+++ b/libjxl_amd/csrc/hip/jxl_hip_filter_fused.h
@@ -361,11 +361,11 @@
   return f2{copysignf(a.x > 0.0031308f ? hi.x : lo.x, v.x), copysignf(a.y > 0.0031308f ? hi.y : lo.y, v.y)};
 }
 
-__device__ __forceinline__ f2 LinearToSrgb2ForU8(f2 v) {
-  const f2 p = f2{__builtin_amdgcn_exp2f(__builtin_amdgcn_logf(v.x) * (1.0f / 2.4f)), __builtin_amdgcn_exp2f(__builtin_amdgcn_logf(v.y) * (1.0f / 2.4f))};
-  const f2 hi = p * 1.055f - 0.055f;
-  const f2 lo = v * 12.92f;
-  return f2{v.x > 0.0031308f ? hi.x : lo.x, v.y > 0.0031308f ? hi.y : lo.y};
+__device__ __forceinline__ float LinearToSrgbForU8(float v) {
+  const float p = __builtin_amdgcn_exp2f(__builtin_amdgcn_logf(v) * (1.0f / 2.4f));
+  const float hi = p * 1.055f - 0.055f;
+  const float lo = v * 12.92f;
+  return v > 0.0031308f ? hi : lo;
 }
 
 struct P2 {
@@ -379,14 +379,16 @@
 __device__ __forceinline__ P2 operator*(P2 a, float b) { return P2{a.x * b, a.y * b}; }
 __device__ __forceinline__ P2 operator*(float b, P2 a) { return P2{b * a.x, b * a.y}; }
 __device__ __forceinline__ P2 Max0(P2 a) { return P2{__builtin_fmaxf(a.x, 0.0f), __builtin_fmaxf(a.y, 0.0f)}; }
+template <bool LE1>
+__device__ __forceinline__ P2 EpfWeight(P2 w) {
+  if constexpr (LE1) return P2{__builtin_amdgcn_fmed3f(w.x, 0.0f, 1.0f), __builtin_amdgcn_fmed3f(w.y, 0.0f, 1.0f)};
+  return Max0(w);
+}
 __device__ __forceinline__ P2 Srgb2(P2 v) {
   const f2 r = LinearToSrgb2(f2{v.x, v.y});
   return P2{r.x, r.y};
 }
-__device__ __forceinline__ P2 Srgb2ForU8(P2 v) {
-  const f2 r = LinearToSrgb2ForU8(f2{v.x, v.y});
-  return P2{r.x, r.y};
-}
+__device__ __forceinline__ P2 Srgb2ForU8(P2 v) { return P2{LinearToSrgbForU8(v.x), LinearToSrgbForU8(v.y)}; }
 __device__ __forceinline__ __amdgpu_buffer_rsrc_t RawBuffer(const void* p) {
   return __builtin_amdgcn_make_buffer_rsrc(const_cast<void*>(p), 0, 0xFFFFFFFFu, 0x00020000);
 }
@@ -402,7 +404,7 @@
   return P2{f.x, f.y};
 }
 
-template <bool U8SRGB, int EPF = 1, bool GAB = true, bool GREY = false>
+template <bool U8SRGB, int EPF = 1, bool GAB = true, bool GREY = false, bool LE1 = true>
 __global__ __launch_bounds__(64 * kRowsWaves) void k_filter_rows2(const FusedFilterParams* params, int strip_rows) {
   static_assert(EPF == 1 || EPF == 2, "(Gaborish +) one or two EPF iterations");
   static_assert(U8SRGB || !GREY, "the one-channel writer exists for 8-bit sRGB only");
@@ -438,6 +440,8 @@
   const GF32W rgbf = U8SRGB ? nullptr : (GF32W)(uintptr_t)P.f.rgbf;
   const bool linear_output = U8SRGB ? false : P.f.linear_output != 0;
   const P2 zero2 = P2{0.0f, 0.0f};
+  float cm1x = xb0 ? P.bsm[1] : P.sm[1], cm1y = xb1 ? P.bsm[1] : P.sm[1], bm1 = P.bsm[1];
+  if constexpr (EPF == 1) asm volatile("" : "+v"(cm1x), "+v"(cm1y), "+v"(bm1));
   P2 p[3][4], h1[3][4], g[3][4], dh[4], dv[4];
   P2 e[3][4];
   float is_prev = 0.0f;
@@ -521,7 +525,9 @@
       for (int c = 0; c < 3; c++) {
         const P2 gn = g[c][N], gm = g[c][M1];
         a.x = __builtin_fabsf(gn.x - gn.y) * P.f.ch_scale[c] + a.x;
-        a.y = __builtin_fabsf(FromRight(gn.x) - gn.y) * P.f.ch_scale[c] + a.y;
+        float dr = FromRight(gn.x) - gn.y;
+        asm volatile("" : "+v"(dr));
+        a.y = __builtin_fabsf(dr) * P.f.ch_scale[c] + a.y;
         b.x = __builtin_fabsf(gm.x - gn.x) * P.f.ch_scale[c] + b.x;
         b.y = __builtin_fabsf(gm.y - gn.y) * P.f.ch_scale[c] + b.y;
       }
@@ -535,14 +541,15 @@
       return P2{w.x + d[M1].y, w.y + FromRight(d[M1].x)};
     };
     const P2 pv = plus_sum(dv);
-    const P2 ph = plus_sum(dh);
     if (EPF == 2 ? (j >= 2 * HALO - 2 && r1 <= y1) : (j >= 2 * HALO && r < y1)) {
+      const P2 ph = plus_sum(dh);
       P2 o[3] = {g[0][M2], g[1][M2], g[2][M2]};
       {
         const float is_k = is < -3.90524291751269967465540850526868f ? -__builtin_inff() : is;
         const int rm1 = EPF == 2 ? (r1 < 0 ? -1 - r1 : (r1 >= ys ? 2 * ys - 1 - r1 : r1)) : r;
         const bool yb = ((rm1 & 7) == 0) || ((rm1 & 7) == 7);
-        const P2 inv_sig = P2{is_k * ((xb0 || yb) ? P.bsm[1] : P.sm[1]), is_k * ((xb1 || yb) ? P.bsm[1] : P.sm[1])};
+        const P2 inv_sig = EPF == 1 ? P2{is_k * (yb ? bm1 : cm1x), is_k * (yb ? bm1 : cm1y)}
+                                    : P2{is_k * ((xb0 || yb) ? P.bsm[1] : P.sm[1]), is_k * ((xb1 || yb) ? P.bsm[1] : P.sm[1])};
         P2 wk[4];
         wk[0] = pv_prev * inv_sig + 1.0f;
         wk[1] = P2{FromLeft(ph.y) * inv_sig.x + 1.0f, ph.x * inv_sig.y + 1.0f};
@@ -551,7 +558,7 @@
         P2 wsum = P2{1.0f, 1.0f};
 #pragma unroll
         for (int k = 0; k < 4; k++) {
-          wk[k] = Max0(wk[k]);
+          wk[k] = EpfWeight<LE1>(wk[k]);
           wsum = wsum + wk[k];
         }
         const P2 inv_w = P2{__builtin_amdgcn_rcpf(wsum.x), __builtin_amdgcn_rcpf(wsum.y)};
@@ -596,7 +603,7 @@
             sad.x = __builtin_fabsf(nb[k][c].x - e[c][M1].x) * P.f.ch_scale[c] + sad.x;
             sad.y = __builtin_fabsf(nb[k][c].y - e[c][M1].y) * P.f.ch_scale[c] + sad.y;
           }
-          const P2 wk2 = Max0(sad * inv_sig2 + 1.0f);
+          const P2 wk2 = EpfWeight<LE1>(sad * inv_sig2 + 1.0f);
           wsum = wsum + wk2;
 #pragma unroll
           for (int c = 0; c < 3; c++) acc[c] = wk2 * nb[k][c] + acc[c];
diff --git a/libjxl_amd/csrc/hip/jxl_hip_lanes_trip.inc b/libjxl_amd/csrc/hip/jxl_hip_lanes_trip.inc
--- a/libjxl_amd/csrc/hip/jxl_hip_lanes_trip.inc
+++ b/libjxl_amd/csrc/hip/jxl_hip_lanes_trip.inc
@@ -70,7 +70,7 @@
 #define LT_PENDING_8 "3"
 #define LT_PENDING_6 "5"
 
-#define LT_TRIP(V, J, FPRE, WAIT, MID, WF, F, PACK, TAIL)                                                                  \
+#define LT_TRIP(V, J, XC, FPRE, WAIT, MID, WF, F, PACK, TAIL)                                                                  \
   "v_and_b32 " LT_T1 ", %[em], " LT_RS "\n\t"                                                               \
   "v_lshrrev_b32 " LT_T3 ", 12, %[st]\n\t"                                                          \
   FPRE                                                                                                               \
@@ -106,6 +106,7 @@
   "s_cbranch_scc0 .Llt_skip" J "_%=\n\t"                                                                             \
                                        \
   "s_and_saveexec_b64 s[100:101], s[98:99]\n\t"                                                                      \
+  XC                                                                                                                 \
   LT_MSB_##V                                                                                       \
   LT_LSB_##V                                                                                       \
   "v_alignbit_b32 " LT_TC ", " LT_W1 ", " LT_W0 ", %[bp]\n\t"                \
@@ -178,7 +179,7 @@
   "ds_read_u8 " LT_F2 ", " LT_TB "\n\t"                          \
   "ds_read_u8 " LT_F3 ", " LT_TC "\n\t"
 
-#define JXL_LANES_TRIP_LOOP_(V, LT_COUNT, p_grp, p_st, p_bp, p_k, p_nzl, p_ctxe, p_aa, p_nb, p_dst, p_alo, p_ahi, p_log2c, p_cb, p_covm2, p_ring, p_rend, p_size, p_act,     \
+#define JXL_LANES_TRIP_LOOP_(V, LT_COUNT, LT_XCOUNT, p_grp, p_st, p_bp, p_k, p_nzl, p_ctxe, p_aa, p_nb, p_dst, p_alo, p_ahi, p_log2c, p_cb, p_covm2, p_ring, p_rend, p_size, p_act,     \
                             p_cont, p_le, p_em, p_clm, p_nnz2, p_shift, p_coef, p_la)                                                                        \
   asm volatile(                                                                                                                                          \
       "s_mov_b64 s[96:97], exec\n\t"                                                                                                                     \
@@ -203,13 +204,13 @@
       "v_lshl_add_u32 " LT_T8 ", " LT_T8 ", 1, %[nnz2]\n\t"                                                                                              \
       "ds_read_u16 " LT_NC ", " LT_T8 "\n"                                                                                                               \
       ".Llt_loop_%=:\n\t"                                                                                                                                \
-      LT_TRIP(V, "0", "", LT_WAITCNT("0"), "", "", LT_F1, "v_lshlrev_b32 " LT_A0 ", %[shift], " LT_T8 "\n\t", LT_LIVE)                                            \
-      LT_TRIP(V, "1", "", LT_WAITCNT("0"), "", "", LT_F2, "v_lshlrev_b32 " LT_T8 ", %[shift], " LT_T8 "\n\tv_perm_b32 " LT_A0 ", " LT_T8 ", " LT_A0 ", %[perm]\n\t",  \
+      LT_TRIP(V, "0", LT_XCOUNT, "", LT_WAITCNT("0"), "", "", LT_F1, "v_lshlrev_b32 " LT_A0 ", %[shift], " LT_T8 "\n\t", LT_LIVE)                                            \
+      LT_TRIP(V, "1", LT_XCOUNT, "", LT_WAITCNT("0"), "", "", LT_F2, "v_lshlrev_b32 " LT_T8 ", %[shift], " LT_T8 "\n\tv_perm_b32 " LT_A0 ", " LT_T8 ", " LT_A0 ", %[perm]\n\t",  \
               LT_LIVE)                                                                                                                                   \
-      LT_TRIP(V, "2", "", LT_WAITCNT("0"), "", "", LT_F3, "v_lshlrev_b32 " LT_A1 ", %[shift], " LT_T8 "\n\t", LT_LIVE)                                            \
+      LT_TRIP(V, "2", LT_XCOUNT, "", LT_WAITCNT("0"), "", "", LT_F3, "v_lshlrev_b32 " LT_A1 ", %[shift], " LT_T8 "\n\t", LT_LIVE)                                            \
                      \
                         \
-      LT_TRIP(V, "3", LT_FREAD("2", "3", "4", "5"), LT_WAITCNT("4"), LT_GROUP_MASKS, LT_WAITCNT(LT_PENDING_##V), LT_F0,                                                              \
+      LT_TRIP(V, "3", LT_XCOUNT, LT_FREAD("2", "3", "4", "5"), LT_WAITCNT("4"), LT_GROUP_MASKS, LT_WAITCNT(LT_PENDING_##V), LT_F0,                                                              \
               "v_lshlrev_b32 " LT_T8 ", %[shift], " LT_T8 "\n\tv_perm_b32 " LT_A1 ", " LT_T8 ", " LT_A1 ", %[perm]\n\t",                                 \
               LT_STORE LT_COUNT "v_add_u32 %[dst], 8, %[dst]\n\t")                                                                                              \
                                                              \
@@ -235,9 +236,11 @@
         "v109", "v110", "v111", "v112", "v113", "v114", "v115", "v116", "v117", "v118", "v119", "v120", "v121", "v122", "v123", "v124", "v125", "v126",  \
         "v127", "v128", "v129", "v130", "v131")
 
-#define JXL_LANES_TRIP_LOOP(...) JXL_LANES_TRIP_LOOP_(8, "", __VA_ARGS__)
-#define JXL_LANES_TRIP_LOOP_COUNTED(...) JXL_LANES_TRIP_LOOP_(8, "s_add_u32 %[grp], %[grp], 1\n\t", __VA_ARGS__)
-#define JXL_LANES_TRIP_LOOP6(...) JXL_LANES_TRIP_LOOP_(6, "", __VA_ARGS__)
-#define JXL_LANES_TRIP_LOOP6_COUNTED(...) JXL_LANES_TRIP_LOOP_(6, "s_add_u32 %[grp], %[grp], 1\n\t", __VA_ARGS__)
+#define LT_GROUP_COUNT "s_add_u32 %[grp], %[grp], 1\n\t"
+#define LT_EXTRA_COUNT "s_add_u32 %[grp], %[grp], 0x8000\n\t"
+#define JXL_LANES_TRIP_LOOP(...) JXL_LANES_TRIP_LOOP_(8, "", "", __VA_ARGS__)
+#define JXL_LANES_TRIP_LOOP_COUNTED(...) JXL_LANES_TRIP_LOOP_(8, LT_GROUP_COUNT, LT_EXTRA_COUNT, __VA_ARGS__)
+#define JXL_LANES_TRIP_LOOP6(...) JXL_LANES_TRIP_LOOP_(6, "", "", __VA_ARGS__)
+#define JXL_LANES_TRIP_LOOP6_COUNTED(...) JXL_LANES_TRIP_LOOP_(6, LT_GROUP_COUNT, LT_EXTRA_COUNT, __VA_ARGS__)
 
 #endif
```

Result: no change. 92710, median of 6 (+0.4%).
